# nickirk/pymes

Hardware: AMD Instinct MI355X
Metric: ccsd_iteration_time (lower is better)
Workload: dtype f64

## Files before the change

### include/pymes_amd.h

```cpp
#ifndef PYMES_AMD_H
#define PYMES_AMD_H

#include <stdint.h>

#ifdef __cplusplus
extern "C" {
#endif

typedef struct pymes_ctx pymes_ctx;

#define PYMES_NOCC_MAX_FUSED 90
#define PYMES_NOCC_MAX_LAMBDA 88
#define PYMES_NOCC_MAX_BRA_DRESS 80

const char* pymes_last_error(void);
const char* pymes_backend(void);
int pymes_ctx_create(pymes_ctx** out, int device, int no, int nv, uint64_t workspace_bytes );
int pymes_ctx_destroy(pymes_ctx* ctx);
int pymes_ctx_set_stream(pymes_ctx* ctx, void* hip_stream);
int pymes_ctx_sync(pymes_ctx* ctx);
int pymes_ctx_workspace(pymes_ctx* ctx, uint64_t* capacity_bytes, uint64_t* high_water_bytes);

int pymes_malloc(pymes_ctx* ctx, uint64_t bytes, void** dev_ptr);
int pymes_free(pymes_ctx* ctx, void* dev_ptr);
// ... 7 lines not shown

int pymes_graph_begin(pymes_ctx* ctx);
int pymes_graph_end(pymes_ctx* ctx, void** graph);
int pymes_graph_abort(pymes_ctx* ctx);
int pymes_graph_launch(pymes_ctx* ctx, void* graph);
int pymes_graph_destroy(pymes_ctx* ctx, void* graph);
int pymes_upload(pymes_ctx* ctx, void* dst_dev, const void* src_host, uint64_t bytes);
int pymes_download(pymes_ctx* ctx, void* dst_host, const void* src_dev, uint64_t bytes);
int pymes_copy(pymes_ctx* ctx, void* dst_dev, const void* src_dev, uint64_t bytes);
int pymes_memset_zero(pymes_ctx* ctx, void* dst_dev, uint64_t bytes);

int pymes_contract(pymes_ctx* ctx, double alpha,
                   const double* A_dev, const char* la, const int64_t* dimA, const int64_t* strideA,
                   const double* B_dev, const char* lb, const int64_t* dimB, const int64_t* strideB,
                   double beta, double* C_dev, const char* lc, const int64_t* dimC, const int64_t* strideC,
                   const char* batch);
int pymes_permute(pymes_ctx* ctx, double alpha, const double* in_dev, const char* li, const int64_t* dim_in,
                  const int64_t* stride_in, double beta, double* out_dev, const char* lo,
                  const int64_t* stride_out);
int pymes_dgemm(pymes_ctx* ctx, int64_t M, int64_t N, int64_t K, double alpha, const double* A_dev, int64_t a_sm,
                int64_t a_sk, const double* B_dev, int64_t b_sk, int64_t b_sn, double beta, double* C_dev,
                int64_t ldc);

int pymes_set_V_pqrs(pymes_ctx* ctx, const double* V, int on_device, const int64_t* strides);
int pymes_set_V_block(pymes_ctx* ctx, const char* name, const double* data, int64_t n_elements, int on_device,
                      const int64_t* strides);
int pymes_V_exchange_asymmetry(pymes_ctx* ctx, double* out_host);
int pymes_exchange_asymmetry(pymes_ctx* ctx, const double* A_dev, const double* B_dev, const int64_t* dims,
                             double* out_host);
int pymes_set_V_from_factors(pymes_ctx* ctx, const double* B_host, int naux);
int pymes_set_integral_shard(pymes_ctx* ctx, int rank, int world);
int pymes_integral_bytes(pymes_ctx* ctx, int64_t* bytes);
int pymes_shard_rows_ptr(pymes_ctx* ctx, const double** vp, const double** vm, int64_t* row0, int64_t* row1, int64_t* ldp,
                         int64_t* ldm);
int pymes_V_block_ptr(pymes_ctx* ctx, const char* name, int dressed, double** dev_ptr, int64_t* n_elements);
int pymes_set_orbital_energies(pymes_ctx* ctx, const double* eps_o_host, const double* eps_v_host);

int pymes_ccsd_t_triples(pymes_ctx* ctx, int64_t* n_triples);
int pymes_ccsd_t(pymes_ctx* ctx, const double* eps_host, const double* t1_dev, const double* t2_dev, int64_t t_begin,
                 int64_t t_end, double* per_triple_dev, double* e_out_host);

int pymes_ccsd_t_lambda(pymes_ctx* ctx, const double* eps_host, const double* t2_dev, const double* lam1_dev,
                        const double* lam2_dev, int64_t t_begin, int64_t t_end, double* per_triple_dev, double* e_out_host);

int pymes_fno_density(pymes_ctx* ctx, const double* v_ijab_dev, int n_frozen, double* D_host, double* e_mp2_host);
int pymes_derive_context(pymes_ctx* src, pymes_ctx* dst, int n_frozen, const double* C_host, int nv_dst);

int pymes_mp2(pymes_ctx* ctx, double level_shift, double* t2_dev, double* e_out_host);
int pymes_ccsd_dress_fock(pymes_ctx* ctx, const double* f_dev, const double* t1_dev, double* fd_dev);
#define PYMES_DRESS_ABIJ_REDUCED (1u << 16)
int pymes_ccsd_dress_V(pymes_ctx* ctx, const double* t1_dev, uint32_t block_mask);
int pymes_ccsd_dress_V_slab(pymes_ctx* ctx, const double* t1_dev, uint32_t block_mask, int p_begin, int p_end,
                            int q_begin, int q_end);
int pymes_ccsd_singles_residual(pymes_ctx* ctx, const double* fd_dev, const double* t1_dev, const double* t2_dev,
                                double* r1_dev);
int pymes_ccsd_singles_residual_partial(pymes_ctx* ctx, const double* fd_dev, const double* t1_dev, const double* t2_dev,
                                        double* r1_dev, int rank, int world, uint32_t flags );
#define PYMES_DCD 1u
#define PYMES_USE_DRESSED 2u
#define PYMES_SKIP_LADDER 4u
#define PYMES_SYM_LADDER 8u
#define PYMES_SLAB_RINGS_ONLY 64u
#define PYMES_SLAB_LADDERS_ONLY 128u
#define PYMES_REUSE_LAYOUTS 32u
#define PYMES_T1_ZERO (1u << 20)
#define PYMES_SYM_RINGS 16u
int pymes_doubles_residual(pymes_ctx* ctx, const double* f_dev, const double* t2_dev, double* r2_dev,
                           uint32_t flags);
int pymes_ladder(pymes_ctx* ctx, const double* t2_dev, double* r2_dev, int a_begin, int a_end, int dressed,
                 double beta);
int pymes_ladder_sym(pymes_ctx* ctx, const double* t2_dev, double* L_dev, int64_t row_begin, int64_t row_end,
                     int dressed, int hole_ladder);
int pymes_ladder_sym_unpack(pymes_ctx* ctx, const double* L_dev, double* r2_dev, double beta);
int pymes_ladder_sym_multi(pymes_ctx* ctx, const double* const* x_dev, int k, double* L_all_dev, int dressed);
int pymes_ladder_dress(pymes_ctx* ctx, const double* V_dev, const double* Pk_dev, const double* t1_dev, double* W_dev,
                       int64_t ld, int64_t r0, int64_t r1, int minus_half);
int pymes_pair_layouts(pymes_ctx* ctx, const double* x_dev, double* Xd_dev, double* Xx_dev, double* Xt_dev);
int pymes_symmetrised_assemble(pymes_ctx* ctx, const double* V_dev, const double* L_dev, const double* N_dev,
                               const double* D_dev, const double* X_dev, double* R_dev);
int pymes_hole_ladder_packed(pymes_ctx* ctx, const double* x_dev, const double* I_dev, double* L_dev, int64_t row_begin,
                             int64_t row_end, const double* y_dev);
int pymes_hole_ladder_packed_multi(pymes_ctx* ctx, const double* const* x_dev, const double* const* I_dev,
                                   const double* const* y_dev, int k, double* L_all_dev);
int pymes_ccsd_residuals(pymes_ctx* ctx, const double* f_dev, const double* t1_dev, const double* t2_dev, uint32_t flags,
                         double* r1_dev, double* r2_dev);
int pymes_ccsd_iterate(pymes_ctx* ctx, const double* f_dev, double* t1_dev, double* t2_dev, uint32_t flags, double level_shift,
                       double delta, double* dt1_dev, double* dt2_dev, double* out6_host);
int pymes_ccsd_release(pymes_ctx* ctx);

int pymes_residual_slab(pymes_ctx* ctx, const double* f_dev, const double* t2_dev, double* ETd_dev, double* ETx_dev,
                        double* L_dev, int rank, int world, uint32_t flags, const double* t1_dev, double* QK_dev,
                        const double* P_dev);
int pymes_slab_prepare_ws(pymes_ctx* ctx, int64_t* n_doubles);
int pymes_slab_prepare(pymes_ctx* ctx, const double* t2_dev, double* P_dev, int rank, int world, uint32_t flags);
int pymes_residual_finish(pymes_ctx* ctx, const double* f_dev, const double* t2_dev, const double* ETd_dev,
                          const double* ETx_dev, const double* L_dev, double* r2_dev, uint32_t flags,
                          const double* t1_dev, const double* QK_dev);
int pymes_ccsd_dress_abcd_rows(pymes_ctx* ctx, const double* t1_dev, int a_begin, int a_end, int lower_only);
int pymes_residual_finish_pairs(pymes_ctx* ctx, const double* f_dev, const double* t2_dev, const double* ETd_dev,
                                const double* ETx_dev, const double* L_dev, double* Rc_dev, uint32_t flags,
                                const double* t1_dev, const double* QK_dev, int rank, int world, const double* Xvv_dev);
int pymes_xvv_partial(pymes_ctx* ctx, const double* f_dev, const double* t2_dev, double* Xvv_dev, int rank, int world,
                      uint32_t flags);
int pymes_ccsd_dress_fock_ws(pymes_ctx* ctx, int64_t* n_doubles);
int pymes_ccsd_dress_fock_partial(pymes_ctx* ctx, const double* t1_dev, double* W_dev, int rank, int world);
int pymes_ccsd_dress_fock_finish(pymes_ctx* ctx, const double* f_dev, const double* t1_dev, const double* W_dev,
// ... 30 lines not shown
    double *ETd, *ETx, *L, *QK, *Tall, *W, *Xvv, *P, *R1, *S;
} pymes_shard_buffers;
int pymes_shard_buffer_sizes(pymes_ctx* ctx, int world, int64_t* sizes_out);
int pymes_ccsd_sharded_residuals(pymes_ctx* ctx, const double* f_dev, double* fd_dev, const double* t1_dev, double* t2_dev,
                                 const pymes_shard_buffers* buffers, uint32_t flags, double* rc_dev);
int pymes_ccsd_sharded_finish(pymes_ctx* ctx, const double* f_dev, const double* t1_dev, const double* tc_dev,
                              const double* dtc_dev, const pymes_shard_buffers* buffers, int* slot);
int pymes_ccsd_sharded_energy(pymes_ctx* ctx, int slot, double* out_host );
int pymes_ccsd_sharded_await(pymes_ctx* ctx, double* t2_dev, const pymes_shard_buffers* buffers);
int pymes_ccd_sharded_residuals(pymes_ctx* ctx, const double* f_dev, double* t2_dev, const pymes_shard_buffers* buffers,
                                uint32_t flags, double* rc_dev);
#define PYMES_OWNER_TILES (1u << 21)
typedef int (*pymes_alltoallv_fn)(void* user, const double* send_dev, const int64_t* send_counts, double* recv_dev,
                                  const int64_t* recv_counts, void* stream, int64_t* ticket);
int pymes_set_alltoallv(pymes_ctx* ctx, pymes_alltoallv_fn fn );
int pymes_owner_tile_sizes(pymes_ctx* ctx, int rank, int world, int64_t* send_doubles, int64_t* recv_doubles);
int pymes_set_owner_tile_buffers(pymes_ctx* ctx, double* send_dev, double* recv_dev);
int pymes_ccsd_energy(pymes_ctx* ctx, const double* f_dev, const double* t1_dev, const double* t2_dev,
                      double* e_out_host);
int pymes_ccd_energy(pymes_ctx* ctx, const double* t2_dev, double* e_out_host);

int pymes_ueg_eval_2b(pymes_ctx* ctx, int n_p, int n_ele, int imax, int mode, double L, double k_cutoff, double gamma,
                      int lattice_cutoff, const int32_t* k_int_host, const int32_t* index_map_host, double* V_dev);

int pymes_ueg_eval_2b_corr(pymes_ctx* ctx, int n_p, int n_ele, int imax, int mode, double L, int lattice_cutoff,
                           int correlator, const double* params_host, const int32_t* k_int_host,
                           const int32_t* index_map_host, double* V_dev);
int pymes_ueg_eval_2b_tab(pymes_ctx* ctx, int n_p, int n_ele, int imax, int mode, double L, int lattice_cutoff,
                          const int32_t* k_int_host, const int32_t* index_map_host, const double* tab_scalar_host,
                          const double* tab_array_host, int64_t tab_len, double* V_dev);

int pymes_dots(pymes_ctx* ctx, int npairs, const double* const* x_dev, const double* const* y_dev, int64_t n,
               double* out_host);
int pymes_dots_var(pymes_ctx* ctx, int npairs, const double* const* x_dev, const double* const* y_dev,
                   const int64_t* n, double* out_host);
int pymes_lincomb(pymes_ctx* ctx, double* out_dev, int nx, const double* const* x_dev, const double* c_host,
                  int64_t n);
int pymes_gemm_group_begin(pymes_ctx* ctx);
int pymes_gemm_group_end(pymes_ctx* ctx, int64_t* launches, int64_t* products);
int pymes_gram(pymes_ctx* ctx, int m, int n, const double* const* x_dev, const double* const* y_dev, int64_t len,
               double* out_host);
int pymes_lincomb_multi(pymes_ctx* ctx, int m, int n, const double* const* x_dev, const double* c_host,
                        const double* beta_host, double* const* y_dev, int64_t len);
int pymes_diis_mix(pymes_ctx* ctx, double* state_host, int ntypes, int m, int was_full, const double* const* err_hist_dev,
                   const double* const* err_new_dev, const int64_t* sizes, const double* const* amp_hist_dev,
                   double* const* out_dev);
int pymes_diis_step(pymes_ctx* ctx, double* state_dev, int npairs, const double* const* x_dev, const double* const* y_dev,
                    const int64_t* n, int ntypes, int m, int was_full);
int pymes_diis_solve(double* state_host, const double* overlaps_host, int ntypes, int m, int was_full);
int pymes_lincomb_dev(pymes_ctx* ctx, double* out_dev, int nx, const double* const* x_dev, const double* coeff_dev,
                      int64_t n);
#define PYMES_SYM_TAIL (1u << 22)
int pymes_sym_tail(pymes_ctx* ctx, int* yes);
int pymes_cc_update_to_sym(pymes_ctx* ctx, double* t_out_dev, double* dt_dev, const double* t_in_dev, const double* r_dev,
                           double level_shift, double delta);
int pymes_dots_sym(pymes_ctx* ctx, int npairs, const double* const* x_dev, const double* const* y_dev, const int64_t* n,
                   const int* sym, double* out_host);
int pymes_lincomb_sym(pymes_ctx* ctx, double* out_dev, int nx, const double* const* x_dev, const double* c_host, int64_t n);
int pymes_diis_mix_sym(pymes_ctx* ctx, double* state_host, int ntypes, int m, int was_full, const double* const* err_hist_dev,
                       const double* const* err_new_dev, const int64_t* sizes, const double* const* amp_hist_dev,
                       double* const* out_dev, const int* sym_types);
int pymes_energy_norms_start_sym(pymes_ctx* ctx, const double* f_dev, const double* t1_dev, const double* t2_dev,
                                 const double* dt2_dev, int* slot);
int pymes_pair_layouts_sym(pymes_ctx* ctx, const double* x_dev, double* Xd_dev, double* Xx_dev, double* Xt_dev);
int pymes_cmul(pymes_ctx* ctx, const double* mr_dev, const double* mi_dev, const double* xr_dev, const double* xi_dev,
               double* yr_dev, double* yi_dev, int64_t n);

int pymes_hf_fock_matrix(pymes_ctx* ctx, const double* h_host, double* f_host);

int pymes_fcidump_header(const char* path, int* n_elec, int* n_orb);
int pymes_fcidump_read_host(const char* path, int is_tc, double* e_core, double* eps_host, double* h_host,
                            double* V_host);
int pymes_fcidump_load(pymes_ctx* ctx, const char* path, int is_tc, double* e_core, double* eps_host, double* h_host,
                       int64_t* n_two_electron_lines);

int pymes_packed_header(const char* path, int* kind, int* n_elec, int* n_orb, int* naux);
int pymes_packed_load(pymes_ctx* ctx, const char* path, double* e_core, double* eps_host, double* h_host);
int pymes_packed_write(pymes_ctx* ctx, const char* path, int n_elec, double e_core, const double* eps_host,
                       const double* h_host);
int pymes_packed_write_factors(const char* path, int n_elec, int n_orb, int naux, double e_core, const double* eps_host,
                               const double* h_host, const double* B_host);

typedef struct pymes_eom pymes_eom;
int pymes_eom_sigma_prepare(pymes_ctx* ctx, const double* f_host, const double* t2_dev, int dressed, pymes_eom** out);
int pymes_eom_sigma_flags(pymes_eom* h, int* flags);
int pymes_eom_sigma_apply(pymes_eom* h, int k, const double* const* u1_dev, const double* const* u2_dev, const int* sym,
                          double* const* s1_dev, double* const* s2_dev);
int pymes_eom_diagonals(pymes_ctx* ctx, const double* f_host, const double* t2_dev, int dressed, double* d1_dev, double* d2_dev);
int pymes_scratch_trim(pymes_ctx* ctx);
int pymes_eom_sigma_destroy(pymes_eom* h);

#define PYMES_IPEA_IP 0
#define PYMES_IPEA_EA 1
typedef struct pymes_ipea pymes_ipea;
int pymes_ipea_sigma_prepare(pymes_ctx* ctx, const double* f_host, const double* t2_dev, int dressed, int kind, pymes_ipea** out);
int pymes_ipea_sigma_flags(pymes_ipea* h, int* flags);
int pymes_ipea_sigma_apply(pymes_ipea* h, int k, const double* const* r1_dev, const double* const* r2_dev, double* const* s1_dev,
                           double* const* s2_dev);
int pymes_ipea_sigma_diagonals(pymes_ipea* h, double* d1_dev, double* d2_dev);
int pymes_ipea_sigma_correction(pymes_ipea* h, int n, const double* const* s_dev, const double* const* r_dev, const double* w_host,
                                const double* d_dev, double shift, double* const* q_dev, int64_t off2, int64_t len,
                                double* norms_host);
int pymes_ipea_sigma_destroy(pymes_ipea* h);
int pymes_ipea_sigma_apply_left(pymes_ipea* h, int k, const double* const* l1_dev, const double* const* l2_dev,
                                double* const* o1_dev, double* const* o2_dev);
int pymes_ipea_dyson(pymes_ipea* h, const double* t1_dev, const double* lam1_dev, const double* lam2_dev, int k,
// ... 35 lines not shown
```

### pymes_amd/_lib.py

```python
import ctypes as C
import os

import numpy as np

_HERE = os.path.dirname(os.path.abspath(__file__))
DEFAULT_PATH = os.environ.get("PYMES_AMD_LIBRARY") or os.path.join(_HERE, "lib", "libpymes_amd.so")

c_double_p = C.POINTER(C.c_double)
c_i64_p = C.POINTER(C.c_int64)


class ShardBuffers(C.Structure):
    _fields_ = [(k, C.c_void_p) for k in ("ETd", "ETx", "L", "QK", "Tall", "W", "Xvv", "P", "R1", "S")]

c_pp = C.POINTER(C.c_void_p)

SIGNATURES = {
    "pymes_last_error": (C.c_char_p, []),
    "pymes_backend": (C.c_char_p, []),
    "pymes_ctx_create": (C.c_int, [c_pp, C.c_int, C.c_int, C.c_int, C.c_uint64]),
    "pymes_ctx_destroy": (C.c_int, [C.c_void_p]),
    "pymes_ctx_set_stream": (C.c_int, [C.c_void_p, C.c_void_p]),
    "pymes_ctx_sync": (C.c_int, [C.c_void_p]),
    "pymes_ctx_workspace": (C.c_int, [C.c_void_p, C.POINTER(C.c_uint64), C.POINTER(C.c_uint64)]),
# ... 108 lines not shown
    "pymes_scatter": (C.c_int, [C.c_void_p, C.c_void_p, C.c_uint64, c_i64_p, c_double_p, C.c_int64]),
    "pymes_tc_single_contraction": (C.c_int, [C.c_void_p, C.c_void_p, C.c_int, C.c_int, C.c_void_p]),
    "pymes_tc_double_contraction": (C.c_int, [C.c_void_p, C.c_void_p, C.c_int, C.c_int, C.c_void_p]),
    "pymes_tc_triple_contraction": (C.c_int, [C.c_void_p, C.c_void_p, C.c_int, C.c_int, c_double_p]),
    "pymes_dots": (C.c_int, [C.c_void_p, C.c_int, c_pp, c_pp, C.c_int64, c_double_p]),
    "pymes_dots_var": (C.c_int, [C.c_void_p, C.c_int, c_pp, c_pp, c_i64_p, c_double_p]),
    "pymes_lincomb": (C.c_int, [C.c_void_p, C.c_void_p, C.c_int, c_pp, c_double_p, C.c_int64]),
    "pymes_cmul": (C.c_int, [C.c_void_p] * 7 + [C.c_int64]),
    "pymes_ccsd_residuals": (C.c_int, [C.c_void_p, C.c_void_p, C.c_void_p, C.c_void_p, C.c_uint32, C.c_void_p, C.c_void_p]),
    "pymes_ccsd_iterate": (C.c_int, [C.c_void_p, C.c_void_p, C.c_void_p, C.c_void_p, C.c_uint32, C.c_double, C.c_double,
                                     C.c_void_p, C.c_void_p, C.c_void_p]),
    "pymes_ccsd_release": (C.c_int, [C.c_void_p]),
    "pymes_set_collectives": (C.c_int, [C.c_void_p, C.c_void_p]),
    "pymes_shard_buffer_sizes": (C.c_int, [C.c_void_p, C.c_int, c_i64_p]),
    "pymes_ccsd_sharded_residuals": (C.c_int, [C.c_void_p] * 6 + [C.c_uint32, C.c_void_p]),
    "pymes_ccd_sharded_residuals": (C.c_int, [C.c_void_p] * 4 + [C.c_uint32, C.c_void_p]),
    "pymes_set_alltoallv": (C.c_int, [C.c_void_p, C.c_void_p]),
    "pymes_owner_tile_sizes": (C.c_int, [C.c_void_p, C.c_int, C.c_int, c_i64_p, c_i64_p]),
    "pymes_set_owner_tile_buffers": (C.c_int, [C.c_void_p, C.c_void_p, C.c_void_p]),
    "pymes_ccsd_sharded_finish": (C.c_int, [C.c_void_p] * 6 + [C.POINTER(C.c_int)]),
    "pymes_ccsd_sharded_energy": (C.c_int, [C.c_void_p, C.c_int, C.c_void_p]),
    "pymes_ccsd_sharded_await": (C.c_int, [C.c_void_p, C.c_void_p, C.c_void_p]),
    "pymes_cshift_inv": (C.c_int, [C.c_void_p, C.c_void_p] + [C.c_double] * 5 + [C.c_void_p, C.c_void_p, C.c_int64]),
    "pymes_eom_sigma_prepare": (C.c_int, [C.c_void_p, C.c_void_p, C.c_void_p, C.c_int, C.c_void_p]),
    "pymes_eom_sigma_flags": (C.c_int, [C.c_void_p, C.c_void_p]),
    "pymes_eom_sigma_apply": (C.c_int, [C.c_void_p, C.c_int] + [C.c_void_p] * 5),
    "pymes_eom_diagonals": (C.c_int, [C.c_void_p, C.c_void_p, C.c_void_p, C.c_int, C.c_void_p, C.c_void_p]),
    "pymes_scratch_trim": (C.c_int, [C.c_void_p]),
    "pymes_eom_sigma_destroy": (C.c_int, [C.c_void_p]),
    "pymes_eom_sigma_apply_left": (C.c_int, [C.c_void_p, C.c_int] + [C.c_void_p] * 5),
    "pymes_lambda_step": (C.c_int, [C.c_void_p] * 5 + [C.c_double, C.c_double, C.c_int, C.c_int] + [C.c_void_p] * 5),
    "pymes_rdm1": (C.c_int, [C.c_void_p] * 5 + [C.c_double, C.c_void_p]),
    "pymes_ipea_sigma_prepare": (C.c_int, [C.c_void_p, C.c_void_p, C.c_void_p, C.c_int, C.c_int, C.c_void_p]),
    "pymes_ipea_sigma_flags": (C.c_int, [C.c_void_p, C.c_void_p]),
    "pymes_ipea_sigma_apply": (C.c_int, [C.c_void_p, C.c_int] + [C.c_void_p] * 4),
    "pymes_ipea_sigma_apply_left": (C.c_int, [C.c_void_p, C.c_int] + [C.c_void_p] * 4),
    "pymes_ipea_dyson": (C.c_int, [C.c_void_p] * 4 + [C.c_int] + [C.c_void_p] * 6),
    "pymes_ipea_sigma_diagonals": (C.c_int, [C.c_void_p, C.c_void_p, C.c_void_p]),
    "pymes_ipea_sigma_correction": (C.c_int, [C.c_void_p, C.c_int, C.c_void_p, C.c_void_p, C.c_void_p, C.c_void_p, C.c_double,
                                              C.c_void_p, C.c_int64, C.c_int64, C.c_void_p]),
    "pymes_ipea_sigma_destroy": (C.c_int, [C.c_void_p]),
    "pymes_tdm1": (C.c_int, [C.c_void_p] * 5 + [C.c_int] + [C.c_void_p] * 7),
    "pymes_eom_correction": (C.c_int, [C.c_void_p, C.c_int, C.c_void_p, C.c_void_p, C.c_void_p, C.c_void_p, C.c_double,
                                       C.c_void_p, C.c_int64, C.c_int64, C.c_void_p]),
    "pymes_diis_mix": (C.c_int, [C.c_void_p, C.c_void_p, C.c_int, C.c_int, C.c_int, c_pp, c_pp, c_i64_p, c_pp, c_pp]),
    "pymes_diis_solve": (C.c_int, [C.c_void_p, C.c_void_p, C.c_int, C.c_int, C.c_int]),
    "pymes_diis_step": (C.c_int, [C.c_void_p, C.c_void_p, C.c_int, c_pp, c_pp, c_i64_p, C.c_int, C.c_int, C.c_int]),
    "pymes_gemm_group_begin": (C.c_int, [C.c_void_p]),
    "pymes_gemm_group_end": (C.c_int, [C.c_void_p, c_i64_p, c_i64_p]),
    "pymes_gram": (C.c_int, [C.c_void_p, C.c_int, C.c_int, c_pp, c_pp, C.c_int64, c_double_p]),
    "pymes_lincomb_multi": (C.c_int, [C.c_void_p, C.c_int, C.c_int, c_pp, C.c_void_p, C.c_void_p, c_pp, C.c_int64]),
    "pymes_lincomb_dev": (C.c_int, [C.c_void_p, C.c_void_p, C.c_int, c_pp, C.c_void_p, C.c_int64]),
    "pymes_sym_tail": (C.c_int, [C.c_void_p, C.POINTER(C.c_int)]),
    "pymes_cc_update_to_sym": (C.c_int, [C.c_void_p, C.c_void_p, C.c_void_p, C.c_void_p, C.c_void_p, C.c_double, C.c_double]),
    "pymes_dots_sym": (C.c_int, [C.c_void_p, C.c_int, c_pp, c_pp, c_i64_p, C.POINTER(C.c_int), c_double_p]),
    "pymes_lincomb_sym": (C.c_int, [C.c_void_p, C.c_void_p, C.c_int, c_pp, c_double_p, C.c_int64]),
    "pymes_diis_mix_sym": (C.c_int, [C.c_void_p, C.c_void_p, C.c_int, C.c_int, C.c_int, c_pp, c_pp, c_i64_p, c_pp, c_pp,
                                     C.POINTER(C.c_int)]),
    "pymes_energy_norms_start_sym": (C.c_int, [C.c_void_p, C.c_void_p, C.c_void_p, C.c_void_p, C.c_void_p,
                                               C.POINTER(C.c_int)]),
    "pymes_pair_layouts_sym": (C.c_int, [C.c_void_p, C.c_void_p, C.c_void_p, C.c_void_p, C.c_void_p]),
    "pymes_stats": (C.c_int, [C.c_void_p, C.c_int, c_i64_p, c_double_p, c_i64_p, c_double_p]),
    "pymes_prof_enable": (C.c_int, [C.c_void_p, C.c_int]),
    "pymes_prof_reset": (C.c_int, [C.c_void_p]),
    "pymes_prof_query": (C.c_int, [C.c_void_p, C.c_int, c_i64_p, c_i64_p, c_double_p, c_double_p]),
}

PYMES_DCD, PYMES_USE_DRESSED, PYMES_SKIP_LADDER, PYMES_SYM_LADDER, PYMES_SYM_RINGS = 1, 2, 4, 8, 16
PYMES_OWNER_TILES = 1 << 21
PYMES_REUSE_LAYOUTS = 32
PYMES_T1_ZERO = 1 << 20
PYMES_SYM_TAIL = 1 << 22
PYMES_SLAB_RINGS_ONLY, PYMES_SLAB_LADDERS_ONLY = 64, 128
PYMES_DRESS_ABIJ_REDUCED = 1 << 16


class PymesError(RuntimeError):
    pass


class Library:

    BACKEND = "hip-gfx950"

    def __init__(self, path=None):
        path = path or DEFAULT_PATH
        if not os.path.exists(path):
            raise PymesError(
                f"{path} not found: build the HIP extension first (python -c 'import __graft_entry__ as g; "
                "g.build()' or make -C pymes_amd/csrc).  pymes_amd has no CPU fallback.")
        self.path = path
        self.dll = C.CDLL(path)
        for name, (res, args) in SIGNATURES.items():
            fn = getattr(self.dll, name)
            fn.restype, fn.argtypes = res, args
        self.backend = self.dll.pymes_backend().decode()
        if self.backend != self.BACKEND:
            raise PymesError(f"{path} reports backend '{self.backend}', expected '{self.BACKEND}'")

    def call(self, name, *args):
        rc = getattr(self.dll, name)(*args)
        if rc != 0:
            raise PymesError(f"{name}: {self.dll.pymes_last_error().decode()}")


_default = None
# ... 21 lines not shown
```

### pymes_amd/csrc/capi.cpp

```cpp
#include <chrono>
#include <cstdio>
#include <cstring>
#include <exception>
#include <algorithm>
#include <mutex>
#include <set>
#include <string>
#include <vector>

#include "../../include/pymes_amd.h"
#include "diis_small.h"
#include "engine.h"
#include "eom.h"
#include "fcidump.h"
#include "packed.h"

using pymes::Engine;
using pymes::TView;

struct pymes_ctx {
    Engine* e;
};
struct pymes_eom {
    pymes::EomSigma* s;
// ... 368 lines not shown
        need(eo, "eps_o");
        need(ev, "eps_v");
        E(ctx).set_orbital_energies(eo, ev);
    });
}

int pymes_mp2(pymes_ctx* ctx, double shift, double* t2, double* e_out) {
    return guarded([&] {
        need(t2, "t2");
        need(e_out, "e_out");
        E(ctx).mp2(shift, t2, e_out);
    });
}
int pymes_ccsd_dress_fock(pymes_ctx* ctx, const double* f, const double* t1, double* fd) {
    return guarded([&] {
        need(f, "f"); need(t1, "t1"); need(fd, "fd");
        E(ctx).dress_fock(f, t1, fd);
    });
}
int pymes_ccsd_residuals(pymes_ctx* ctx, const double* f, const double* t1, const double* t2, uint32_t flags, double* r1,
                         double* r2) {
    return guarded([&] {
        need(f, "f"); need(t1, "t1"); need(t2, "t2"); need(r1, "r1"); need(r2, "r2");
        if (flags & ~(PYMES_DCD | PYMES_T1_ZERO | PYMES_SYM_TAIL))
            throw pymes::Error("ccsd_residuals: flags are PYMES_DCD | PYMES_T1_ZERO | PYMES_SYM_TAIL");
        E(ctx).ccsd_residuals(f, t1, t2, (flags & PYMES_DCD) | ((flags & PYMES_T1_ZERO) ? Engine::kT1Zero : 0u) |
                                             ((flags & PYMES_SYM_TAIL) ? Engine::kSymTail : 0u), r1, r2);
    });
}
int pymes_ccsd_iterate(pymes_ctx* ctx, const double* f, double* t1, double* t2, uint32_t flags, double level_shift, double delta,
                       double* dt1, double* dt2, double* out6) {
    return guarded([&] {
        need(f, "f"); need(t1, "t1"); need(t2, "t2"); need(dt1, "dt1"); need(dt2, "dt2"); need(out6, "out");
        if (flags & ~(PYMES_DCD | PYMES_T1_ZERO)) throw pymes::Error("ccsd_iterate: flags are PYMES_DCD | PYMES_T1_ZERO");
        Engine& e = E(ctx);
        if (e.capturing()) throw pymes::Error("ccsd_iterate reads the energy back: not inside a launch graph");
        e.ccsd_iterate(f, t1, t2, (flags & PYMES_DCD) | ((flags & PYMES_T1_ZERO) ? Engine::kT1Zero : 0u), level_shift, delta, dt1,
                       dt2, out6);
    });
}
int pymes_ccsd_release(pymes_ctx* ctx) {
    return guarded([&] {
        Engine& e = E(ctx);
        if (e.capturing()) throw pymes::Error("ccsd_release while a launch graph is being recorded");
        e.release_residual_buffers();
    });
}
int pymes_ccsd_dress_V(pymes_ctx* ctx, const double* t1, uint32_t mask) {
    return guarded([&] {
        need(t1, "t1");
        E(ctx).dress_V(t1, mask);
    });
}
int pymes_ccsd_dress_V_slab(pymes_ctx* ctx, const double* t1, uint32_t mask, int p_begin, int p_end, int q_begin,
                            int q_end) {
    return guarded([&] {
        need(t1, "t1");
        const int64_t cut[4] = {p_begin, p_end, q_begin, q_end};
        E(ctx).dress_V(t1, mask, cut);
    });
}
int pymes_ccsd_singles_residual(pymes_ctx* ctx, const double* fd, const double* t1, const double* t2, double* r1) {
    return guarded([&] {
        need(fd, "fd"); need(t1, "t1"); need(t2, "t2"); need(r1, "r1");
        E(ctx).singles_residual(fd, t1, t2, r1);
    });
}
int pymes_ccsd_singles_residual_partial(pymes_ctx* ctx, const double* fd, const double* t1, const double* t2, double* r1,
                                        int rank, int world, uint32_t flags) {
    return guarded([&] {
        need(fd, "fd"); need(t1, "t1"); need(t2, "t2"); need(r1, "r1");
        E(ctx).singles_residual_partial(fd, t1, t2, r1, rank, world, (flags & PYMES_REUSE_LAYOUTS) != 0);
    });
}
int pymes_doubles_residual(pymes_ctx* ctx, const double* f, const double* t2, double* r2, uint32_t flags) {
    return guarded([&] {
        need(f, "f"); need(t2, "t2"); need(r2, "r2");
        E(ctx).doubles_residual(f, t2, r2, flags);
    });
}
int pymes_ladder(pymes_ctx* ctx, const double* t2, double* r2, int a0, int a1, int dressed, double beta) {
    return guarded([&] {
        need(t2, "t2"); need(r2, "r2");
        E(ctx).ladder(t2, r2, a0, a1, dressed != 0, beta);
    });
}
int pymes_ladder_sym(pymes_ctx* ctx, const double* t2, double* L, int64_t r0, int64_t r1, int dressed, int hole) {
    return guarded([&] {
        need(t2, "t2"); need(L, "L");
        E(ctx).ladder_sym(t2, L, r0, r1, dressed != 0, hole);
    });
}
int pymes_symmetrised_assemble(pymes_ctx* ctx, const double* V, const double* L, const double* N, const double* D,
                               const double* X, double* R) {
    return guarded([&] {
        need(N, "N"); need(D, "D"); need(X, "X"); need(R, "R");
        pymes::Engine& e = E(ctx);
        if (!dev::fused_pair_kernels_ok(e.no)) throw pymes::Error("symmetrised_assemble: nocc too large for the LDS tile");
        dev::residual_assemble(V, L, N, D, X, R, e.no, e.nv, e.stream);
    });
}
int pymes_hole_ladder_packed(pymes_ctx* ctx, const double* x, const double* I, double* L, int64_t r0, int64_t r1,
                             const double* y) {
    return guarded([&] {
        need(x, "x"); need(I, "I"); need(L, "L");
        E(ctx).hole_ladder_packed(x, I, L, r0, r1, y);
// ... 127 lines not shown
            dev::pairs_unpack(xc_all + static_cast<int64_t>(r) * (c1 - c0) * 2 * o2, full, e.no, e.nv, r0, r1, e.stream);
        }
    });
}
int pymes_cc_update_pairs(pymes_ctx* ctx, double* tc, double* dtc, const double* rc, double shift, double delta, int rank,
                          int world) {
    return guarded([&] {
        need(tc, "tc"); need(dtc, "dtc"); need(rc, "rc");
        pymes::Engine& e = E(ctx);
        int64_t r0, r1;
        e.need_eps("cc_update_pairs");
        e.pair_chunk(rank, world, r0, r1);
        dev::cc_update_pairs(tc, dtc, rc, e.eps_o, e.eps_v, shift, delta, e.no, e.nv, r0, r1, e.stream);
    });
}
int pymes_ccsd_dress_abcd_rows(pymes_ctx* ctx, const double* t1, int a0, int a1, int lower_only) {
    return guarded([&] {
        need(t1, "t1");
        E(ctx).dress_abcd_rows(t1, a0, a1, lower_only != 0);
    });
}
int pymes_cc_update(pymes_ctx* ctx, double* t, double* dt, const double* r, double shift, double delta, int rank) {
    return guarded([&] {
        need(t, "t"); need(dt, "dt"); need(r, "r");
        E(ctx).cc_update(t, dt, r, shift, delta, rank);
    });
}
int pymes_cc_update_to(pymes_ctx* ctx, double* t_out, double* dt, const double* t_in, const double* r, double shift,
                       double delta, int rank) {
    return guarded([&] {
        need(t_out, "t_out"); need(dt, "dt"); need(t_in, "t_in"); need(r, "r");
        E(ctx).cc_update_to(t_out, dt, t_in, r, shift, delta, rank);
    });
}
int pymes_energy_norms(pymes_ctx* ctx, const double* f, const double* t1, const double* t2, const double* dt2,
                       double* out) {
    return guarded([&] {
        need(t2, "t2"); need(out, "out");
        if ((f == nullptr) != (t1 == nullptr)) throw pymes::Error("f and t1 must be given together");
        E(ctx).energy_norms(f, t1, t2, dt2, out);
    });
}
int pymes_energy_norms_start(pymes_ctx* ctx, const double* f, const double* t1, const double* t2, const double* dt2, int* slot) {
    return guarded([&] {
        need(t2, "t2"); need(slot, "slot");
        if ((f == nullptr) != (t1 == nullptr)) throw pymes::Error("f and t1 must be given together");
        *slot = E(ctx).energy_norms_start(f, t1, t2, dt2);
    });
}
int pymes_sym_tail(pymes_ctx* ctx, int* yes) {
    return guarded([&] {
        need(yes, "yes");
        *yes = Eq(ctx).sym_tail() ? 1 : 0;
    });
}
int pymes_cc_update_to_sym(pymes_ctx* ctx, double* t_out, double* dt, const double* t_in, const double* r, double shift,
                           double delta) {
    return guarded([&] {
        need(t_out, "t_out"); need(dt, "dt"); need(t_in, "t_in"); need(r, "r");
        E(ctx).cc_update_to(t_out, dt, t_in, r, shift, delta, 4, true);
    });
}
int pymes_energy_norms_start_sym(pymes_ctx* ctx, const double* f, const double* t1, const double* t2, const double* dt2,
                                 int* slot) {
    return guarded([&] {
        need(t2, "t2"); need(slot, "slot");
        if ((f == nullptr) != (t1 == nullptr)) throw pymes::Error("f and t1 must be given together");
        *slot = E(ctx).energy_norms_start(f, t1, t2, dt2, true);
    });
}
int pymes_pair_layouts_sym(pymes_ctx* ctx, const double* x, double* Xd, double* Xx, double* Xt) {
    return guarded([&] {
        need(x, "x"); need(Xx, "Xx"); need(Xt, "Xt");
        Engine& e = E(ctx);
        if (!dev::fused_pair_kernels_ok(e.no)) throw pymes::Error("pair_layouts: nocc too large for the LDS tile");
        if (e.sym_tail()) dev::t2_layouts_sym(x, Xd, Xx, Xt, e.no, e.nv, e.stream);
        else dev::t2_layouts(x, Xd, Xx, Xt, e.no, e.nv, e.stream);
    });
}
int pymes_energy_norms_wait(pymes_ctx* ctx, int slot, double* out) {
    return guarded([&] {
        need(out, "out");
        Eq(ctx).energy_norms_wait(slot, out);
    });
}
int pymes_readback_start(pymes_ctx* ctx, const double* dev_ptr, int n, int* slot) {
    return guarded([&] {
        need(dev_ptr, "dev_ptr"); need(slot, "slot");
        *slot = dev::readback_start(dev_ptr, n, E(ctx).stream);
    });
}
int pymes_readback_wait(pymes_ctx* ctx, int slot, double* out, int n) {
    return guarded([&] {
        need(out, "out");
        Eq(ctx);
        dev::readback_wait(slot, out, n);
    });
}
int pymes_energy_norms_pairs(pymes_ctx* ctx, const double* f, const double* t1, const double* tc, const double* dtc,
                             int rank, int world, double* out) {
    return guarded([&] {
        need(tc, "tc"); need(out, "out");
        if ((f == nullptr) != (t1 == nullptr)) throw pymes::Error("f and t1 must be given together");
        E(ctx).energy_norms_pairs(f, t1, tc, dtc, rank, world, out);
    });
}
// ... 696 lines not shown
```

### pymes_amd/csrc/cc.cpp

```cpp
#include <algorithm>
#include <cstdio>
#include <cstring>
#include <cstdlib>
#include <optional>
#include <vector>

#include "../../include/pymes_amd.h"
#include "engine.h"

#include <cmath>

namespace pymes {
static_assert(Engine::kT1Zero == PYMES_T1_ZERO && Engine::kOwnerTiles == PYMES_OWNER_TILES,
              "the engine's flag bits are the public ones");

namespace {
inline int64_t lpitch(int64_t n) { return PairDims::lpitch(n); }
inline TView packed_rows(double* p, int64_t rows, int64_t cols) { return slice(make_view(p, {rows, lpitch(cols)}), 1, 0, cols); }
inline TView pitched(double* p, int64_t r, int64_t c, int64_t ld) { return slice(make_view(p, {r, ld}), 1, 0, c); }
constexpr int P_klij = 0, P_ijka = 1, P_ijak = 2, P_ijab = 3, P_iajk = 4, P_iajb = 5, P_iabj = 6, P_iabc = 7,
              P_aibc = 11, P_abij = 12, P_abic = 13, P_abci = 14, P_abcd = 15;
}

double* Engine::get_static(const std::string& key) {
// ... 142 lines not shown
        contract(1.0, X1, "ajcl", Tx, "clbi", 0.0, Rx, "ajbi");
    }

    permute(1.0, Rd, "aibj", 1.0, R, "abij");
    if (quad) permute(1.0, Rx, "ajbi", 1.0, R, "abij");
    permute(1.0, Exd, "aibj", 1.0, R, "abij");
    permute(1.0, Exd, "bjai", 1.0, R, "abij");
    permute(1.0, Exx, "ajbi", 1.0, R, "abij");
    permute(1.0, Exx, "biaj", 1.0, R, "abij");
    permute(1.0, Exn, "abij", 1.0, R, "abij");
    permute(1.0, Exn, "baji", 1.0, R, "abij");
}

void Engine::ensure_xs() {
    if (!xs_oo_) xs_oo_ = static_cast<double*>(dev::dmalloc(sizeof(double) * no * no));
    if (!xs_vv_) xs_vv_ = static_cast<double*>(dev::dmalloc(sizeof(double) * nv * nv));
}

bool Engine::ring_fold_enabled() {
    if (const char* e = getenv("PYMES_RING_FOLD")) return atoi(e) != 0;
    return true;
}

bool Engine::sym_tail() const {
    if (const char* e = getenv("PYMES_SYM_TAIL"))
        if (atoi(e) == 0) return false;
    return dev::sym_tail_ok() && dev::fused_pair_kernels_ok(no);
}

void Engine::pair_layouts_of(const double* t2, bool want_td, bool sym) {
    const int64_t o = no, v = nv, ov = o * v;
    for (int i = want_td ? 0 : 1; i < 3; ++i)
        if (!lay_[i]) {
            if (capturing_) throw Error("pair_layouts_of: the pair layouts must exist before a launch graph is recorded (run one eager pass first)");
            lay_[i] = static_cast<double*>(dev::dmalloc(sizeof(double) * ov * ov));
        }
    lay_t2_ = nullptr;
    if (dev::fused_pair_kernels_ok(no)) {
        if (sym && sym_tail()) dev::t2_layouts_sym(t2, want_td ? lay_[0] : nullptr, lay_[1], lay_[2], no, nv, stream);
        else dev::t2_layouts(t2, want_td ? lay_[0] : nullptr, lay_[1], lay_[2], no, nv, stream);
        stats.permute_calls++;
        stats.permute_bytes += 8.0 * (want_td ? 5.0 : 4.0) * double(ov * ov);
    } else {
        TView T = make_view(const_cast<double*>(t2), {v, v, o, o});
        TView t4 = make_view(lay_[0], {v, o, v, o});
        if (want_td) permute(1.0, T, "abij", 0.0, t4, "aibj");
        t4.p = lay_[1];
        permute(1.0, T, "abij", 0.0, t4, "ajbi");
        t4.p = lay_[2];
        permute(2.0, T, "abij", 0.0, t4, "aibj");
        permute(-1.0, T, "baij", 1.0, t4, "aibj");
    }
    lay_t2_ = t2;
}

void Engine::slab_ladders(const double* t2, double* L, int rank, int world, unsigned flags, const double* t1, double* QK,
                          const double* P) {
    const bool dcd = flags & PYMES_DCD, dressed = flags & PYMES_USE_DRESSED;
    const int64_t o = no, v = nv;
    int64_t r0, r1;
    chunk(pair_dims().npp, rank, world, r0, r1);
    if (t1) {
        if (!QK) throw Error("residual_slab: QK buffer missing");
        int64_t q0, q1;
        chunk(o * v, rank, world, q0, q1);
        ladder_t1(t1, t2, L, r0, r1, QK, q0, q1, dcd, P ? P + o * o : nullptr);
    } else {
        ladder_sym(t2, L, r0, r1, dressed, dcd ? 2 : 1);
    }
}

void Engine::slab_rings_rows(const RingSlab& s) {
    const int64_t ov = static_cast<int64_t>(no) * nv, c0 = s.c0, c1 = s.c1, nc = c1 - c0;
    const bool quad = s.quad;
    const TView &Tx = s.Tx, &Ttd = s.Ttd, &ETd = s.ETd, &ETx = s.ETx;
    auto pairm = [&](double* p) { return make_view(p, {ov, ov}); };
    auto slabT = [&]() { return make_view(arena.alloc(nc * ov), {nc, ov}); };
    TView MT = slabT(), N1T = slabT();
    s.load_rows(2.0, s.Viabj, "kbcj", MT);
    s.load_rows(-1.0, s.Viajb, "kbjc", N1T);
    axpby(1.0, N1T, 1.0, MT);
    ring_xd_ = 0.0;
    auto rowsOf = [&](const TView& m) { return slice(m, 0, c0, c1); };
    if (quad) {
        contract(0.5, rowsOf(Ttd), "ny", pairm(get_static("Ld")), "yx", 1.0, MT, "nx");
        contract(0.5, rowsOf(Tx), "ny", pairm(get_static("Vx")), "yx", 1.0, N1T, "nx");
    } else {
        contract(1.0, rowsOf(Ttd), "ny", pairm(get_static("Vd")), "yx", 1.0, MT, "nx");
    }
    contract(1.0, N1T, "nk", Tx, "km", 0.0, ETx, "nm");
    contract(0.5, MT, "nk", Ttd, "km", 0.5, ETd, "nm", "", &ETx);
}

void Engine::slab_rings_cols(const RingSlab& s) {
    const int64_t o = no, v = nv, nn = n, ov = o * v, c0 = s.c0, c1 = s.c1, nc = c1 - c0;
    const bool quad = s.quad, traces = s.traces, fold = s.fold;
    const double w = quad ? 1.0 : 0.5;
    const double* t2 = s.t2;
    const TView &F = s.F, &Viajb = s.Viajb, &Viabj = s.Viabj, &Tx = s.Tx, &Ttd = s.Ttd, &ETd = s.ETd, &ETx = s.ETx;
    auto pairm = [&](double* p) { return make_view(p, {ov, ov}); };
    auto slab = [&]() { return make_view(arena.alloc(ov * nc), {ov, nc}); };
    auto cols = [&](const TView& m) { return slice(m, 1, c0, c1); };
    TView M = slab(), N1 = slab();
    const int64_t ring_tiles = ((ov + 127) / 128) * ((ov + 127) / 128);
    const bool paired = ring_tiles < 512;
    ring_xd_ = paired ? 0.5 : 0.0;
// ... 35 lines not shown
        ensure_xs();
        xs_oo_tag_.clear();
        xs_vv_tag_.clear();
        dev::pair_traces(M.p, nc, -cz, 0.0, xs_vv_, xs_oo_, no, nv, stream, quad ? N1.p : nullptr, -cu);
    }
    if (quad && paired) {
        pair_gemm(0.5, get_static("Ldh"), get_static("Vx"), Ttd.p, Tx.p, 1.0, M.p, N1.p);
    } else if (quad) {
        contract(0.5, pairm(get_static("Ld")), "xy", cols(Ttd), "yn", 1.0, M, "xn");
        contract(0.5, pairm(get_static("Vx")), "xy", cols(Tx), "yn", 1.0, N1, "xn");
    } else {
        contract(paired ? 0.5 : 1.0, pairm(get_static("Vd")), "xy", cols(Ttd), "yn", 1.0, M, "xn");
    }
    if (traces) {
        dev::pair_traces(M.p, nc, cz, 1.0, xs_vv_, xs_oo_, no, nv, stream, quad ? N1.p : nullptr, cu);
        xs_oo_tag_.set(t2, 0, 1);
        xs_vv_tag_.set(t2, 0, 1);
    }
    if (fold) {
        TView Xoo = make_view(arena.alloc(o * o), {o, o}), Xvv = make_view(arena.alloc(v * v), {v, v});
        copy(slice(slice(F, 0, 0, o), 1, 0, o), Xoo);
        axpby(w, make_view(xs_oo_, {o, o}), 1.0, Xoo);
        copy(slice(slice(F, 0, o, nn), 1, o, nn), Xvv);
        axpby(-w, make_view(xs_vv_, {v, v}), 1.0, Xvv);
        auto add_Dx = [&](const TView& m, double wgt) {
            const int64_t ld = m.st[0];
            const int64_t dv[3] = {v, v, o}, sv_in[3] = {1, v, 0}, sv_out[3] = {o * ld, o, ld + 1};
            axpby(wgt, make_view(Xvv.p, 3, dv, sv_in), 1.0, make_view(m.p, 3, dv, sv_out));
            const int64_t dn[3] = {v, o, o}, so_in[3] = {0, o, 1}, so_out[3] = {o * ld + o, ld, 1};
            axpby(-wgt, make_view(Xoo.p, 3, dn, so_in), 1.0, make_view(m.p, 3, dn, so_out));
        };
        add_Dx(M, paired ? 0.25 : 0.5);
        add_Dx(N1, 0.5);
        ring_fold_.set(t2, s.ETd_p);
    }
    if (paired) {
        pair_gemm(1.0, Tx.p, Ttd.p, N1.p, M.p, 0.0, ETx.p, ETd.p);
    } else {
        contract(1.0, Tx, "mk", N1, "kn", 0.0, ETx, "mn");
        contract(0.5, Ttd, "mk", M, "kn", 0.5, ETd, "mn", "", &ETx);
    }
}

void Engine::residual_slab(const double* f, const double* t2, double* ETd_p, double* ETx_p, double* L, int rank,
                           int world, unsigned flags, const double* t1, double* QK, const double* P) {
    const bool dcd = flags & PYMES_DCD, dressed = flags & PYMES_USE_DRESSED,
               skip_ladder = flags & (PYMES_SKIP_LADDER | PYMES_SLAB_RINGS_ONLY), skip_rings = flags & PYMES_SLAB_LADDERS_ONLY;
    const bool quad = !dcd;
    const int64_t o = no, v = nv, nn = n, ov = o * v;
    if (world < 1 || rank < 0 || rank >= world) throw Error("residual_slab: bad rank/world");
    if (L && !skip_ladder) check_shard_rank("residual_slab", rank, world);
    const double w = quad ? 1.0 : 0.5;
    TView F = make_view(const_cast<double*>(f), {nn, nn});
    if (L && !skip_ladder) slab_ladders(t2, L, rank, world, flags, t1, QK, P);
    if (skip_rings) return;
    ring_fold_.clear();
    int64_t c0, c1;
    chunk(ov, rank, world, c0, c1);
    const int64_t nc = c1 - c0;
    if (nc <= 0) return;
    TView Viajb = block(P_iajb, dressed), Viabj = block(P_iabj, dressed);

    ArenaScope scope(arena);
    auto pairm = [&](double* p) { return make_view(p, {ov, ov}); };
    const bool traces = !P && nc == ov;
    const bool fold = traces && ring_fold_enabled();
    pair_layouts_of(t2, !fold, flags & kSymTail);
    TView Td = pairm(lay_[0]), Tx = pairm(lay_[1]), Ttd = pairm(lay_[2]);
    TView ETd = slice(pairm(ETd_p), 0, c0, c1), ETx = slice(pairm(ETx_p), 0, c0, c1);
    const int64_t b0 = c0 / o, b1 = (c1 + o - 1) / o;
    auto load_cols = [&](double alpha, const TView& blk, const char* spec, const TView& dst) {
        TView src = slice(blk, 1, b0, b1);
        if (b0 * o == c0 && b1 * o == c1) {
            permute(alpha, src, spec, 0.0, make_view(dst.p, {v, o, b1 - b0, o}), "ckbj");
        } else {
            ArenaScope s2(arena);
            TView tmp = make_view(arena.alloc(ov * (b1 - b0) * o), {ov, (b1 - b0) * o});
            permute(alpha, src, spec, 0.0, make_view(tmp.p, {v, o, b1 - b0, o}), "ckbj");
            copy(slice(tmp, 1, c0 - b0 * o, c1 - b0 * o), dst);
        }
    };
    auto load_rows = [&](double alpha, const TView& blk, const char* spec, const TView& dst) {
        TView src = slice(blk, 1, b0, b1);
        if (b0 * o == c0 && b1 * o == c1) {
            permute(alpha, src, spec, 0.0, make_view(dst.p, {b1 - b0, o, v, o}), "bjck");
        } else {
            ArenaScope s2(arena);
            TView tmp = make_view(arena.alloc((b1 - b0) * o * ov), {(b1 - b0) * o, ov});
            permute(alpha, src, spec, 0.0, make_view(tmp.p, {b1 - b0, o, v, o}), "bjck");
            copy(slice(tmp, 0, c0 - b0 * o, c1 - b0 * o), dst);
        }
    };
    const RingSlab rs{t2, ETd_p, quad, traces, fold, c0, c1, F, Viajb, Viabj, Tx, Ttd, ETd, ETx, load_cols, load_rows};
    if (nc != ov) slab_rings_rows(rs);
    else slab_rings_cols(rs);
    if (!fold) {
        ArenaScope s2(arena);
        TView Foo = slice(slice(F, 0, 0, o), 1, 0, o);
        TView Xoo = make_view(arena.alloc(o * o), {o, o});
        copy(Foo, Xoo);
        if (P) {
            axpby(1.0, make_view(const_cast<double*>(P), {o, o}), 1.0, Xoo);
        } else if (traces) {
            axpby(w, make_view(xs_oo_, {o, o}), 1.0, Xoo);
        } else {
            TView Tp = make_view(arena.alloc(o * o * v * v), {v, v, o, o});
            permute(1.0, make_view(Ttd.p, {v, o, v, o}), "cidl", 0.0, Tp, "cdli");
            contract(w, make_view(get_static("Vk3"), {v, v, o, o}), "cdlk", Tp, "cdli", 1.0, Xoo, "ki");
        }
        TView Trows = make_view(Td.p + c0 * ov, {nc, v, o});
        TView Erows = make_view(ETd.p, {nc, v, o});
        contract(-1.0, Trows, "nak", Xoo, "ki", 1.0, Erows, "nai");
    }
}

int64_t Engine::slab_prepare_ws_doubles() const {
    const PairDims d = pair_dims();
    return static_cast<int64_t>(no) * no + d.opp * d.ldp + d.opp * d.ldm;
}

// ... 537 lines not shown
    const double t_q = 2.0 * double(o * v) * (double(npp) * double(opp) + double(npm) * double(opm)) / 70e12;
    return t_dress < 0.8 * t_q;
}

void Engine::ladder_t1(const double* t1, const double* t2, double* L, int64_t row0, int64_t row1, double* QK,
                       int64_t q0, int64_t q1, bool dcd, const double* J) {
    const PairDims d = pair_dims();
    const int64_t o = no, v = nv, ov = o * v, npp = d.npp, npm = d.npm, opp = d.opp, opm = d.opm, ldp = d.ldp, ldm = d.ldm;
    if (row0 < 0 || row1 > npp || row0 > row1) throw Error("ladder_t1: bad pair-row range");
    if (q0 < 0 || q1 > ov || q0 > q1) throw Error("ladder_t1: bad (k,b) row range");
    const int64_t rows = row1 - row0, qrows = q1 - q0;
    const PackedV V = rows > 0 ? ladder_rows("ladder_t1", row0, row1, false) : PackedV{nullptr, nullptr, false};
    bool dress = bra_dress_pays();
    const std::string kkey = ":" + std::to_string(q0) + ":" + std::to_string(q1);
    const std::string rkey = ":" + std::to_string(row0) + ":" + std::to_string(row1);
    if (dress && rows > 0 && (!static_.count("VpKx") || !static_.count("VpDress" + rkey))) {
        const int64_t lp = d.vlp, lm = d.vlm;
        const bool need_p = !static_.count("VpKx");
        double *tp = nullptr, *tm = nullptr, *px = nullptr, *mx = nullptr, *wp = nullptr, *wm = nullptr;
        bool ok = true;
        auto grab = [&](double*& p, int64_t n) { if (ok) { p = static_cast<double*>(dev::try_dmalloc(sizeof(double) * n)); ok = p != nullptr; } };
        if (!static_.count("VpDress" + rkey)) { grab(wp, rows * lp); grab(wm, rows * lm); }
        if (need_p) { grab(px, ov * lp); grab(mx, ov * lm); grab(tp, ov * lp); grab(tm, ov * lm); }
        if (!ok) {
            for (double* p : {tp, tm, px, mx, wp, wm}) dev::dfree(p);
            if (!(rows == npp && qrows == ov))
                throw Error("ladder_t1: out of device memory for the dressed copy of the packed V_abcd (PYMES_LADDER_DRESS=0 on every rank selects the Q_kb form)");
            dress_off_ = true;
            dress = false;
        } else {
            if (wp) {
                static_["VpDress" + rkey] = wp; static_["VmDress" + rkey] = wm;
                static_doubles_["VpDress" + rkey] = rows * lp; static_doubles_["VmDress" + rkey] = rows * lm;
            }
            if (need_p) {
                static_["VpKx"] = px;
                static_["VmKx"] = mx;
                static_doubles_["VpKx"] = ov * lp; static_doubles_["VmKx"] = ov * lm;
                dev::ladder_pack_V(block(P_iabc).p, tp, tm, 0, nv, 0, ov, stream, lp, lm);
                permute(1.0, make_view(tp, {o, v, lp}), "kxc", 0.0, make_view(px, {v, o, lp}), "xkc");
                permute(1.0, make_view(tm, {o, v, lm}), "kxc", 0.0, make_view(mx, {v, o, lm}), "xkc");
                dev::stream_sync(stream);
                dev::dfree(tp);
                dev::dfree(tm);
            }
        }
    }
    if (!dress && qrows > 0 && !static_.count("VpK" + kkey)) {
        double* vp = new_static("VpK" + kkey, qrows * d.vlp);
        double* vm = new_static("VmK" + kkey, qrows * d.vlm);
        dev::ladder_pack_V(block(P_iabc).p, vp, vm, 0, nv, q0, q1, stream, d.vlp, d.vlm);
    }
    ijab_pack();
    ArenaScope scope(arena);
    TView Lrows = make_view(L + row0 * o * o, {rows, o * o});
    TView LS = slice(Lrows, 1, 0, opp), LA = slice(Lrows, 1, opp, o * o);
    {
        ArenaScope s2(arena);
        double* Sp = arena.alloc(npp * ldp);
        double* Am = arena.alloc(std::max<int64_t>(npm * ldm, 1));
        dev::ladder_pack_T(t2, t1, Sp, Am, no, nv, dev::PACK_ROW_HALF, ldp, ldm, stream);
        stats.permute_calls++;
        stats.permute_bytes += 8.0 * 2.0 * double(v * v * o * o);
        TView SpT = pitched(Sp, npp, opp, ldp), AmT = pitched(Am, npm, opm, ldm);
        const double* Ap = V.Vp;
        const double* Am_ = V.Vm;
        if (dress && rows > 0) {
            ArenaScope s3(arena);
            double* ws = arena.alloc(dev::ladder_dress_ws_doubles(no, nv));
            dev::ladder_dress(Ap, static_["VpKx"], t1, static_["VpDress" + rkey], no, nv, d.vlp, row0, row1, -1.0, ws, stream);
            if (npm > 0)
                dev::ladder_dress(Am_, static_["VmKx"], t1, static_["VmDress" + rkey], no, nv, d.vlm, row0, row1, 1.0, ws, stream);
            Ap = static_["VpDress" + rkey];
            Am_ = static_["VmDress" + rkey];
        }
        TView Qp, QS, QA;
        if (qrows > 0 && !dress) {
            Qp = make_view(arena.alloc(qrows * o * o), {qrows, o * o});
            QS = slice(Qp, 1, 0, opp);
            QA = slice(Qp, 1, opp, o * o);
        }
        {
            GemmGroupScope grp(stream);
            if (rows > 0) {
                contract(1.0, packed_rows(const_cast<double*>(Ap), rows, npp), "rk", SpT, "kn", 0.0, LS, "rn");
                if (opm > 0 && npm > 0) contract(1.0, packed_rows(const_cast<double*>(Am_), rows, npm), "rk", AmT, "kn", 0.0, LA, "rn");
            }
            if (qrows > 0 && !dress) {
                contract(1.0, packed_rows(static_["VpK" + kkey], qrows, npp), "rk", SpT, "kn", 0.0, QS, "rn");
                if (opm > 0 && npm > 0) contract(1.0, packed_rows(static_["VmK" + kkey], qrows, npm), "rk", AmT, "kn", 0.0, QA, "rn");
            }
            grp.close();
        }
        if (rows > 0 && opm > 0 && npm <= 0) zero(LA);
        if (qrows > 0 && dress) {
            TView t = make_view(const_cast<double*>(t1), {v, o});
            TView Qr = make_view(QK + q0 * o * o, {qrows, o, o});
            axpby(1.0, make_view(block(P_iajk).p + q0 * o * o, {qrows, o, o}), 0.0, Qr);
            contract(1.0, make_view(block(P_iabj).p + q0 * v * o, {qrows, v, o}), "qcj", t, "ci", 1.0, Qr, "qij", "q");
            contract(1.0, make_view(block(P_iajb).p + q0 * o * v, {qrows, o, v}), "qid", t, "dj", 1.0, Qr, "qij");
        } else if (qrows > 0) {
            if (opm > 0 && npm <= 0) zero(QA);
            dev::rows_unpack(Qp.p, QK + q0 * o * o, qrows, no, stream);
            TView t = make_view(const_cast<double*>(t1), {v, o});
            TView Qr = make_view(QK + q0 * o * o, {qrows, o, o});
            axpby(1.0, make_view(block(P_iajk).p + q0 * o * o, {qrows, o, o}), 1.0, Qr);
            contract(1.0, make_view(block(P_iabj).p + q0 * v * o, {qrows, v, o}), "qcj", t, "ci", 1.0, Qr, "qij", "q");
            contract(1.0, make_view(block(P_iajb).p + q0 * o * v, {qrows, o, v}), "qid", t, "dj", 1.0, Qr, "qij");
        }
    }
    if (rows == 0) return;
    const HoleOperand h = hole_operand(block(P_klij, true).p);
    TView Ipv = pitched(h.Ip, opp, opp, ldp), Imv = pitched(h.Im, opp, opm, ldm);
    TView IpK = pitched(h.Ip, ldp, opp, ldp), ImK = pitched(h.Im, ldp, opm, ldm);
    double* SpR = arena.alloc(npp * ldp);
    double* AmR = arena.alloc(npp * ldp);
    const int rflags = dev::PACK_COL_HALF | dev::PACK_AM_PROWS | dev::PACK_AM_PCOLS;
    auto rowsS = [&]() { return slice(make_view(SpR, {npp, ldp}), 0, row0, row1); };
    auto rowsA = [&]() { return slice(make_view(AmR, {npp, ldp}), 0, row0, row1); };
    if (dcd) {
        hole_operand_add(h, nullptr, nullptr, 2.0);
        dev::ladder_pack_T(t2, nullptr, SpR, AmR, no, nv, rflags, ldp, ldp, stream, row0, row1);
        contract(1.0, rowsS(), "rk", IpK, "kn", 1.0, LS, "rn");
        if (opm > 0) contract(1.0, rowsA(), "rk", ImK, "kn", 1.0, LA, "rn");
    }
    const double bI = dcd ? 1.0 : 2.0;
    if (J) {
        double* j = const_cast<double*>(J);
        axpby(1.0, pitched(j, opp, opp, ldp), bI, Ipv);
        if (opm > 0) axpby(1.0, pitched(j + opp * ldp, opp, opm, ldm), bI, Imv);
    } else {
        ArenaScope s2(arena);
        double* Sp = arena.alloc(npp * ldp);
        double* Am = arena.alloc(std::max<int64_t>(npm * ldm, 1));
        dev::ladder_pack_T(t2, nullptr, Sp, Am, no, nv, dev::PACK_ROW_HALF, ldp, ldm, stream);
        hole_operand_add(h, Sp, Am, bI, true);
    }
    dev::ladder_pack_T(dcd ? nullptr : t2, t1, SpR, AmR, no, nv, rflags, ldp, ldp, stream, row0, row1);
    stats.permute_calls += 3;
    stats.permute_bytes += 8.0 * 4.0 * double(v * v * o * o);
    GemmGroupScope grp(stream);
    contract(1.0, rowsS(), "rk", IpK, "kn", 1.0, LS, "rn");
    if (opm > 0) contract(1.0, rowsA(), "rk", ImK, "kn", 1.0, LA, "rn");
    grp.close();
}

void Engine::ladder_sym_unpack(const double* L, double* r2, double beta) {
    dev::ladder_unpack(L, r2, beta, no, nv, stream);
    stats.permute_calls++;
    stats.permute_bytes += 8.0 * 2.5 * double(nv) * nv * no * no;
}

int64_t Engine::dress_fock_ws_doubles() const {
    const int64_t o = no, v = nv;
    return 2 * v * v + 4 * o * v + 2 * o * o;
}

void Engine::dress_fock_partial(const double* t1, double* W, int rank, int world) {
    const int64_t o = no, v = nv;
    if (world < 1 || rank < 0 || rank >= world) throw Error("dress_fock_partial: bad rank/world");
    int64_t j0, j1;
    chunk(o, rank, world, j0, j1);
    TView G1 = make_view(W, {v, v}), G2 = make_view(G1.p + v * v, {v, v}), J1 = make_view(G2.p + v * v, {o, v}),
          J2 = make_view(J1.p + o * v, {o, v}), L1 = make_view(J2.p + o * v, {o, o}), L2 = make_view(L1.p + o * o, {o, o}),
          K1 = make_view(L2.p + o * o, {o, v}), K2 = make_view(K1.p + o * v, {v, o});
    if (j1 <= j0) {
        dev::memset_zero(W, sizeof(double) * dress_fock_ws_doubles(), stream);
        return;
    }
    TView t = slice(make_view(const_cast<double*>(t1), {v, o}), 1, j0, j1);
    const bool all = (j0 == 0 && j1 == o);
    auto js = [&](int pat) { return all ? block(pat) : slice(block(pat), 0, j0, j1); };
    const bool fused_g12 = dev::fock_g12_ok(nv);
    if (fused_g12) {
        ArenaScope s2(arena);
        const int ja = static_cast<int>(j0), jb = static_cast<int>(j1);
        double* ws = arena.alloc(dev::fock_g12_ws_doubles(nv, nv, jb - ja));
        dev::fock_g12(block(P_iabc).p, t1, G1.p, G2.p, no, nv, nv, ja, jb, ws, stream);
        double* ws2 = arena.alloc(dev::fock_g12_ws_doubles(nv, no, jb - ja));
        dev::fock_g12(block(P_ijab).p, t1, J1.p, J2.p, no, nv, no, ja, jb, ws2, stream);
    }
    struct Batch {
        Batch() { dev::gemv_batch_begin(); }
        ~Batch() { try { dev::gemv_batch_end(); } catch (...) {} }
    };
    {
        Batch batch;
        if (!fused_g12) {
            contract(1.0, t, "bj", js(P_iabc), "jabc", 0.0, G1, "ac");
            contract(1.0, t, "bj", js(P_iabc), "jacb", 0.0, G2, "ac");
        }
        if (!fused_g12) {
            contract(1.0, t, "bj", js(P_ijab), "jkbc", 0.0, J1, "kc");
            contract(1.0, t, "bj", js(P_ijab), "jkcb", 0.0, J2, "kc");
        }
        contract(1.0, t, "bj", js(P_ijak), "jkbi", 0.0, L1, "ki");
        contract(1.0, t, "bj", js(P_ijka), "jkib", 0.0, L2, "ki");
        contract(1.0, t, "bj", js(P_iabj), "jabi", 0.0, K1, "ia");
        contract(1.0, t, "bj", js(P_iajb), "jaib", 0.0, K2, "ai");
        dev::gemv_batch_end();
    }
}

void Engine::dress_fock_finish(const double* f, const double* t1, const double* W, double* fd) {
    ArenaScope scope(arena);
    dev::fock_finish(f, t1, W, fd, arena.alloc(static_cast<int64_t>(no) * no), no, nv, stream);
}

void Engine::dress_fock(const double* f, const double* t1, double* fd) {
    ArenaScope scope(arena);
    double* W = arena.alloc(dress_fock_ws_doubles());
    dress_fock_partial(t1, W, 0, 1);
    dress_fock_finish(f, t1, W, fd);
}

void Engine::xvv_partial(const double* f, const double* t2, double* Xvv_p, int rank, int world, unsigned flags) {
    const bool dcd = flags & PYMES_DCD;
    const int64_t o = no, v = nv, nn = n;
    if (world < 1 || rank < 0 || rank >= world) throw Error("xvv_partial: bad rank/world");
    int64_t k0, k1;
    chunk(o, rank, world, k0, k1);
    TView Xvv = make_view(Xvv_p, {v, v});
    TView F = make_view(const_cast<double*>(f), {nn, nn});
    if (rank == 0) copy(slice(slice(F, 0, o, nn), 1, o, nn), Xvv);
    else zero(Xvv);
    ensure_xs();
    xs_vv_tag_.clear();
    TView S = make_view(xs_vv_, {v, v});
    if (k1 <= k0) {
        zero(S);
    } else {
        ArenaScope scope(arena);
        TView T = make_view(const_cast<double*>(t2), {v, v, o, o});
        TView Tk = slice(T, 2, k0, k1);
        TView Ttd = make_view(arena.alloc(v * (k1 - k0) * v * o), {v, k1 - k0, v, o});
        permute(2.0, Tk, "adkl", 0.0, Ttd, "akdl");
        permute(-1.0, Tk, "dakl", 1.0, Ttd, "akdl");
        TView Vk = slice(make_view(get_static("Vk"), {o, v, o, v}), 0, k0, k1);
        contract(1.0, Ttd, "akdl", Vk, "kdlc", 0.0, S, "ac");
        axpby(dcd ? -0.5 : -1.0, S, 1.0, Xvv);
    }
    xs_vv_tag_.set(t2, rank, world);
}

void Engine::dressed_into(int pattern, const std::vector<int>& pos, int k, const TView& t1v, const TView& dst,
                          bool reduced, const int64_t* cut) {
    auto has = [&](int axis) { return cut && cut[2 * axis + 1] > cut[2 * axis]; };
    auto cutq = [&](TView v, int pat) {
        for (int axis = 0; axis < 2; ++axis)
            if (has(axis) && (pat >> (3 - axis) & 1)) v = slice(v, axis, cut[2 * axis], cut[2 * axis + 1]);
        return v;
    };
    if (k == 0) {
        copy(cutq(block(pattern), pattern), dst);
        return;
    }
    const bool fuse_copy = (k - 1 == 0);
    if (!fuse_copy) dressed_into(pattern, pos, k - 1, t1v, dst, reduced, cut);
    const TView raw = fuse_copy ? cutq(block(pattern), pattern) : TView();
    const TView* cin = fuse_copy ? &raw : nullptr;
    if (cin) {
        bool same = true;
        for (int i = 0; i < 4; ++i) same = same && (raw.dim[i] == 1 || raw.st[i] == dst.st[i]);
        if (!same) {
            copy(raw, dst);
            cin = nullptr;
        }
    }
    const int x = pos[k - 1];
    const int other = pattern ^ (1 << (3 - x));
    int depth = k - 1;
    if (reduced && k == 4) depth = 2;
    if (reduced && k == 2) depth = 0;
    ArenaScope scope(arena);
    TView oth;
    long memo_key = ((long)other << 8) | (long)depth;
    for (int i = 0; i < depth; ++i) memo_key = (memo_key << 3) | (long)(pos[i] + 1);
    if (depth == 0) {
        oth = cutq(block(other), other);
    } else if (!reduced && dress_memo_.count(memo_key)) {
        oth = dress_memo_[memo_key];
    } else {
        int64_t d[4];
        for (int i = 0; i < 4; ++i) d[i] = (other >> (3 - i) & 1) ? nv : no;
        for (int axis = 0; axis < 2; ++axis)
            if (has(axis) && (other >> (3 - axis) & 1)) d[axis] = cut[2 * axis + 1] - cut[2 * axis];
        oth = make_view(arena.alloc(d[0] * d[1] * d[2] * d[3]), 4, d, nullptr);
        dressed_into(other, pos, depth, t1v, oth, reduced, cut);
    }
    const TView tcut = (x < 2 && has(x)) ? slice(t1v, 0, cut[2 * x], cut[2 * x + 1]) : t1v;
    switch (x) {
        case 3: contract(1.0, oth, "pqrx", t1v, "xs", 1.0, dst, "pqrs", "", cin); break;
        case 2: contract(1.0, oth, "pqxs", t1v, "xr", 1.0, dst, "pqrs", "pq", cin); break;
        case 1: contract(-1.0, tcut, "qx", oth, "pxrs", 1.0, dst, "pqrs", "p", cin); break;
        case 0: contract(-1.0, tcut, "px", oth, "xqrs", 1.0, dst, "pqrs", "", cin); break;
        default: throw Error("bad index position");
    }
}

void Engine::dress_V(const double* t1, uint32_t mask, const int64_t* cut) {
    ++dress_generation_;
    TView t = make_view(const_cast<double*>(t1), {(int64_t)nv, (int64_t)no});
    for (int axis = 0; axis < 2 && cut; ++axis)
        if (cut[2 * axis] < 0 || cut[2 * axis + 1] > nv || cut[2 * axis] > cut[2 * axis + 1]) throw Error("dress_V: bad index range");
    ArenaScope memo_scope(arena);
    struct MemoGuard {
        std::map<long, TView>& m;
        ~MemoGuard() { m.clear(); }
    } memo_guard{dress_memo_};
    dress_memo_.clear();
    if ((mask >> P_klij & 1u) && (mask >> P_iabj & 1u)) {
        const int pat = P_klij | 2;
        const std::vector<int> pos = {3};
        int64_t d[4] = {no, no, nv, no};
        TView oth = make_view(arena.alloc(d[0] * d[1] * d[2] * d[3]), 4, d, nullptr);
        dressed_into(pat, pos, 1, t, oth, false, cut);
        dress_memo_[(((long)pat << 8 | 1L) << 3) | 4L] = oth;
    }
    for (int pat = 0; pat < 16; ++pat) {
        if (!(mask >> pat & 1u)) continue;
        TView dst = block_view(ensure_dressed(pat), pat);
        for (int axis = 0; axis < 2 && cut; ++axis) {
            if (cut[2 * axis + 1] <= cut[2 * axis]) continue;
            if (!(pat >> (3 - axis) & 1)) continue;
            dst = slice(dst, axis, cut[2 * axis], cut[2 * axis + 1]);
        }
        std::vector<int> pos;
        if (!(pat >> 0 & 1)) pos.push_back(3);
        if (!(pat >> 1 & 1)) pos.push_back(2);
        if (pat >> 2 & 1) pos.push_back(1);
        if (pat >> 3 & 1) pos.push_back(0);
        dressed_into(pat, pos, static_cast<int>(pos.size()), t, dst, pat == P_abij && (mask >> 16 & 1u), cut);
        if (pat == P_abcd && lpack_.dressed) lpack_.valid = false;
    }
}

void Engine::singles_residual(const double* fd, const double* t1, const double* t2, double* r1) {
    const int64_t o = no, v = nv, nn = n;
    TView D = make_view(const_cast<double*>(fd), {nn, nn});
    TView Dov = slice(slice(D, 0, 0, o), 1, o, nn), Dvo = slice(slice(D, 0, o, nn), 1, 0, o);
    TView t = make_view(const_cast<double*>(t1), {v, o});
    TView T = make_view(const_cast<double*>(t2), {v, v, o, o});
    TView R = make_view(r1, {v, o});
    ArenaScope scope(arena);
    TView Tq = make_view(arena.alloc(o * o * v * v), {v, o, v, o});
    TView P1 = make_view(arena.alloc(o * o * v * v), {o, v, v, o});
    permute(2.0, T, "abij", 0.0, Tq, "aibj");
    permute(-1.0, T, "abji", 1.0, Tq, "aibj");
    permute(2.0, T, "bcij", 0.0, P1, "jbci");
    permute(-1.0, T, "bcji", 1.0, P1, "jbci");
    copy(Dvo, R);
    contract(1.0, Tq, "aibj", Dov, "jb", 1.0, R, "ai");
    contract(1.0, block(P_aibc), "ajbc", P1, "jbci", 1.0, R, "ai");
    TView S2 = make_view(arena.alloc(o * o), {o, o});
    contract(1.0, make_view(get_static("Vjbck"), {o, v, v, o}), "jbck", P1, "jbci", 0.0, S2, "ki");
    contract(-1.0, t, "ak", S2, "ki", 1.0, R, "ai");
    contract(-1.0, Tq, "ajbk", block(P_ijka), "jkib", 1.0, R, "ai");
    TView S4 = make_view(arena.alloc(v * v), {v, v});
    contract(1.0, Tq, "ajbk", block(P_ijab), "jkcb", 0.0, S4, "ac");
    contract(-1.0, S4, "ac", t, "ci", 1.0, R, "ai");
}

void Engine::singles_residual_partial(const double* fd, const double* t1, const double* t2, double* r1, int rank, int world,
                                      bool reuse_layouts) {
    const int64_t o = no, v = nv, nn = n;
    if (world < 1 || rank < 0 || rank >= world) throw Error("singles_residual_partial: bad rank/world");
    int64_t j0, j1;
    chunk(o, rank, world, j0, j1);
    const int64_t nj = j1 - j0;
    TView D = make_view(const_cast<double*>(fd), {nn, nn});
// ... 18 lines not shown
    } else {
        Tq = make_view(arena.alloc(v * nj * v * o), {v, nj, v, o});
        P1 = make_view(arena.alloc(nj * v * v * o), {nj, v, v, o});
        permute(2.0, slice(T, 2, j0, j1), "abjk", 0.0, Tq, "ajbk");
        permute(-1.0, slice(T, 3, j0, j1), "abkj", 1.0, Tq, "ajbk");
        permute(2.0, slice(T, 3, j0, j1), "bcij", 0.0, P1, "jbci");
        permute(-1.0, slice(T, 2, j0, j1), "bcji", 1.0, P1, "jbci");
    }
    contract(1.0, Tq, "bjai", slice(Dov, 0, j0, j1), "jb", 1.0, R, "ai");
    contract(1.0, slice(block(P_aibc), 1, j0, j1), "ajbc", P1, lp1, 1.0, R, "ai");
    if (!have_oo) {
        TView S2 = make_view(arena.alloc(o * o), {o, o});
        contract(1.0, slice(make_view(get_static("Vjbck"), {o, v, v, o}), 0, j0, j1), "jbck", P1, lp1, 0.0, S2, "ki");
        contract(-1.0, t, "ak", S2, "ki", 1.0, R, "ai");
    }
    contract(-1.0, Tq, "ajbk", slice(block(P_ijka), 0, j0, j1), "jkib", 1.0, R, "ai");
    if (!have_vv) {
        TView S4 = make_view(arena.alloc(v * v), {v, v});
        contract(1.0, Tq, "ajbk", slice(block(P_ijab), 0, j0, j1), "jkcb", 0.0, S4, "ac");
        contract(-1.0, S4, "ac", t, "ci", 1.0, R, "ai");
    }
}

void Engine::cc_update(double* t, double* dt, const double* r, double shift, double delta, int rank) {
    if (rank != 2 && rank != 4) throw Error("cc_update: rank must be 2 (T1) or 4 (T2)");
    need_eps("cc_update");
    dev::cc_update(t, dt, r, eps_o, eps_v, shift, delta, no, nv, rank, stream);
}

void Engine::ccsd_residuals(const double* f, const double* t1, const double* t2, unsigned flags, double* r1, double* r2) {
    refuse_if_sharded("ccsd_residuals (single rank)");
    const int64_t o = no, v = nv, ov = o * v, npp = v * (v + 1) / 2;
    if (!res_ETd_) {
        if (capturing_) throw Error("ccsd_residuals: the staging buffers must exist before a launch graph is recorded (run one eager pass first)");
        double* got[5] = {nullptr, nullptr, nullptr, nullptr, nullptr};
        const int64_t want[5] = {(o + v) * (o + v), ov * ov, ov * ov, npp * o * o, ov * o * o};
        try {
            for (int i = 0; i < 5; ++i) got[i] = scratch_get(want[i]);
        } catch (...) {
            for (double* p : got)
                if (p) scratch_put(p);
            throw;
        }
        res_fd_ = got[0]; res_ETd_ = got[1]; res_ETx_ = got[2]; res_L_ = got[3]; res_QK_ = got[4];
    }
    const unsigned dcd = flags & PYMES_DCD;
    const unsigned sym = PYMES_SYM_LADDER | PYMES_SYM_RINGS, tail = flags & kSymTail;
    if (flags & PYMES_T1_ZERO) {
        residual_slab(f, t2, res_ETd_, res_ETx_, res_L_, 0, 1, dcd | sym | tail);
        singles_residual_partial(f, t1, t2, r1, 0, 1, true);
        residual_finish(f, t2, res_ETd_, res_ETx_, res_L_, r2, dcd | sym | PYMES_REUSE_LAYOUTS);
        return;
    }
    dress_fock(f, t1, res_fd_);
    dress_V(t1, (1u << pattern_of_name("klij")) | (1u << pattern_of_name("iajb")) | (1u << pattern_of_name("iabj")));
    residual_slab(res_fd_, t2, res_ETd_, res_ETx_, res_L_, 0, 1, dcd | sym | tail | PYMES_USE_DRESSED, t1, res_QK_);
    singles_residual_partial(res_fd_, t1, t2, r1, 0, 1, true);
    residual_finish(res_fd_, t2, res_ETd_, res_ETx_, res_L_, r2, dcd | sym | PYMES_USE_DRESSED | PYMES_REUSE_LAYOUTS, t1, res_QK_);
}

void Engine::ccsd_iterate(const double* f, double* t1, double* t2, unsigned flags, double shift, double delta, double* dt1,
                          double* dt2, double out[6]) {
    refuse_if_sharded("ccsd_iterate (single rank)");
    const int64_t o = no, v = nv;
    if (!res_r1_) {
        if (capturing_) throw Error("ccsd_iterate: the staging buffers must exist before a launch graph is recorded");
        double* r1 = scratch_get(v * o);
        try {
            res_r2_ = scratch_get(v * v * o * o);
        } catch (...) {
            scratch_put(r1);
            throw;
        }
        res_r1_ = r1;
    }
    ccsd_residuals(f, t1, t2, flags | kSymTail, res_r1_, res_r2_);
    cc_update_to(t1, dt1, t1, res_r1_, shift, delta, 2);
    cc_update_to(t2, dt2, t2, res_r2_, shift, delta, 4, true);
    energy_norms(f, t1, t2, dt2, out, true);
}

void Engine::set_collectives(const Collectives* c) {
    if (t2_in_flight_) {
        t2_in_flight_ = false;
        dev::phase_sync();
        if (coll_.wait(coll_.user, t2_ticket_, stream) != 0) throw Error("collective hook: wait failed");
    }
    if (!c) {
        coll_ = Collectives();
        coll_set_ = false;
        return;
    }
    if (!c->allreduce_start || !c->allgather_start || !c->wait) throw Error("set_collectives: allreduce_start, allgather_start and wait are required");
    if (c->world < 1 || c->rank < 0 || c->rank >= c->world) throw Error("set_collectives: need 0 <= rank < world");
    coll_ = *c;
    coll_set_ = true;
}

namespace {
struct Hooks {
    const Engine::Collectives& c;
    void* stream;
    int64_t allreduce(double* buf, int64_t n) const {
        dev::gemm_group_sync();
        dev::phase_sync();
        int64_t t = 0;
        if (c.allreduce_start(c.user, buf, n, stream, &t) != 0) throw Error("collective hook: allreduce_start failed");
        return t;
// ... 834 lines not shown
```

### pymes_amd/csrc/device_api.h

```cpp
#pragma once
#include <cstddef>
#include <cstdint>

namespace dev {

typedef void* stream_t;

const char* backend_name();
void  set_device(int ordinal);
void* dmalloc(size_t bytes);
void* try_dmalloc(size_t bytes);
void  dfree(void* p);
void  memcpy_h2d(void* d, const void* h, size_t bytes, stream_t s);
void  memcpy_d2h(void* h, const void* d, size_t bytes, stream_t s);
void  memcpy_d2d(void* d, const void* s_, size_t bytes, stream_t s);
void  memset_zero(void* d, size_t bytes, stream_t s);
void  stream_sync(stream_t s);
size_t mem_free_bytes();
size_t mem_total_bytes();
stream_t stream_create();
void  stream_destroy(stream_t s);
int64_t live_allocations();
typedef void* event_t;
event_t event_create();
// ... 29 lines not shown
bool fock_g12_ok(int nv);
int64_t fock_g12_ws_doubles(int nv, int na, int nj);
void fock_g12(const double* V, const double* t1, double* G1, double* G2, int no, int nv, int na, int j0, int j1, double* ws,
              stream_t s);
void fock_finish(const double* f, const double* t1, const double* W, double* fd, double* ft, int no, int nv, stream_t s);
void gemv_batch_begin();
void gemv_batch_end();

void gemm_group_begin(stream_t s);
void gemm_group_end();
void gemm_group_sync();
void gemm_group_stats(long* launches, long* products);

void phase_sync();
bool phase_pending();
long phase_generation();
void phase_enable(int mode);
void phase_hold(bool on);
void phase_call_end();
void phase_stats(long* tasks, long* launches, long* levels, long* flushes);

struct Permute {
    int rank;
    int64_t dim[6];
    int64_t s_in[6], s_out[6];
    double alpha, beta;
    const double* in; double* out;
};
void permute(const Permute& p, stream_t s);

void mp2_amplitudes(double* t, const double* w, const double* eo, const double* ev, double shift,
                    int no, int nv, stream_t s);
void cc_update(double* t, double* dt, const double* r, const double* eo, const double* ev, double shift,
               double delta, int no, int nv, int rank, stream_t s);
void dots(int npairs, const double* const* x, const double* const* y, const int64_t* n, double* out_host,
          stream_t s);
void energy_norms(const double* f, const double* t1, const double* t2, const double* Edir, const double* Eex,
                  const double* dt2, int no, int nv, double out_host[6], stream_t s);
int energy_norms_start(const double* f, const double* t1, const double* t2, const double* Edir, const double* Eex,
                       const double* dt2, int no, int nv, stream_t s);
int readback_start(const double* dev_ptr, int n, stream_t s);
void readback_wait(int slot, double* out_host, int n);
void energy_norms_pairs(const double* f, const double* t1, const double* tc, const double* Edir, const double* Eex,
                        const double* dtc, int no, int nv, int64_t r0, int64_t r1, bool with_t1, double out_host[6],
                        stream_t s);
void energy_norms_pairs_dev(const double* f, const double* t1, const double* tc, const double* Edir, const double* Eex,
                            const double* dtc, int no, int nv, int64_t r0, int64_t r1, bool with_t1, double* out_dev,
                            stream_t s);
void exchange_asymmetry(const double* A, const double* B, const int64_t d[4], double out_host[2], stream_t s);
void cc_update_to(double* t_out, double* dt, const double* t_in, const double* r, const double* eo, const double* ev,
                  double shift, double delta, int no, int nv, int rank, stream_t s);
void lincomb(double* out, int nx, const double* const* x, const double* c, int64_t n, stream_t s);
bool sym_tail_ok();
void cc_update_to_sym(double* t_out, double* dt, const double* t_in, const double* r, const double* eo, const double* ev,
                      double shift, double delta, int no, int nv, stream_t s);
void lincomb_sym(double* out, int nx, const double* const* x, const double* c, int no, int nv, stream_t s);
void dots_sym(int npairs, const double* const* x, const double* const* y, const int64_t* n, const int* sym, int no, int nv,
              double* out_host, stream_t s);
int energy_norms_start_sym(const double* f, const double* t1, const double* t2, const double* Edir, const double* Eex,
                           const double* dt2, int no, int nv, stream_t s);
void t2_layouts_sym(const double* T, double* Td, double* Tx, double* Ttd, int no, int nv, stream_t s);
void gram(int m, int n, const double* const* x, const double* const* y, int64_t len, double* out_host, stream_t s);
void lincomb_multi(int m, int n, const double* const* x, const double* c, const double* beta, double* const* y, int64_t len,
                   stream_t s);
void diis_step(double* state, int npairs, const double* const* x, const double* const* y, const int64_t* n, int ntypes, int m,
               int was_full, stream_t s);
void lincomb_dev(double* out, int nx, const double* const* x, const double* coeff_dev, int64_t n, stream_t s);
void cmul(const double* mr, const double* mi, const double* xr, const double* xi, double* yr, double* yi, int64_t n, stream_t s);
void exchange_split(const double* u, double* us, double* w, double* dg, int no, int nv, stream_t s);
void sgn_ij_add(double* D, const double* R, int no, int nv, stream_t s);
void cshift_inv(const double* d, double zr, double zi, double hr, double hi, double shift, double* mr, double* mi, int64_t n,
                stream_t s);
int64_t eom_diag_ws_doubles(int no, int nv);
void eom_diagonals(const double* V, const double* T, const double* dai, const double* iaai, const double* iaia, const double* ijij,
                   const double* abab, double* d1, double* d2, int no, int nv, double* ws, stream_t s);
void tau_build(double* tau, const double* t2, const double* t1, int no, int nv, stream_t s);

void ladder_pack_V(const double* V, double* Vp, double* Vm, int nr, int nc, int64_t rp0, int64_t rp1, stream_t s,
                   int64_t ldvp = 0, int64_t ldvm = 0);
void ladder_pack_V_factors(const double* B, double* Vp, double* Vm, int naux, int n, int no, int64_t rp0, int64_t rp1,
                           stream_t s, int64_t ldvp, int64_t ldvm);
int64_t triples_partial_doubles(int nv, int64_t nt);
void triples_energy(const double* W, int64_t nt, int64_t t0, const double* Vijab, const double* t1, const double* eps,
                    double* partial, double* out, int no, int nv, stream_t s);
void lambda_triples_energy(const double* WR, const double* WL, int64_t nt, int64_t t0, const double* Vijab, const double* l1,
                           const double* eps, double* partial, double* out, int no, int nv, stream_t s);
int64_t fno_density_partial_doubles(int noa, int nv);
void fno_density(const double* Vijab, const double* eps_o, const double* eps_v, int no, int nf, int nv, double* partial,
                 double* D, double* e, stream_t s);
bool ladder_dress_ok(int no, int nv);
int64_t ladder_dress_ws_doubles(int no, int nv);
void ladder_dress(const double* V, const double* Pk, const double* t1, double* W, int no, int nv, int64_t ld, int64_t row0,
                  int64_t row1, double sgn, double* ws, stream_t s);
enum { PACK_ROW_HALF = 1, PACK_AM_PROWS = 2, PACK_COL_HALF = 4, PACK_AM_PCOLS = 8 };
void ladder_pack_T(const double* X, const double* t1, double* Sp, double* Am, int nc, int nr, int flags, int64_t ldp,
                   int64_t ldm, stream_t s, int64_t rp0 = 0, int64_t rp1 = -1);
void ladder_unpack(const double* L, double* R, double beta, int no, int nv, stream_t s);
bool fused_pair_kernels_ok(int no);
void t2_layouts(const double* T, double* Td, double* Tx, double* Ttd, int no, int nv, stream_t s, double ca = 2.0,
                double cb = -1.0);
void residual_assemble(const double* V, const double* L, const double* N, const double* D, const double* X, double* R,
                       int no, int nv, stream_t s, double xd = 0.0);
void pairs_pack(const double* full, double* Xc, int no, int nv, int64_t r0, int64_t r1, stream_t s);
void pairs_unpack(const double* Xc, double* full, int no, int nv, int64_t r0, int64_t r1, stream_t s);
void cc_update_pairs(double* tc, double* dtc, const double* rc, const double* eo, const double* ev, double shift,
                     double delta, int no, int nv, int64_t r0, int64_t r1, stream_t s);
void residual_assemble_pairs(const double* V, const double* L, const double* Np, const double* D, const double* X,
                             double* Rc, int no, int nv, int64_t r0, int64_t r1, int a0, int nbp, stream_t s, double xd = 0.0);
void rows_unpack(const double* Q, double* out, int64_t rows, int no, stream_t s);
void ring_operands(const double* Viabj, const double* Viajb, double* M, double* N1, double a1, double a2, int no, int nv,
                   stream_t s);
void pair_traces(const double* M, int64_t ld, double alpha, double beta, double* out_vv, double* out_oo, int no, int nv,
                 stream_t s, const double* M2 = nullptr, double alpha2 = 0.0);

void ipea_pack(int k, const double* const* r1, const double* const* r2, int P, int S, int n1, double* U1, double* R, double* Rx,
               double* Rt, double* Rn, stream_t s);
void ipea_assemble(int k, const double* D, const double* E, const double* L, const double* S1, int P, int S, int n1,
                   double* const* s1, double* const* s2, stream_t s);
void ipea_unpack(int k, const double* dU1, const double* dR, const double* dRx, const double* dRt, const double* dRn, int P, int S,
                 int n1, double* const* o1, double* const* o2, stream_t s);
struct DysonParts {
    const double* t1 = nullptr; const double* lam1 = nullptr; const double* Yoo = nullptr; const double* Yvv = nullptr;
    const double* L1 = nullptr; const double* R1 = nullptr; const double* A = nullptr; const double* B = nullptr;
    const double* C = nullptr;
    double* psiL = nullptr; double* psiR = nullptr;
};
void ipea_dyson_assemble(const DysonParts& q, int k, int kind, int no, int nv, stream_t s);
void ipea_diagonals(const double* Loo, const double* Lvv, int kind, int no, int nv, double* d1, double* d2, stream_t s);
int64_t ipea_correction_ws_doubles(int n, int64_t len);
void ipea_correction(int n, const double* const* sv, const double* const* rv, const double* w_host, const double* d, double shift,
                     double* const* q, int64_t n1, int64_t off2, int64_t len, double* ws, double* out_dev, stream_t s);

struct LambdaParts {
    const double* D = nullptr; const double* Pd = nullptr; const double* Px = nullptr; const double* Lp = nullptr;
    const double* La = nullptr; const double* S1 = nullptr;
    double cd = 1.0, cx = 0.0;
    const double* Vijab = nullptr; const double* eta1 = nullptr; const double* eo = nullptr; const double* ev = nullptr;
    double shift = 0.0, err_scale = 1.0;
    const double* lam1 = nullptr; const double* lam2 = nullptr;
    double* out1 = nullptr; double* out2 = nullptr; double* err1 = nullptr; double* err2 = nullptr;
    double* ws = nullptr; double* norm_dev = nullptr;
    int64_t lp_ld = 0, la_ld = 0;
};
int64_t lambda_assemble_ws_doubles(int nv);
void lambda_assemble(const LambdaParts& q, int no, int nv, stream_t s);
bool lambda_assemble_ok(int no);
void rdm1_assemble(const double* Xvv, const double* Xoo, const double* Xov, const double* l1, const double* t1, int no, int nv,
                   double ref, double* g, stream_t s);
struct Tdm1Parts {
    const double* t1 = nullptr; const double* lam1 = nullptr; const double* L1 = nullptr; const double* R1 = nullptr;
    const double* Xvv = nullptr; const double* Xoo = nullptr; const double* Xov = nullptr;
    const double* Yvv = nullptr; const double* Yoo = nullptr; const double* Yov = nullptr;
    const double* Zvv = nullptr; const double* Zoo = nullptr; const double* Zov = nullptr;
    const double* Le = nullptr; const double* Eov = nullptr;
    double* gl = nullptr; double* gr = nullptr; double* r0 = nullptr;
};
void tdm1_assemble(const Tdm1Parts& q, int k, int no, int nv, stream_t s);

void hf_fock(const double* const dir[4], const double* const exc[4], const double* h_dev, double* f_dev, int no, int nv,
             stream_t s);

int64_t fcidump_fill(double* V, const double* val_host, const int32_t* pqrs_host, int64_t count, int n, bool is_tc,
                     stream_t s);

void scatter(double* dst, const int64_t* idx_host, const double* val_host, int64_t n, stream_t s);
void tc_single_contraction(const double* L, double* D, int nb, int no, stream_t s);
// ... 19 lines not shown
```

### pymes_amd/csrc/engine.cpp

```cpp
#include "engine.h"

#include <algorithm>
#include <cstdio>
#include <cstdlib>
#include <cstring>
#include <tuple>

namespace pymes {

TView make_view(double* p, int rank, const int64_t* dims, const int64_t* strides) {
    if (rank < 0 || rank > 6) throw Error("tensor rank must be 0..6");
    TView t;
    t.p = p;
    t.rank = rank;
    int64_t s = 1;
    for (int i = rank - 1; i >= 0; --i) {
        t.dim[i] = dims[i];
        t.st[i] = strides ? strides[i] : s;
        s *= dims[i];
    }
    return t;
}
TView make_view(double* p, std::initializer_list<int64_t> dims) {
    int64_t d[6];
// ... 52 lines not shown
    if (top_ + bytes > cap_)
        throw Error("workspace exhausted: need " + std::to_string((top_ + bytes) >> 20) + " MiB, have " +
                    std::to_string(cap_ >> 20) + " MiB (pass a larger workspace_bytes to pymes_ctx_create)");
    double* p = reinterpret_cast<double*>(base_ + top_);
    top_ += bytes;
    high_ = std::max(high_, top_);
    return p;
}

int pattern_of_name(const char* name) {
    if (!name || std::strlen(name) != 4) throw Error("block name must have 4 letters");
    int pat = 0;
    for (int i = 0; i < 4; ++i) {
        const char c = name[i];
        if (c >= 'a' && c <= 'd') pat |= 1 << (3 - i);
        else if (!(c >= 'i' && c <= 'l')) throw Error(std::string("bad block name: ") + name);
    }
    return pat;
}
std::string canonical_name(int pattern) {
    static const char* names[16] = {"klij", "ijka", "ijak", "ijab", "iajk", "iajb", "iabj", "iabc",
                                    "aijk", "aijb", "aibj", "aibc", "abij", "abic", "abci", "abcd"};
    return names[pattern & 15];
}

Engine::Engine(int device_, int no_, int nv_, size_t workspace_bytes) : device(device_), no(no_), nv(nv_), n(no_ + nv_) {
    if (no < 1 || nv < 1) throw Error("need at least one occupied and one virtual orbital");
    dev::set_device(device);
    own_stream_ = dev::stream_create();
    stream = own_stream_;
    if (workspace_bytes == 0) {
        const double o = no, v = nv;
        double bytes = 8.0 * (24.0 * o * o * v * v + 2.0 * o * v * v * v + 4.0 * (o + v) * (o + v) * o * o) +
                       (64 << 20);
        workspace_bytes = static_cast<size_t>(bytes);
    }
    arena.init(workspace_bytes);
    splitk_doubles_ = 32 << 20;
    splitk_ws_ = static_cast<double*>(dev::dmalloc(sizeof(double) * splitk_doubles_));
    eps_o = static_cast<double*>(dev::dmalloc(sizeof(double) * no));
    eps_v = static_cast<double*>(dev::dmalloc(sizeof(double) * nv));
}

Engine::~Engine() {
    try {
        dev::set_device(device);
        if (capturing_) dev::graph_abort(stream);
        dev::stream_sync(stream);
        for (auto g : graphs_) dev::graph_destroy(g);
        for (void* p : user_allocs_) dev::dfree(p);
        for (auto& kv : scratch_free_) dev::dfree(kv.second);
        for (auto& kv : scratch_live_) dev::dfree(kv.first);
        for (auto& p : lay_) dev::dfree(p);
        dev::dfree(xs_oo_);
        dev::dfree(xs_vv_);
        for (auto& p : V_) dev::dfree(p);
        for (auto& p : Vd_) dev::dfree(p);
        for (auto& kv : static_) dev::dfree(kv.second);
        dev::dfree(splitk_ws_);
        dev::dfree(lpack_.Vp);
        dev::dfree(lpack_.Vm);
        dev::dfree(srows_.Vp);
        dev::dfree(srows_.Vm);
        dev::dfree(eps_o);
        dev::dfree(eps_v);
        arena.release();
        dev::stream_destroy(own_stream_);
    } catch (...) {
    }
}


double* Engine::scratch_get(int64_t doubles) {
    doubles = std::max<int64_t>(doubles, 1);
    auto it = scratch_free_.find(doubles);
    double* p;
    if (it != scratch_free_.end()) {
        p = it->second;
        scratch_free_.erase(it);
    } else {
        p = static_cast<double*>(dev::try_dmalloc(sizeof(double) * static_cast<size_t>(doubles)));
        if (!p) {
            scratch_trim();
            try {
                p = static_cast<double*>(dev::dmalloc(sizeof(double) * static_cast<size_t>(doubles)));
            } catch (const std::exception&) {
                throw Error("out of device memory (" + std::to_string((doubles * 8) >> 20) + " MiB of scratch)");
            }
        }
    }
    scratch_live_[p] = doubles;
    return p;
}
void Engine::scratch_put(double* p) {
    auto it = scratch_live_.find(p);
    if (it == scratch_live_.end()) return;
    scratch_free_.emplace(it->second, p);
    scratch_live_.erase(it);
}
void Engine::scratch_trim() {
    if (scratch_free_.empty()) return;
    dev::stream_sync(stream);
    for (auto& kv : scratch_free_) dev::dfree(kv.second);
    scratch_free_.clear();
}
int64_t Engine::scratch_free_bytes() const {
// ... 577 lines not shown
                                     double*, double*, stream_t) {
    throw std::runtime_error("ipea_pack: not available in this backend");
}
__attribute__((weak)) void ipea_assemble(int, const double*, const double*, const double*, const double*, int, int, int,
                                         double* const*, double* const*, stream_t) {
    throw std::runtime_error("ipea_assemble: not available in this backend");
}
__attribute__((weak)) void ipea_unpack(int, const double*, const double*, const double*, const double*, const double*, int, int, int,
                                       double* const*, double* const*, stream_t) {
    throw std::runtime_error("ipea_unpack: not available in this backend");
}
__attribute__((weak)) void ipea_dyson_assemble(const DysonParts&, int, int, int, int, stream_t) {
    throw std::runtime_error("ipea_dyson_assemble: not available in this backend");
}
__attribute__((weak)) void ipea_diagonals(const double*, const double*, int, int, int, double*, double*, stream_t) {
    throw std::runtime_error("ipea_diagonals: not available in this backend");
}
__attribute__((weak)) int64_t ipea_correction_ws_doubles(int, int64_t) { return 1; }
__attribute__((weak)) void ipea_correction(int, const double* const*, const double* const*, const double*, const double*, double,
                                           double* const*, int64_t, int64_t, int64_t, double*, double*, stream_t) {
    throw std::runtime_error("ipea_correction: not available in this backend");
}
__attribute__((weak)) int64_t lambda_assemble_ws_doubles(int) { return 1; }
__attribute__((weak)) bool lambda_assemble_ok(int) { return true; }
__attribute__((weak)) void lambda_assemble(const LambdaParts&, int, int, stream_t) {
    throw std::runtime_error("lambda_assemble: not available in this backend");
}
__attribute__((weak)) void rdm1_assemble(const double*, const double*, const double*, const double*, const double*, int, int,
                                         double, double*, stream_t) {
    throw std::runtime_error("rdm1_assemble: not available in this backend");
}
__attribute__((weak)) void tdm1_assemble(const Tdm1Parts&, int, int, int, stream_t) {
    throw std::runtime_error("tdm1_assemble: not available in this backend");
}
__attribute__((weak)) bool sym_tail_ok() { return false; }
__attribute__((weak)) void cc_update_to_sym(double*, double*, const double*, const double*, const double*, const double*, double,
                                            double, int, int, stream_t) {
    throw std::runtime_error("cc_update_to_sym: not available in this backend");
}
__attribute__((weak)) void lincomb_sym(double*, int, const double* const*, const double*, int, int, stream_t) {
    throw std::runtime_error("lincomb_sym: not available in this backend");
}
__attribute__((weak)) void dots_sym(int, const double* const*, const double* const*, const int64_t*, const int*, int, int, double*,
                                    stream_t) {
    throw std::runtime_error("dots_sym: not available in this backend");
}
__attribute__((weak)) int energy_norms_start_sym(const double*, const double*, const double*, const double*, const double*,
                                                 const double*, int, int, stream_t) {
    throw std::runtime_error("energy_norms_start_sym: not available in this backend");
}
__attribute__((weak)) void t2_layouts_sym(const double*, double*, double*, double*, int, int, stream_t) {
    throw std::runtime_error("t2_layouts_sym: not available in this backend");
}
}
```

### pymes_amd/csrc/engine.h

```cpp
#pragma once
#include <algorithm>
#include <cstdint>
#include <functional>
#include <map>
#include <set>
#include <stdexcept>
#include <string>
#include <vector>

#include "device_api.h"

namespace pymes {

struct TView {
    double* p = nullptr;
    int rank = 0;
    int64_t dim[6] = {1, 1, 1, 1, 1, 1};
    int64_t st[6] = {0, 0, 0, 0, 0, 0};
    int64_t size() const {
        int64_t n = 1;
        for (int i = 0; i < rank; ++i) n *= dim[i];
        return n;
    }
};
// ... 71 lines not shown
std::string canonical_name(int pattern);

class Engine {
  public:
    Engine(int device, int no, int nv, size_t workspace_bytes);
    ~Engine();

    int device;
    int no, nv, n;
    dev::stream_t stream = nullptr;
    Arena arena;
    ContractStats stats;

    void set_stream(dev::stream_t s) { stream = s; }
    void* user_malloc(size_t bytes);
    void user_free(void* p);
    double* scratch_get(int64_t doubles);
    void scratch_put(double* p);
    void scratch_trim();
    int64_t scratch_free_bytes() const;
    void graph_begin();
    dev::graph_t graph_end();
    void graph_abort();
    void graph_launch(dev::graph_t g);
    void graph_destroy(dev::graph_t g);
    bool capturing() const { return capturing_; }
    uint64_t dress_generation() const { return dress_generation_; }
    void exchange_asymmetry_V(double out[2]);

    void contract(double alpha, const TView& A, const char* sa, const TView& B, const char* sb, double beta,
                  const TView& C, const char* sc, const char* batch = "", const TView* Cin = nullptr);
    void permute(double alpha, const TView& in, const char* si, double beta, const TView& out, const char* so);
    void axpby(double alpha, const TView& in, double beta, const TView& out);
    void copy(const TView& in, const TView& out) { axpby(1.0, in, 0.0, out); }
    void zero(const TView& t);

    void set_V_full(const double* V, bool on_device, const int64_t strides[4]);
    void set_V_block(const char* name, const double* data, bool on_device, const int64_t strides[4]);
    void set_V_from_factors(const double* B_host, int naux);
    void set_integral_shard(int rank, int world);
    bool integral_shard() const { return shard_on_; }
    void refuse_if_sharded(const char* who) const;
    void shard_rows(const double** vp, const double** vm, int64_t* row0, int64_t* row1, int64_t* ldp, int64_t* ldm) const;
    int64_t integral_bytes() const;
    TView block(int pattern, bool dressed = false);
    double* ensure_block(int pattern);
    bool has_block(int pattern, bool dressed = false) const;
    void set_orbital_energies(const double* eo_host, const double* ev_host);

    void mp2(double shift, double* t2, double e_out[2]);
    void hf_fock_matrix(const double* h_host, double* f_host);
    void dress_fock(const double* f, const double* t1, double* fd);
    int64_t dress_fock_ws_doubles() const;
    void dress_fock_partial(const double* t1, double* W, int rank, int world);
    void dress_fock_finish(const double* f, const double* t1, const double* W, double* fd);
    void xvv_partial(const double* f, const double* t2, double* Xvv, int rank, int world, unsigned flags);
    void dress_V(const double* t1, uint32_t mask, const int64_t* cut = nullptr);
    void singles_residual(const double* fd, const double* t1, const double* t2, double* r1);
    void singles_residual_partial(const double* fd, const double* t1, const double* t2, double* r1, int rank, int world,
                                  bool reuse_layouts = false);
    void doubles_residual(const double* f, const double* t2, double* r2, unsigned flags);
    void ladder(const double* t2, double* r2, int a0, int a1, bool dressed, double beta);
    void ladder_sym(const double* t2, double* L, int64_t row0, int64_t row1, bool dressed, int hole = 0);
    void ladder_sym_multi(const double* const* xs, int k, double* L_all, bool dressed);
    void ladder_sym_adjoint(const double* x, double* LS, double* LA, bool dressed);
    void ladder_sym_adjoint_multi(const double* const* xs, int k, double* LS, double* LA, bool dressed);
    PairDims pair_dims() const { return PairDims(no, nv); }
    int64_t ladder_adjoint_pitch(bool symmetric_half) const { return pair_dims().adjoint_pitch(symmetric_half); }
    void hole_ladder_packed_multi(const double* const* xs, const double* const* Is, const double* const* ys, int k, double* L_all);
    void hole_ladder_packed(const double* x, const double* I, double* L, int64_t row0, int64_t row1,
                            const double* y = nullptr);
    void ladder_sym_unpack(const double* L, double* r2, double beta);
    void residual_slab(const double* f, const double* t2, double* ETd, double* ETx, double* L, int rank, int world,
                       unsigned flags, const double* t1 = nullptr, double* QK = nullptr, const double* P = nullptr);
    int64_t slab_prepare_ws_doubles() const;
    void slab_prepare(const double* t2, double* P, int rank, int world, unsigned flags);
    void residual_finish(const double* f, const double* t2, const double* ETd, const double* ETx, const double* L,
                         double* r2, unsigned flags, const double* t1 = nullptr, const double* QK = nullptr);
    void residual_finish_pairs(const double* f, const double* t2, const double* ETd, const double* ETx, const double* L,
                               double* Rc, unsigned flags, const double* t1, const double* QK, int rank, int world,
                               const double* Xvv_in = nullptr);
    void pair_chunk(int rank, int world, int64_t& r0, int64_t& r1) const;
    void amplitude_side_abij(const double* t1, const double* QK, const TView& N, int64_t a0, int64_t a1, int64_t b1,
                             bool with_partner, double beta = 1.0);
    void ladder_t1(const double* t1, const double* t2, double* L, int64_t row0, int64_t row1, double* QK, int64_t q0,
                   int64_t q1, bool dcd, const double* J = nullptr);
    void dress_abcd_rows(const double* t1, int a0, int a1, bool lower_only);
    static constexpr unsigned kT1Zero = 1u << 20;
    static constexpr unsigned kSymTail = 1u << 22;
    bool sym_tail() const;
    void ccsd_residuals(const double* f, const double* t1, const double* t2, unsigned flags, double* r1, double* r2);
    void ccsd_iterate(const double* f, double* t1, double* t2, unsigned flags, double shift, double delta, double* dt1,
                      double* dt2, double out[6]);
    void release_residual_buffers();
    void cc_update(double* t, double* dt, const double* r, double shift, double delta, int rank);
    void cc_update_to(double* t_out, double* dt, const double* t_in, const double* r, double shift, double delta, int rank,
                      bool sym = false);
    void dots(int npairs, const double* const* x, const double* const* y, const int64_t* n, const int* sym, double* out);
    void lincomb(double* out, int nx, const double* const* x, const double* c, int64_t n, bool sym);
    void ccsd_energy(const double* f, const double* t1, const double* t2, double out[3]);
    void ccd_energy(const double* t2, double out[2]);
    void energy_norms(const double* f, const double* t1, const double* t2, const double* dt2, double out[6], bool sym = false);
    int energy_norms_start(const double* f, const double* t1, const double* t2, const double* dt2, bool sym = false);
    void energy_norms_wait(int slot, double out[6]);
    void energy_norms_pairs(const double* f, const double* t1, const double* tc, const double* dtc, int rank, int world,
                            double out[6]);
    struct Collectives {
        void* user = nullptr;
        int rank = 0, world = 1;
        int (*allreduce_start)(void* user, double* buf, int64_t n, void* stream, int64_t* ticket) = nullptr;
        int (*allgather_start)(void* user, double* buf, int64_t chunk, void* stream, int64_t* ticket) = nullptr;
        int (*wait)(void* user, int64_t ticket, void* stream) = nullptr;
        void (*mark)(void* user, const char* phase) = nullptr;
    };
    struct ShardBuffers {
        double *ETd, *ETx, *L, *QK, *Tall, *W, *Xvv, *P, *R1, *S;
    };
    void set_collectives(const Collectives* c);
    bool has_collectives() const { return coll_set_; }
    typedef int (*alltoallv_fn)(void* user, const double* send, const int64_t* send_counts, double* recv,
                                const int64_t* recv_counts, void* stream, int64_t* ticket);
    void set_alltoallv(alltoallv_fn fn) { alltoallv_ = fn; }
    void set_owner_tile_buffers(double* send, double* recv) { xs_ = send; xr_ = recv; }
    void owner_tile_sizes(int rank, int world, int64_t* send_doubles, int64_t* recv_doubles) const;
    static constexpr unsigned kOwnerTiles = 1u << 21;
    void ccsd_sharded_residuals(const double* f, double* fd, const double* t1, double* t2, const ShardBuffers& b,
                                unsigned flags, double* rc);
    void ccd_sharded_residuals(const double* f, double* t2, const ShardBuffers& b, unsigned flags, double* rc);
    int ccsd_sharded_finish(const double* f, const double* t1, const double* tc, const double* dtc, const ShardBuffers& b);
    void ccsd_sharded_energy(int slot, double out[6]);
    void ccsd_sharded_await(double* t2, const ShardBuffers& b);
    static int64_t triples_count(int no);
    double ccsd_t(const double* eps_host, const double* t1, const double* t2, int64_t t_begin, int64_t t_end, double* per_triple);
    double ccsd_t_lambda(const double* eps_host, const double* t2, const double* lam1, const double* lam2, int64_t t_begin,
                         int64_t t_end, double* per_triple);
    void check_hermitian(const char* who, const char* why);
    double fno_density(const double* Vijab, int n_frozen, double* D_host);
    void derive_from(Engine& src, int n_frozen, const double* C_host, int nv_dst);
    void invalidate_static();

    double* eps_o = nullptr;
    double* eps_v = nullptr;
    bool eps_set = false;
    void need_eps(const char* who) const;
    double* splitk_ws() const { return splitk_ws_; }
    int64_t splitk_ws_doubles() const { return splitk_doubles_; }

  private:
    double* lay_[3] = {nullptr, nullptr, nullptr};
    const double* lay_t2_ = nullptr;
    void pair_layouts_of(const double* t2, bool want_td, bool sym = false);
    struct FoldTag {
        const double* t2 = nullptr;
        const double* etd = nullptr;
        bool is(const double* t, const double* e) const { return t2 && t2 == t && etd == e; }
        void set(const double* t, const double* e) { t2 = t; etd = e; }
        void clear() { t2 = etd = nullptr; }
    } ring_fold_;
    static bool ring_fold_enabled();
    struct SumTag {
        const double* t2 = nullptr;
        int rank = 0, world = 0;
        bool is(const double* p, int r, int w) const { return t2 && t2 == p && rank == r && world == w; }
        void set(const double* p, int r, int w) { t2 = p; rank = r; world = w; }
        void clear() { t2 = nullptr; }
    };
    double ring_xd_ = 0.0;
    double* xs_oo_ = nullptr;
    double* xs_vv_ = nullptr;
    SumTag xs_oo_tag_, xs_vv_tag_;
    void ensure_xs();
    dev::stream_t own_stream_ = nullptr;
    std::set<void*> user_allocs_;
    Collectives coll_;
    alltoallv_fn alltoallv_ = nullptr;
    double *xs_ = nullptr, *xr_ = nullptr;
    struct Rect { int64_t r0, r1, c0, c1; };
    std::vector<Rect> owner_tile_rects(int from, int to, int world) const;
    int64_t owner_tiles_start(const ShardBuffers& b);
    void owner_tiles_finish(const ShardBuffers& b);
    bool coll_set_ = false, t2_in_flight_ = false;
    int64_t t2_ticket_ = 0;
    double *res_fd_ = nullptr, *res_ETd_ = nullptr, *res_ETx_ = nullptr, *res_L_ = nullptr, *res_QK_ = nullptr, *res_r1_ = nullptr,
           *res_r2_ = nullptr;
    std::multimap<int64_t, double*> scratch_free_;
    std::map<double*, int64_t> scratch_live_;
    std::set<dev::graph_t> graphs_;
    std::set<dev::graph_t> graphs_dressing_;
    bool release_wanted_ = false;
    bool capturing_ = false;
    uint64_t dress_generation_ = 0, capture_generation_ = 0;
    double* V_[16] = {nullptr};
    double* Vd_[16] = {nullptr};
    std::map<std::string, double*> static_;
    std::map<std::string, int64_t> static_doubles_;
    double* new_static(const std::string& key, int64_t doubles);
    bool shard_on_ = false;
    int shard_rank_ = 0, shard_world_ = 1;
    struct ShardRows {
        double* Vp = nullptr;
        double* Vm = nullptr;
        int64_t row0 = 0, row1 = 0;
        bool set = false;
    } srows_;
    void shard_rows_alloc();
    void set_V_full_sharded(const double* V, bool on_device, const int64_t strides[4]);
    void shard_rows_from(const double* V0, const int64_t st[4], bool on_device);
    void shard_rows_from_factors(const double* Bd, int naux);
    void check_shard_rows(const char* who, int64_t row0, int64_t row1, bool dressed) const;
    void check_shard_rank(const char* who, int rank, int world) const;
    struct LadderPack {
        double* Vp = nullptr;
        double* Vm = nullptr;
        int64_t row0 = 0, row1 = 0;
        bool dressed = false, valid = false;
    } lpack_;
    bool ensure_ladder_pack(int64_t row0, int64_t row1, bool dressed);
    struct PackedV {
        double* Vp;
        double* Vm;
        bool packed;
    };
    PackedV ladder_rows(const char* who, int64_t row0, int64_t row1, bool dressed);
    PackedV ijab_pack();
    struct HoleOperand {
        double* Ip;
        double* Im;
    };
    void hole_operand_pack(const double* I, const HoleOperand& h);
    HoleOperand hole_operand(const double* I);
    void hole_operand_add(const HoleOperand& h, const double* Sp, const double* Am, double beta, bool grouped = false);
    void hole_ladder_rows(const double* x, const double* I, double* L, int64_t row0, int64_t row1, const double* y,
                          const double* ySp = nullptr, const double* yAm = nullptr);
    struct RingSlab {
        const double* t2;
        const double* ETd_p;
        bool quad, traces, fold;
        int64_t c0, c1;
        TView F, Viajb, Viabj, Tx, Ttd, ETd, ETx;
        std::function<void(double, const TView&, const char*, const TView&)> load_cols, load_rows;
    };
    void slab_ladders(const double* t2, double* L, int rank, int world, unsigned flags, const double* t1, double* QK,
                      const double* P);
    void slab_rings_rows(const RingSlab& s);
    void slab_rings_cols(const RingSlab& s);
    bool bra_dress_pays() const;
    bool dress_off_ = false;
    double* splitk_ws_ = nullptr;
    int64_t splitk_doubles_ = 0;
    double* get_static(const std::string& key);
    std::map<long, TView> dress_memo_;
    void dressed_into(int pattern, const std::vector<int>& pos, int k, const TView& t1v, const TView& dst,
                      bool reduced = false, const int64_t* cut = nullptr);
    int64_t block_size(int pattern) const;
    TView block_view(double* p, int pattern) const;
    double* ensure_dressed(int pattern);
};

}
```

### pymes_amd/csrc/kernels.hip

```cpp
#include <hip/hip_runtime.h>
#include <type_traits>

#include <algorithm>
#include <atomic>
#include <chrono>
#include <cmath>
#include <cstdio>
#include <cstdlib>
#include <cstring>
#include <mutex>
#include <stdexcept>
#include <string>
#include <vector>

#include "../../include/pymes_amd.h"
#include "device_api.h"
#include "diis_small.h"
#include "device_util.h"
#include "launch.h"

namespace {

constexpr int kThreads = 256;
constexpr int BK = 16;
// ... 2156 lines not shown
    double* out;
    LinPtrs p;
    int nx, no, nv;
};
__global__ void __launch_bounds__(256) lincomb_sym_kernel(const LinSymK k) {
    double* out = k.out;
    const int nx = k.nx, no = k.no, nv = k.nv;
    extern __shared__ double tile[];
    int a, b;
    unrank_pair(blockIdx.x, a, b);
    const int p = no + 1, o2 = no * no;
    const long ab = ((long)a * nv + b) * o2, ba = ((long)b * nv + a) * o2;
    for (int e = threadIdx.x; e < o2; e += blockDim.x) {
        const int i = e / no, j = e - i * no;
        double s = 0.0;
        for (int q = 0; q < nx; ++q) s += k.p.x[q][ab + e] * k.p.c[q];
        out[ab + e] = s;
        tile[i * p + j] = s;
    }
    if (a == b) return;
    __syncthreads();
    for (int e = threadIdx.x; e < o2; e += blockDim.x) {
        const int j = e / no, i = e - j * no;
        out[ba + e] = tile[i * p + j];
    }
}

__global__ void __launch_bounds__(256) t2_layouts_sym_kernel(const LayoutsK k) {
    const double* __restrict__ T = k.T;
    double* __restrict__ Td = k.Td;
    double* __restrict__ Tx = k.Tx;
    double* __restrict__ Ttd = k.Ttd;
    const int no = k.no, nv = k.nv;
    extern __shared__ double tile[];
    const int a = blockIdx.x / nv, b = blockIdx.x - a * nv;
    const int p = no + 1, o2 = no * no;
    const long ov = (long)no * nv;
    const double* __restrict__ Tab = T + ((long)a * nv + b) * o2;
    const long base = (long)a * no * ov + (long)b * no;
    for (int e = threadIdx.x; e < o2; e += blockDim.x) {
        const int i = e / no, j = e - i * no;
        const double x = Tab[e];
        tile[i * p + j] = x;
        if (Td) Td[base + (long)i * ov + j] = x;
    }
    __syncthreads();
    for (int e = threadIdx.x; e < o2; e += blockDim.x) {
        const int i = e / no, j = e - i * no;
        Ttd[base + (long)i * ov + j] = 2.0 * tile[i * p + j] - tile[j * p + i];
    }
    for (int e = threadIdx.x; e < o2; e += blockDim.x) {
        const int j = e / no, i = e - j * no;
        Tx[base + (long)j * ov + i] = tile[i * p + j];
    }
}

struct DotsSymK {
    DotsK d;
    unsigned symmask;
    int o2, nv;
};
template <int VEC, int SVEC>
__global__ void __launch_bounds__(256) dots_stage1_sym_kernel(const DotsSymK k) {
    __shared__ double sh[4];
    const int nb = k.d.nb, npairs = k.d.npairs;
    const int lin = blockIdx.x;
    int pair, b;
    if ((nb & 7) == 0) { const int q = lin >> 3; pair = q % npairs; b = (q / npairs) * 8 + (lin & 7); }
    else { pair = lin / nb; b = lin - pair * nb; }
    if (!((k.symmask >> pair) & 1u)) {
        dots_stage1_body<VEC>(k.d, blockIdx.x, sh);
        return;
    }
    const double* __restrict__ x = k.d.p.x[pair];
    const double* __restrict__ y = k.d.p.y[pair];
    const int o2 = k.o2, nv = k.nv;
    const long npp = (long)nv * (nv + 1) / 2;
    double off = 0.0, dia = 0.0;
    for (long t = b; t < npp; t += nb) {
        int va, vb;
        unrank_pair(t, va, vb);
        const long base = ((long)va * nv + vb) * o2;
        double s = 0.0;
        if (SVEC == 2) {
            const double2* __restrict__ x2 = reinterpret_cast<const double2*>(x + base);
            const double2* __restrict__ y2 = reinterpret_cast<const double2*>(y + base);
            double s1 = 0.0;
#pragma unroll 4
            for (int i = threadIdx.x; i < (o2 >> 1); i += 256) {
                const double2 u = x2[i], w = y2[i];
                s += u.x * w.x;
                s1 += u.y * w.y;
            }
            s += s1;
        } else {
#pragma unroll 4
            for (int i = threadIdx.x; i < o2; i += 256) s += x[base + i] * y[base + i];
        }
        if (va == vb) dia += s;
        else off += s;
    }
    const double r_off = block_sum(off, sh), r_dia = block_sum(dia, sh);
    if (threadIdx.x == 0) k.d.partial[pair * kDotBlocks + b] = 2.0 * r_off + r_dia;
}

template <int VEC>
// ... 427 lines not shown
        double acc[4] = {0.0, 0.0, 0.0, 0.0};
#pragma unroll
        for (int u = 0; u < 4; ++u) {
            const int a = a0 + 4 * u;
            if (a < nv)
                for (int k = lane; k < no; k += 64) {
                    const long e = (long)k * ld + (long)a * no + k;
                    double v = alpha * base[e];
                    if (base2) v += alpha2 * base2[e];
                    acc[u] += v;
                }
        }
#pragma unroll
        for (int u = 0; u < 4; ++u) {
#pragma unroll
            for (int off = 32; off > 0; off >>= 1) acc[u] += __shfl_down(acc[u], off, 64);
            const int a = a0 + 4 * u;
            if (lane == 0 && a < nv) {
                double* o = out_vv + (long)a * nv + c;
                *o = (beta == 0.0 ? 0.0 : beta * *o) + acc[u];
            }
        }
        return;
    }
    double (*part)[64] = reinterpret_cast<double (*)[64]>(smem);
    const int k = vb - nvv;
    for (int i0 = 0; i0 < no; i0 += 64) {
        const int i = i0 + lane;
        double acc = 0.0;
        if (i < no) {
#pragma unroll 4
            for (int c = wave; c < nv; c += 4) {
                const long e = ((long)c * no + k) * ld + (long)c * no + i;
                double v = alpha * M[e];
                if (M2) v += alpha2 * M2[e];
                acc += v;
            }
        }
        part[wave][lane] = acc;
        __syncthreads();
        if (wave == 0 && i < no) {
            const double sum = ((part[0][lane] + part[1][lane]) + part[2][lane]) + part[3][lane];
            double* o = out_oo + (long)k * no + i;
            *o = (beta == 0.0 ? 0.0 : beta * *o) + sum;
        }
        __syncthreads();
    }
}
__global__ void __launch_bounds__(256) pair_traces_kernel(const TracesK q) {
    __shared__ double part[kTracesLdsDoubles];
    pair_traces_body(q, blockIdx.x, part);
}

enum : unsigned short {
    PK_GEMM = 0, PK_SPLITK, PK_PERM_DIRECT, PK_PERM_TILED, PK_GEMV_COLS, PK_GEMV_FINISH, PK_GEMV_ROWS, PK_CC_UPDATE, PK_LINCOMB,
    PK_DOTS1, PK_DOTS2, PK_ENERGY, PK_TAU, PK_PACK_T, PK_LADDER_UNPACK, PK_RING_OPERANDS, PK_T2_LAYOUTS, PK_ASSEMBLE,
    PK_ROWS_UNPACK, PK_FOCK_G12, PK_FOCK_G12_FIN, PK_FOCK_FT, PK_FOCK_FIN, PK_TRACES, PK_DOTS_FINAL, PK_KINDS
};
constexpr const char* kPhaseKindNames[] = {"gemm", "splitk", "perm", "permT", "gemvC", "gemvF", "gemvR", "update", "lincomb", "dots1", "dots2",
                                           "energy", "tau", "packT", "unpackL", "ringops", "layouts", "assemble", "unpackR", "fockG", "fockGf",
                                           "fockFt", "fockFin", "traces", "dotsF"};
static_assert(sizeof(kPhaseKindNames) / sizeof(kPhaseKindNames[0]) == PK_KINDS, "one name per phase kind");
struct SplitkTaskK { GemmK g; int BM, BN; };
struct PermTaskK { PermK p; long total; int tiles_q, tiles_l; };
struct GemvTaskK { GemvItem it; double* ws; const double* yin; double beta; };

constexpr int kPhaseMaxTasks = 24;
constexpr int kPhaseBlobWords = 440;
struct PhaseK {
    int n;
    int blk_end[kPhaseMaxTasks];
    int nblk[kPhaseMaxTasks];
    unsigned short kind[kPhaseMaxTasks], sub[kPhaseMaxTasks], off[kPhaseMaxTasks];
    long blob[kPhaseBlobWords];
};
static_assert(sizeof(PhaseK) <= 4096, "kernel arguments are limited to 4 KB");

template <typename T>
__device__ __forceinline__ const T& phase_args(const long* args) { return *reinterpret_cast<const T*>(args); }
template <int BM, int BN>
__device__ __forceinline__ void phase_gemm_layouts(const GemmK& g, const int lay, const long bid) {
    switch (lay) {
        case 0: dgemm_body<BM, BN, false, false, 1>(g, bid); break;
        case 1: dgemm_body<BM, BN, false, false, 2>(g, bid); break;
        case 2: dgemm_body<BM, BN, false, true, 1>(g, bid); break;
        case 3: dgemm_body<BM, BN, false, true, 2>(g, bid); break;
        case 4: dgemm_body<BM, BN, true, false, 1>(g, bid); break;
        case 5: dgemm_body<BM, BN, true, false, 2>(g, bid); break;
        case 6: dgemm_body<BM, BN, true, true, 1>(g, bid); break;
        default: dgemm_body<BM, BN, true, true, 2>(g, bid); break;
    }
}
template <bool HEAVY>
__device__ __forceinline__ void phase_body(const PhaseK& ph) {
    extern __shared__ __attribute__((aligned(16))) double smem[];
    __shared__ double sh[4];
    const int b = blockIdx.x;
    int it = 0;
    while (it + 1 < ph.n && b >= ph.blk_end[it]) ++it;
    const int start = it ? ph.blk_end[it - 1] : 0;
    const int span = ph.blk_end[it] - start;
    const int nblk = ph.nblk[it];
    const int kind = ph.kind[it], sub = ph.sub[it];
    const long* const args = ph.blob + ph.off[it];
    int vb = b - start;
    if (kind == PK_GEMM) vb = (int)xcd_remap(vb, span);
    if (vb >= nblk) return;
    switch (kind) {
        case PK_GEMM:
            if constexpr (HEAVY) {
                const GemmK& g = phase_args<GemmK>(args);
                const int shape = sub >> 3, lay = sub & 7;
                if (shape == 0) phase_gemm_layouts<64, 64>(g, lay, vb);
                else if (shape == 1) phase_gemm_layouts<64, 32>(g, lay, vb);
// ... 13 lines not shown
            const PermTaskK& k = phase_args<PermTaskK>(args);
            permute_tiled_body(k.p, k.tiles_q, k.tiles_l, vb, smem);
        } break;
        case PK_GEMV_COLS: {
            const GemvTaskK& k = phase_args<GemvTaskK>(args);
            gemv_cols_item(k.it, vb, k.ws);
        } break;
        case PK_GEMV_FINISH: {
            const GemvTaskK& k = phase_args<GemvTaskK>(args);
            gemv_finish_item(k.it, vb, k.ws, k.beta, k.yin);
        } break;
        case PK_GEMV_ROWS:
            if (sub) gemv_rows_body<2>(phase_args<GemvRowsK>(args), vb);
            else gemv_rows_body<1>(phase_args<GemvRowsK>(args), vb);
            break;
        case PK_CC_UPDATE: cc_update_body(phase_args<CcUpdateK>(args), vb, nblk); break;
        case PK_LINCOMB: lincomb_body(phase_args<LinK>(args), vb, nblk); break;
        case PK_DOTS1:
            if (sub) dots_stage1_body<2>(phase_args<DotsK>(args), vb, sh);
            else dots_stage1_body<1>(phase_args<DotsK>(args), vb, sh);
            break;
        case PK_DOTS2: dots_stage2_body(phase_args<Dots2K>(args), vb, sh); break;
        case PK_DOTS_FINAL: dots_final_body(phase_args<DotsFinalK>(args), vb, sh); break;
        case PK_ENERGY:
            if constexpr (HEAVY) {
                if (sub) energy_norms_body<2>(phase_args<EnergyK>(args), vb, nblk, sh);
                else energy_norms_body<1>(phase_args<EnergyK>(args), vb, nblk, sh);
            }
            break;
        case PK_TAU: tau_body(phase_args<TauK>(args), vb, nblk); break;
        case PK_PACK_T: ladder_pack_T_body(phase_args<PackTK>(args), vb); break;
        case PK_LADDER_UNPACK: ladder_unpack_body(phase_args<UnpackK>(args), vb, nblk); break;
        case PK_RING_OPERANDS: ring_operands_body(phase_args<RingOpK>(args), vb); break;
        case PK_T2_LAYOUTS:
            if (sub) t2_layouts_body<true>(phase_args<LayoutsK>(args), vb);
            else t2_layouts_body<false>(phase_args<LayoutsK>(args), vb);
            break;
        case PK_ASSEMBLE: residual_assemble_body(phase_args<AssembleK>(args), vb); break;
        case PK_ROWS_UNPACK: rows_unpack_body(phase_args<RowsUnpackK>(args), vb, nblk); break;
        case PK_FOCK_G12:
            if constexpr (HEAVY) {
                if (sub) fock_g12_body<2>(phase_args<FockG12K>(args), vb);
                else fock_g12_body<1>(phase_args<FockG12K>(args), vb);
            }
            break;
        case PK_FOCK_G12_FIN: fock_g12_finish_body(phase_args<FockG12FinK>(args), vb); break;
        case PK_FOCK_FT:
            if constexpr (HEAVY) fock_ft_body(phase_args<FockFinK>(args), vb);
            break;
        case PK_FOCK_FIN:
            if constexpr (HEAVY) fock_finish_body(phase_args<FockFinK>(args), vb);
            break;
        case PK_TRACES: pair_traces_body(phase_args<TracesK>(args), vb, smem); break;
        default: break;
    }
}
__global__ void __launch_bounds__(kThreads, 2) phase_kernel(const PhaseK ph) { phase_body<true>(ph); }
__global__ void __launch_bounds__(kThreads, 8) phase_light_kernel(const PhaseK ph) { phase_body<false>(ph); }
__host__ __device__ constexpr bool phase_kind_heavy(int kind) {
    return kind == PK_GEMM || kind == PK_ENERGY || kind == PK_FOCK_G12 || kind == PK_FOCK_FT || kind == PK_FOCK_FIN;
}

struct Prof {
    bool on = false;
    std::vector<std::pair<hipEvent_t, hipEvent_t>> ev;
    std::vector<std::pair<hipEvent_t, hipEvent_t>> pool;
    std::vector<std::string> what;
    std::vector<double> fl;
    std::vector<int> klass;
    std::vector<int> nk;
    double flops = 0.0;
};
thread_local Prof g_prof;

double* g_dot_ws[kMaxDevices] = {nullptr};
double* g_dot_host[kMaxDevices] = {nullptr};
constexpr int kGramTiles = 64;
double* g_gram_ws[kMaxDevices] = {nullptr};
double* g_gram_host[kMaxDevices] = {nullptr};
std::atomic<long> g_live_allocs{0};

struct PhaseRange { uintptr_t lo, hi; uintptr_t pitch = 0, width = 0; };
inline PhaseRange prange(const void* p, long doubles) {
    const uintptr_t lo = reinterpret_cast<uintptr_t>(p);
    return PhaseRange{lo, p && doubles > 0 ? lo + 8 * (uintptr_t)doubles : lo};
}
inline PhaseRange pbox(const void* base, std::initializer_list<std::pair<long, long>> dims, long slack = 0) {
    long lo = 0, hi = 0;
    for (const auto& d : dims) {
        if (d.first <= 0) return PhaseRange{0, 0};
        const long span = (d.first - 1) * d.second;
        if (span < 0) lo += span; else hi += span;
    }
    const uintptr_t b = reinterpret_cast<uintptr_t>(base);
    PhaseRange r{b + 8 * lo, b + 8 * (hi + 1 + slack)};
    long w = 0, pch = 0;
    int nd = 0;
    for (const auto& d : dims)
        if (d.first > 1) {
            ++nd;
            if (d.second == 1) w = d.first;
            else pch = d.second;
        }
    if (nd == 2 && w > 0 && pch > w + slack) { r.pitch = 8 * (uintptr_t)pch; r.width = 8 * (uintptr_t)(w + slack); }
    return r;
}
// ... 1755 lines not shown

constexpr size_t kPairTileBudget = 64 * 1024;
constexpr size_t pair_tile_bytes(size_t no) { return no * (no + 1) * sizeof(double); }
static_assert(pair_tile_bytes(PYMES_NOCC_MAX_FUSED) <= kPairTileBudget && pair_tile_bytes(PYMES_NOCC_MAX_FUSED + 1) > kPairTileBudget,
              "PYMES_NOCC_MAX_FUSED is the largest nocc whose tile fits the budget");
bool fused_pair_kernels_ok(int no) { return no <= PYMES_NOCC_MAX_FUSED; }

void ring_operands(const double* Viabj, const double* Viajb, double* M, double* N1, double a1, double a2, int no, int nv,
                   stream_t s) {
    if (no < 1 || nv < 1) return;
    const size_t lds = sizeof(double) * (size_t)no * 33;
    if (lds > 64 * 1024) throw std::runtime_error("ring_operands: nocc too large for the LDS tile");
    const RingOpK k{Viabj, Viajb, M, N1, a1, a2, no, nv};
    const long ov2 = (long)no * nv * no * nv;
    const double cost = 32.0 * (double)ov2 / 4.0e6;
    if (phase_open((hipStream_t)s) && phase_small(cost)) {
        PhaseRec& t = phase_push(PK_RING_OPERANDS, 0, (long)no * nv, (int)lds, cost, k);
        phase_reads(t, {prange(Viabj, ov2), prange(Viajb, ov2)});
        phase_writes(t, {prange(M, ov2), prange(N1, ov2)});
        return;
    }
    launch_kernel(ring_operands_kernel, dim3((unsigned)((long)no * nv)), dim3(256), lds, (hipStream_t)s, k);
}

void t2_layouts(const double* T, double* Td, double* Tx, double* Ttd, int no, int nv, stream_t s, double ca, double cb) {
    if (!fused_pair_kernels_ok(no)) throw std::runtime_error("t2_layouts: nocc too large for the LDS tile");
    const size_t lds = sizeof(double) * no * (no + 1);
    const LayoutsK k{T, Td, Tx, Ttd, ca, cb, no, nv};
    const bool res = ca == 2.0 && cb == -1.0;
    const long n4 = (long)nv * nv * no * no;
    const double cost = 40.0 * (double)n4 / 4.0e6;
    if (phase_open((hipStream_t)s) && phase_small(cost)) {
        PhaseRec& t = phase_push(PK_T2_LAYOUTS, res ? 1 : 0, (long)nv * nv, (int)lds, cost, k);
        phase_reads(t, {prange(T, n4)});
        phase_writes(t, {prange(Td, Td ? n4 : 0), prange(Tx, n4), prange(Ttd, n4)});
        return;
    }
    if (res) launch_kernel(t2_layouts_kernel<true>, dim3((unsigned)(nv * nv)), dim3(256), lds, (hipStream_t)s, k);
    else launch_kernel(t2_layouts_kernel<false>, dim3((unsigned)(nv * nv)), dim3(256), lds, (hipStream_t)s, k);
}
void t2_layouts_sym(const double* T, double* Td, double* Tx, double* Ttd, int no, int nv, stream_t s) {
    if (!fused_pair_kernels_ok(no)) throw std::runtime_error("t2_layouts: nocc too large for the LDS tile");
    const long n4 = (long)nv * nv * no * no;
    phase_open((hipStream_t)s);
    if (phase_small(40.0 * (double)n4 / 4.0e6)) {
        t2_layouts(T, Td, Tx, Ttd, no, nv, s);
        return;
    }
    if (!n4) return;
    const LayoutsK k{T, Td, Tx, Ttd, 2.0, -1.0, no, nv};
    launch_kernel(t2_layouts_sym_kernel, dim3((unsigned)(nv * nv)), dim3(256), sizeof(double) * no * (no + 1), (hipStream_t)s, k);
}

void residual_assemble(const double* V, const double* L, const double* N, const double* D, const double* X, double* R,
                       int no, int nv, stream_t s, double xd) {
    if (!fused_pair_kernels_ok(no)) throw std::runtime_error("residual_assemble: nocc too large for the LDS tile");
    const size_t lds = sizeof(double) * no * (no + 1);
    const AssembleK k{V, L, N, D, X, R, xd, no, nv};
    const long n4 = (long)nv * nv * no * no;
    const double cost = 48.0 * (double)n4 / 4.0e6;
    if (phase_open((hipStream_t)s) && phase_small(cost)) {
        PhaseRec& t = phase_push(PK_ASSEMBLE, 0, (long)nv * (nv + 1) / 2, (int)lds, cost, k);
        phase_reads(t, {prange(V, V ? n4 : 0), prange(L, L ? (long)nv * (nv + 1) / 2 * no * no : 0), prange(N, n4), prange(D, n4), prange(X, n4)});
        phase_writes(t, {prange(R, n4)});
        return;
    }
    launch_kernel(residual_assemble_kernel, dim3((unsigned)((long)nv * (nv + 1) / 2)), dim3(256), lds, (hipStream_t)s, k);
}

void pairs_pack(const double* full, double* Xc, int no, int nv, int64_t r0, int64_t r1, stream_t s) {
    if (r1 <= r0) return;
    launch_kernel(pairs_pack_kernel, dim3((unsigned)(r1 - r0)), dim3(256), 0, (hipStream_t)s, full, Xc, no, nv, (long)r0);
}
void energy_norms_pairs(const double* f, const double* t1, const double* tc, const double* Edir, const double* Eex,
                        const double* dtc, int no, int nv, int64_t r0, int64_t r1, bool with_t1, double out_host[6],
                        stream_t s) {
    hipStream_t st = (hipStream_t)s;
    const int dv = current_device();
    ensure_dot_ws(dv);
    const long npairs = std::max<long>(0, (long)(r1 - r0));
    const int nb = (int)std::max<long>(1, std::min<long>(kDotBlocks, 2 * npairs));
    launch_kernel(energy_norms_pairs_kernel, dim3(nb), dim3(256), 0, st, f, t1, tc, Edir, Eex, dtc, no, nv, (long)r0,
                       npairs, with_t1 ? 1 : 0, g_dot_ws[dv]);
    double* out_dev = g_dot_ws[dv] + 16 * kDotBlocks;
    launch_kernel(dots_stage2_kernel, dim3(6), dim3(256), 0, st, g_dot_ws[dv], nb, out_dev);
    HIP_CHECK(copy_async(g_dot_host[dv], out_dev, sizeof(double) * 6, hipMemcpyDeviceToHost, st));
    wait_idle(st);
    for (int i = 0; i < 6; ++i) out_host[i] = g_dot_host[dv][i];
}
void energy_norms_pairs_dev(const double* f, const double* t1, const double* tc, const double* Edir, const double* Eex,
                            const double* dtc, int no, int nv, int64_t r0, int64_t r1, bool with_t1, double* out_dev,
                            stream_t s) {
    hipStream_t st = (hipStream_t)s;
    const int dv = current_device();
    ensure_dot_ws(dv);
    const long npairs = std::max<long>(0, (long)(r1 - r0));
    const int nb = (int)std::max<long>(1, std::min<long>(kDotBlocks, 2 * npairs));
    launch_kernel(energy_norms_pairs_kernel, dim3(nb), dim3(256), 0, st, f, t1, tc, Edir, Eex, dtc, no, nv, (long)r0,
                       npairs, with_t1 ? 1 : 0, g_dot_ws[dv]);
    launch_kernel(dots_stage2_kernel, dim3(6), dim3(256), 0, st, g_dot_ws[dv], nb, out_dev);
}
void pairs_unpack(const double* Xc, double* full, int no, int nv, int64_t r0, int64_t r1, stream_t s) {
    if (r1 <= r0) return;
    launch_kernel(pairs_unpack_kernel, dim3((unsigned)(r1 - r0)), dim3(256), 0, (hipStream_t)s, Xc, full, no, nv, (long)r0);
}
void cc_update_pairs(double* tc, double* dtc, const double* rc, const double* eo, const double* ev, double shift,
// ... 44 lines not shown
    const size_t lds = sizeof(double) * 6 * (size_t)nv;
    const dim3 grid((unsigned)(na * used)), block(256);
    const bool vec2 = !(nv & 1) && !(reinterpret_cast<uintptr_t>(V) & 15);
    if (!vec2 && nv > 512) throw std::runtime_error("fock_g12: unaligned block with nvirt above 512");
    const long av = (long)na * nv;
    const FockG12K k{V, t1, ws, no, nv, na, j0, j1, jper};
    const FockG12FinK kf{ws, G1, G2, av, used};
    const double cost = 8.0 * (double)nj * (double)av * (double)nv / 4.0e6;
    if (phase_open(st) && phase_small(cost)) {
        PhaseRec& t = phase_push(PK_FOCK_G12, vec2 ? 1 : 0, (long)na * used, (int)lds, cost, k);
        phase_reads(t, {prange(V + (long)j0 * av * nv, (long)nj * av * nv), prange(t1, (long)no * nv)});
        phase_writes(t, {prange(ws, (long)used * 2 * av)});
        PhaseRec& u = phase_push(PK_FOCK_G12_FIN, 0, (av + 255) / 256, 0, 1.0, kf);
        phase_reads(u, {prange(ws, (long)used * 2 * av)});
        phase_writes(u, {prange(G1, av), prange(G2, av)});
        return;
    }
    if (vec2) launch_kernel(fock_g12_kernel<2>, grid, block, lds, st, k);
    else launch_kernel(fock_g12_kernel<1>, grid, block, lds, st, k);
    launch_kernel(fock_g12_finish_kernel, dim3((unsigned)((av + 255) / 256)), dim3(256), 0, st, kf);
}

void fock_finish(const double* f, const double* t1, const double* W, double* fd, double* ft, int no, int nv, stream_t s) {
    const long n = no + nv;
    const FockFinK k{f, t1, W, ft, fd, no, nv};
    if (phase_open((hipStream_t)s)) {
        const long wlen = 2L * nv * nv + 4L * no * nv + 2L * no * no;
        PhaseRec& t = phase_push(PK_FOCK_FT, 0, (no * no + 3) / 4, 0, 2.0, k);
        phase_reads(t, {prange(f, n * n), prange(t1, (long)no * nv), prange(W, wlen)});
        phase_writes(t, {prange(ft, (long)no * no)});
        PhaseRec& u = phase_push(PK_FOCK_FIN, 0, (n * n + 3) / 4, 0, 3.0, k);
        phase_reads(u, {prange(f, n * n), prange(t1, (long)no * nv), prange(W, wlen), prange(ft, (long)no * no)});
        phase_writes(u, {prange(fd, n * n)});
        return;
    }
    launch_kernel(fock_ft_kernel, dim3((unsigned)((no * no + 3) / 4)), dim3(256), 0, (hipStream_t)s, k);
    launch_kernel(fock_finish_kernel, dim3((unsigned)((n * n + 3) / 4)), dim3(256), 0, (hipStream_t)s, k);
}

void pair_traces(const double* M, int64_t ld, double alpha, double beta, double* out_vv, double* out_oo, int no, int nv,
                 stream_t s, const double* M2, double alpha2) {
    if (no <= 0 || nv <= 0) return;
    const unsigned blocks = (unsigned)nv * (unsigned)((nv + 15) / 16) + (unsigned)no;
    const TracesK k{M, M2, out_vv, out_oo, (long)ld, alpha, beta, alpha2, no, nv};
    const long ov = (long)no * nv;
    const double cost = 128.0 / 3.0 * (double)ov * (double)ov / 8.0 / 4.0e6 * (M2 ? 2.0 : 1.0) + 3.0;
    if (phase_open((hipStream_t)s) && phase_small(cost)) {
        PhaseRec& t = phase_push(PK_TRACES, 0, blocks, kTracesLdsDoubles * (int)sizeof(double), cost, k);
        phase_reads(t, {pbox(M, {{ov, ld}, {ov, 1}}), M2 ? pbox(M2, {{ov, ld}, {ov, 1}}) : PhaseRange{0, 0}});
        phase_writes(t, {prange(out_vv, (long)nv * nv), prange(out_oo, (long)no * no)});
        return;
    }
    launch_kernel(pair_traces_kernel, dim3(blocks), dim3(256), 0, (hipStream_t)s, k);
}

}

namespace {

bool gemv_dispatch(const GemmProduct& p, hipStream_t st) {
    const dev::Gemm& g = p.g;
    if (g.nb1 != 1 || g.nb2 != 1 || g.K < 256) return false;
    GemvItem it;
    bool cols;
    if (g.M == 1 && g.N >= 64) {
        it.x = g.A; it.xs = p.a_sk; it.W = g.B; it.ys = 1;
        if (p.b_sn == 1) { cols = true; it.R = g.K; it.C = g.N; it.ld = p.b_sk; }
        else { cols = false; it.R = g.N; it.C = g.K; it.ld = p.b_sn; }
    } else if (g.N == 1 && g.M >= 64) {
        it.x = g.B; it.xs = p.b_sk; it.W = g.A; it.ys = g.ldc;
        if (p.a_sk == 1) { cols = false; it.R = g.M; it.C = g.K; it.ld = p.a_sm; }
        else { cols = true; it.R = g.K; it.C = g.M; it.ld = p.a_sk; }
    } else {
        return false;
    }
    const long R = it.R, C = it.C;
    if (!cols && R < 512) return false;
    const double* yin = g.Cin ? g.Cin : g.C;
    const int vec = (even(it.ld) && even(C) && aligned16(it.W)) ? 2 : 1;
    const long cblocks = (C + 256L * vec - 1) / (256L * vec);
    long nchunk = 1;
    it.rchunk = R;
    if (cols) {
        if (!g.splitk_ws || C > g.splitk_ws_doubles) return false;
        nchunk = std::max<long>(1, std::min<long>((2048 + cblocks - 1) / cblocks, R / 32));
        nchunk = std::min<long>(nchunk, g.splitk_ws_doubles / C);
        it.rchunk = (R + nchunk - 1) / nchunk;
        nchunk = (R + it.rchunk - 1) / it.rchunk;
    }
    it.y = g.C; it.ws_off = 0; it.alpha = g.alpha; it.nchunk = (int)nchunk; it.cblocks = (int)cblocks; it.vec = vec;
    it.blk0 = it.out0 = 0;
    const GemvRowsK rk{it.W, it.x, yin, g.C, it.ld, it.xs, R, C, it.ys, g.alpha, g.beta};
    if (phase_open(st)) {
        const double cost = 8.0 * (double)R * (double)C / 4.0e6;
        if (phase_small(cost)) {
            const PhaseRange rW = pbox(it.W, {{R, it.ld}, {C, 1}}, 1);
            if (cols) {
                double* part = phase_ws(g.splitk_ws, g.splitk_ws_doubles, nchunk * C);
                if (part) {
                    const GemvTaskK t{it, part, yin, g.beta};
                    const PhaseRange rP = prange(part, nchunk * C);
                    PhaseRec& a = phase_push(PK_GEMV_COLS, 0, cblocks * nchunk, 0, cost, t);
                    phase_reads(a, {rW, pbox(it.x, {{R, it.xs}})});
                    phase_writes(a, {rP});
                    PhaseRec& f = phase_push(PK_GEMV_FINISH, 0, (C + 255) / 256, 0, 1.0, t);
                    phase_reads(f, {rP, g.beta != 0.0 ? pbox(yin, {{C, it.ys}}) : PhaseRange{0, 0}});
// ... 51 lines not shown
```

### pymes_amd/device.py

```python
import ctypes as C
import weakref

import numpy as np

from . import _lib
from ._lib import PymesError, i64_array, ptr_array

BLOCK_NAMES = ("abci", "iabj", "iajk", "aijk", "klij", "aibj", "ijak", "abic",
               "iajb", "abcd", "iabc", "aijb", "ijka", "aibc", "ijab", "abij")


def pattern_of(name):
    return sum((1 << (3 - p)) for p, ch in enumerate(name) if ch in "abcd")


class DeviceArray:

    def __init__(self, ctx, ptr, shape, owned=True, keepalive=None):
        self.ctx, self.ptr, self.shape = ctx, int(ptr), tuple(int(s) for s in shape)
        self._owned, self._keep = owned, keepalive
        self.size = int(np.prod(self.shape)) if self.shape else 1

    @property
    def nbytes(self):
# ... 285 lines not shown

    def set_orbital_energies(self, eps_o, eps_v):
        eo = np.ascontiguousarray(eps_o, dtype=np.float64)
        ev = np.ascontiguousarray(eps_v, dtype=np.float64)
        assert eo.shape == (self.no,) and ev.shape == (self.nv,)
        self.lib.call("pymes_set_orbital_energies", self.handle, _lib.host_ptr(eo), _lib.host_ptr(ev))

    def phase_enable(self, mode):
        self.lib.call("pymes_phase_enable", int(mode))

    def phase_hold(self):
        import contextlib

        @contextlib.contextmanager
        def hold():
            self.lib.call("pymes_phase_hold", 1)
            try:
                yield
            finally:
                self.lib.call("pymes_phase_hold", 0)
        return hold()

    def phase_stats(self):
        v = [C.c_int64() for _ in range(4)]
        self.lib.call("pymes_phase_stats", *[C.byref(x) for x in v])
        return dict(zip(("tasks", "launches", "levels", "flushes"), (int(x.value) for x in v)))

    @property
    def dress_generation(self):
        n = C.c_uint64()
        self.lib.call("pymes_dress_generation", self.handle, C.byref(n))
        return int(n.value)

    def mp2(self, t2, level_shift=0.0):
        e = (C.c_double * 2)()
        self.lib.call("pymes_mp2", self.handle, float(level_shift), C.c_void_p(t2.ptr), e)
        return e[0], e[1]

    def dress_fock(self, f, t1, out):
        self.lib.call("pymes_ccsd_dress_fock", self.handle, C.c_void_p(f.ptr), C.c_void_p(t1.ptr), C.c_void_p(out.ptr))
        return out

    def dress_V(self, t1, names, reduced_abij=False, q_range=None, p_range=None):
        mask = _lib.PYMES_DRESS_ABIJ_REDUCED if reduced_abij else 0
        for nm in names:
            mask |= 1 << pattern_of(nm)
        if q_range is not None or p_range is not None:
            p0, p1 = p_range if p_range is not None else (0, 0)
            q0, q1 = q_range if q_range is not None else (0, 0)
            self.lib.call("pymes_ccsd_dress_V_slab", self.handle, C.c_void_p(t1.ptr), mask, int(p0), int(p1), int(q0), int(q1))
        else:
            self.lib.call("pymes_ccsd_dress_V", self.handle, C.c_void_p(t1.ptr), mask)

    def ccsd_residuals(self, f, t1, t2, r1, r2, is_dcd=False, t1_zero=False, sym_tail=False):
        self.lib.call("pymes_ccsd_residuals", self.handle, C.c_void_p(f.ptr), C.c_void_p(t1.ptr), C.c_void_p(t2.ptr),
                      (_lib.PYMES_DCD if is_dcd else 0) | (_lib.PYMES_T1_ZERO if t1_zero else 0) |
                      (_lib.PYMES_SYM_TAIL if sym_tail else 0), C.c_void_p(r1.ptr), C.c_void_p(r2.ptr))

    def sym_tail(self):
        yes = C.c_int()
        self.lib.call("pymes_sym_tail", self.handle, C.byref(yes))
        return bool(yes.value)

    def ccsd_iterate(self, f, t1, t2, dt1, dt2, level_shift=0.0, delta=1.0, is_dcd=False, t1_zero=False):
        out = (C.c_double * 6)()
        self.lib.call("pymes_ccsd_iterate", self.handle, C.c_void_p(f.ptr), C.c_void_p(t1.ptr), C.c_void_p(t2.ptr),
                      (_lib.PYMES_DCD if is_dcd else 0) | (_lib.PYMES_T1_ZERO if t1_zero else 0), float(level_shift), float(delta),
                      C.c_void_p(dt1.ptr), C.c_void_p(dt2.ptr), out)
        return tuple(out)

    def ccsd_release(self):
        self.lib.call("pymes_ccsd_release", self.handle)

    def singles_residual(self, fd, t1, t2, out):
        self.lib.call("pymes_ccsd_singles_residual", self.handle, C.c_void_p(fd.ptr), C.c_void_p(t1.ptr),
                      C.c_void_p(t2.ptr), C.c_void_p(out.ptr))
        return out

    def singles_residual_partial(self, fd, t1, t2, out, rank, world, reuse_layouts=False):
        self.lib.call("pymes_ccsd_singles_residual_partial", self.handle, C.c_void_p(fd.ptr), C.c_void_p(t1.ptr),
                      C.c_void_p(t2.ptr), C.c_void_p(out.ptr), int(rank), int(world),
                      _lib.PYMES_REUSE_LAYOUTS if reuse_layouts else 0)
        return out

    def doubles_residual(self, f, t2, out, is_dcd=False, dressed=False, skip_ladder=False, sym_ladder=False,
                         sym_rings=None, sym_tail=False):
        sym_rings = sym_ladder if sym_rings is None else sym_rings
        flags = (_lib.PYMES_DCD if is_dcd else 0) | (_lib.PYMES_USE_DRESSED if dressed else 0) | \
                (_lib.PYMES_SKIP_LADDER if skip_ladder else 0) | (_lib.PYMES_SYM_LADDER if sym_ladder else 0) | \
                (_lib.PYMES_SYM_RINGS if sym_rings else 0) | (_lib.PYMES_SYM_TAIL if sym_tail and sym_rings else 0)
        self.lib.call("pymes_doubles_residual", self.handle, C.c_void_p(f.ptr), C.c_void_p(t2.ptr),
                      C.c_void_p(out.ptr), flags)
        return out

    def ladder(self, t2, out, a_begin, a_end, dressed=False, beta=0.0):
        self.lib.call("pymes_ladder", self.handle, C.c_void_p(t2.ptr), C.c_void_p(out.ptr), int(a_begin), int(a_end),
                      int(dressed), float(beta))
        return out

    @staticmethod
    def _flags(is_dcd, dressed, skip_ladder=False, sym_ladder=False, sym_rings=False):
        return (_lib.PYMES_DCD if is_dcd else 0) | (_lib.PYMES_USE_DRESSED if dressed else 0) | \
               (_lib.PYMES_SKIP_LADDER if skip_ladder else 0) | (_lib.PYMES_SYM_LADDER if sym_ladder else 0) | \
               (_lib.PYMES_SYM_RINGS if sym_rings else 0)

    def residual_slab(self, f, t2, ETd, ETx, L, rank, world, is_dcd=False, dressed=False, t1=None, QK=None, P=None,
# ... 346 lines not shown
```

Baseline: 0.1595.

## Fuse t2 layout and ladder pack fan-out; derive Fock sums from dress_V traces

A single symmetric fan-out kernel now produces the pair layouts (Xx, Xt) and the three ladder packs from t2 in one pass over pair blocks. The ladder and ring code reuse these persistent buffers instead of running separate ladder_pack_T and layout permutes. In addition, dress_V computes partial diagonal traces of the dressed blocks, so the Fock dressing can skip its G1/G2/J contractions. This trades extra persistent device memory and more complex state tracking (fan_t2_/fan_t1_ guards) for fewer full passes over the o^2v^2 amplitudes.

```diff
diff --git a/include/pymes_amd.h b/include/pymes_amd.h
--- a/include/pymes_amd.h
+++ b/include/pymes_amd.h
@@ -83,6 +83,8 @@
 int pymes_ccsd_dress_V(pymes_ctx* ctx, const double* t1_dev, uint32_t block_mask);
 int pymes_ccsd_dress_V_slab(pymes_ctx* ctx, const double* t1_dev, uint32_t block_mask, int p_begin, int p_end,
                             int q_begin, int q_end);
+int pymes_ccsd_dress_V_fock_sums(pymes_ctx* ctx, const double* t1_dev, uint32_t block_mask, double* sums_dev);
+int pymes_fock_traces(pymes_ctx* ctx, int* yes, uint64_t* reads);
 int pymes_ccsd_singles_residual(pymes_ctx* ctx, const double* fd_dev, const double* t1_dev, const double* t2_dev,
                                 double* r1_dev);
 int pymes_ccsd_singles_residual_partial(pymes_ctx* ctx, const double* fd_dev, const double* t1_dev, const double* t2_dev,
@@ -219,6 +221,9 @@
                       int64_t n);
 #define PYMES_SYM_TAIL (1u << 22)
 int pymes_sym_tail(pymes_ctx* ctx, int* yes);
+int pymes_t2_fanout_info(pymes_ctx* ctx, int* yes, uint64_t* fanouts, int64_t* pack_doubles);
+int pymes_t2_fanout(pymes_ctx* ctx, const double* t2_dev, const double* t1_dev, double* Xx_dev, double* Xt_dev,
+                    double* const* packs_dev, int separate);
 int pymes_cc_update_to_sym(pymes_ctx* ctx, double* t_out_dev, double* dt_dev, const double* t_in_dev, const double* r_dev,
                            double level_shift, double delta);
 int pymes_dots_sym(pymes_ctx* ctx, int npairs, const double* const* x_dev, const double* const* y_dev, const int64_t* n,
diff --git a/pymes_amd/_lib.py b/pymes_amd/_lib.py
--- a/pymes_amd/_lib.py
+++ b/pymes_amd/_lib.py
@@ -184,6 +184,10 @@
     "pymes_lincomb_multi": (C.c_int, [C.c_void_p, C.c_int, C.c_int, c_pp, C.c_void_p, C.c_void_p, c_pp, C.c_int64]),
     "pymes_lincomb_dev": (C.c_int, [C.c_void_p, C.c_void_p, C.c_int, c_pp, C.c_void_p, C.c_int64]),
     "pymes_sym_tail": (C.c_int, [C.c_void_p, C.POINTER(C.c_int)]),
+    "pymes_t2_fanout_info": (C.c_int, [C.c_void_p, C.POINTER(C.c_int), C.POINTER(C.c_uint64), c_i64_p]),
+    "pymes_t2_fanout": (C.c_int, [C.c_void_p, C.c_void_p, C.c_void_p, C.c_void_p, C.c_void_p, c_pp, C.c_int]),
+    "pymes_ccsd_dress_V_fock_sums": (C.c_int, [C.c_void_p, C.c_void_p, C.c_uint32, C.c_void_p]),
+    "pymes_fock_traces": (C.c_int, [C.c_void_p, C.POINTER(C.c_int), C.POINTER(C.c_uint64)]),
     "pymes_cc_update_to_sym": (C.c_int, [C.c_void_p, C.c_void_p, C.c_void_p, C.c_void_p, C.c_void_p, C.c_double, C.c_double]),
     "pymes_dots_sym": (C.c_int, [C.c_void_p, C.c_int, c_pp, c_pp, c_i64_p, C.POINTER(C.c_int), c_double_p]),
     "pymes_lincomb_sym": (C.c_int, [C.c_void_p, C.c_void_p, C.c_int, c_pp, c_double_p, C.c_int64]),
diff --git a/pymes_amd/csrc/capi.cpp b/pymes_amd/csrc/capi.cpp
--- a/pymes_amd/csrc/capi.cpp
+++ b/pymes_amd/csrc/capi.cpp
@@ -444,6 +444,19 @@
         E(ctx).dress_V(t1, mask);
     });
 }
+int pymes_ccsd_dress_V_fock_sums(pymes_ctx* ctx, const double* t1, uint32_t mask, double* sums) {
+    return guarded([&] {
+        need(t1, "t1"); need(sums, "sums");
+        E(ctx).dress_V(t1, mask, nullptr, sums);
+    });
+}
+int pymes_fock_traces(pymes_ctx* ctx, int* yes, uint64_t* reads) {
+    return guarded([&] {
+        need(yes, "yes");
+        *yes = Eq(ctx).fock_traces_ok() ? 1 : 0;
+        if (reads) *reads = Eq(ctx).fock_trace_reads();
+    });
+}
 int pymes_ccsd_dress_V_slab(pymes_ctx* ctx, const double* t1, uint32_t mask, int p_begin, int p_end, int q_begin,
                             int q_end) {
     return guarded([&] {
@@ -677,6 +690,25 @@
     return guarded([&] {
         need(yes, "yes");
         *yes = Eq(ctx).sym_tail() ? 1 : 0;
+    });
+}
+int pymes_t2_fanout_info(pymes_ctx* ctx, int* yes, uint64_t* fanouts, int64_t* pack_doubles) {
+    return guarded([&] {
+        need(yes, "yes");
+        Engine& e = Eq(ctx);
+        *yes = e.t2_fanout_ok() ? 1 : 0;
+        if (fanouts) *fanouts = e.fanouts();
+        if (pack_doubles) e.t2_fanout_sizes(pack_doubles);
+    });
+}
+int pymes_t2_fanout(pymes_ctx* ctx, const double* t2, const double* t1, double* Xx, double* Xt, double* const* packs, int separate) {
+    return guarded([&] {
+        need(t2, "t2"); need(t1, "t1"); need(Xx, "Xx"); need(Xt, "Xt"); need(packs, "packs");
+        for (int i = 0; i < 6; ++i) need(packs[i], "packs[i]");
+        Engine& e = E(ctx);
+        if (!dev::fused_pair_kernels_ok(e.no)) throw pymes::Error("t2_fanout: nocc too large for the LDS tile");
+        if (!separate && !dev::sym_tail_ok()) throw pymes::Error("t2_fanout: not available in this backend");
+        e.t2_fanout_to(t2, t1, Xx, Xt, packs, separate != 0);
     });
 }
 int pymes_cc_update_to_sym(pymes_ctx* ctx, double* t_out, double* dt, const double* t_in, const double* r, double shift,
diff --git a/pymes_amd/csrc/cc.cpp b/pymes_amd/csrc/cc.cpp
--- a/pymes_amd/csrc/cc.cpp
+++ b/pymes_amd/csrc/cc.cpp
@@ -218,6 +218,67 @@
         permute(-1.0, T, "baij", 1.0, t4, "aibj");
     }
     lay_t2_ = t2;
+}
+
+bool Engine::t2_fanout_ok() {
+    if (const char* e = getenv("PYMES_T2_FANOUT"))
+        if (atoi(e) == 0) return false;
+    return !fan_off_ && sym_tail() && dev::t2_fanout_sym_ok(no, nv, stream);
+}
+
+void Engine::t2_fanout_sizes(int64_t out[6]) const {
+    const PairDims d = pair_dims();
+    const int64_t sp = d.npp * d.ldp, am = std::max<int64_t>(d.npm * d.ldm, 1);
+    out[0] = sp; out[1] = am; out[2] = sp; out[3] = am; out[4] = sp; out[5] = sp;
+}
+
+void Engine::t2_fanout_to(const double* t2, const double* t1, double* Tx, double* Ttd, double* const packs[6], bool separate) {
+    const PairDims d = pair_dims();
+    if (!separate) {
+        double* const Sp[3] = {packs[0], packs[2], packs[4]};
+        double* const Am[3] = {packs[1], packs[3], packs[5]};
+        dev::t2_fanout_sym(t2, t1, Tx, Ttd, Sp, Am, no, nv, d.ldp, d.ldm, stream);
+        return;
+    }
+    const int rflags = dev::PACK_COL_HALF | dev::PACK_AM_PROWS | dev::PACK_AM_PCOLS;
+    if (sym_tail()) dev::t2_layouts_sym(t2, nullptr, Tx, Ttd, no, nv, stream);
+    else dev::t2_layouts(t2, nullptr, Tx, Ttd, no, nv, stream);
+    dev::ladder_pack_T(t2, t1, packs[0], packs[1], no, nv, dev::PACK_ROW_HALF, d.ldp, d.ldm, stream);
+    dev::ladder_pack_T(t2, nullptr, packs[2], packs[3], no, nv, dev::PACK_ROW_HALF, d.ldp, d.ldm, stream);
+    dev::ladder_pack_T(t2, t1, packs[4], packs[5], no, nv, rflags, d.ldp, d.ldp, stream, 0, d.npp);
+}
+
+bool Engine::t2_fanout(const double* t2, const double* t1) {
+    const PairDims d = pair_dims();
+    const int64_t o = no, v = nv, ov = o * v;
+    int64_t want[6];
+    t2_fanout_sizes(want);
+    bool have = lay_[1] && lay_[2];
+    for (double* p : fan_) have = have && p;
+    if (!have) {
+        if (capturing_) throw Error("t2_fanout: the layouts and packs must exist before a launch graph is recorded (run one eager pass first)");
+        for (int i = 1; i < 3; ++i)
+            if (!lay_[i]) lay_[i] = static_cast<double*>(dev::dmalloc(sizeof(double) * ov * ov));
+        bool ok = true;
+        for (int i = 0; i < 6 && ok; ++i)
+            if (!fan_[i]) ok = (fan_[i] = static_cast<double*>(dev::try_dmalloc(sizeof(double) * want[i]))) != nullptr;
+        if (!ok) {
+            for (double*& p : fan_) { dev::dfree(p); p = nullptr; }
+            fan_off_ = true;
+            return false;
+        }
+    }
+    lay_t2_ = nullptr;
+    fan_t2_ = fan_t1_ = nullptr;
+    t2_fanout_to(t2, t1, lay_[1], lay_[2], fan_, false);
+    ++fanouts_;
+    stats.permute_calls++;
+    stats.permute_bytes += 8.0 * (double(d.npp) * double(o * o) + 2.0 * double(ov) * double(ov) + 4.0 * double(d.npp) * double(d.ldp) +
+                                  2.0 * double(d.npm) * double(d.ldm));
+    lay_t2_ = t2;
+    fan_t2_ = t2;
+    fan_t1_ = t1;
+    return true;
 }
 
 void Engine::slab_ladders(const double* t2, double* L, int rank, int world, unsigned flags, const double* t1, double* QK,
@@ -359,7 +420,16 @@
     if (L && !skip_ladder) check_shard_rank("residual_slab", rank, world);
     const double w = quad ? 1.0 : 0.5;
     TView F = make_view(const_cast<double*>(f), {nn, nn});
+    bool fan = L && !skip_ladder && !skip_rings && t1 && !dcd && !P && world == 1 && (flags & kSymTail) && ring_fold_enabled() &&
+               t2_fanout_ok();
+    struct FanGuard {
+        Engine& e;
+        ~FanGuard() { e.fan_t2_ = e.fan_t1_ = nullptr; }
+    } fan_guard{*this};
+    fan_t2_ = fan_t1_ = nullptr;
+    if (fan) fan = t2_fanout(t2, t1);
     if (L && !skip_ladder) slab_ladders(t2, L, rank, world, flags, t1, QK, P);
+    fan_t2_ = fan_t1_ = nullptr;
     if (skip_rings) return;
     ring_fold_.clear();
     int64_t c0, c1;
@@ -372,7 +442,7 @@
     auto pairm = [&](double* p) { return make_view(p, {ov, ov}); };
     const bool traces = !P && nc == ov;
     const bool fold = traces && ring_fold_enabled();
-    pair_layouts_of(t2, !fold, flags & kSymTail);
+    if (!(fan && fold && lay_t2_ == t2)) pair_layouts_of(t2, !fold, flags & kSymTail);
     TView Td = pairm(lay_[0]), Tx = pairm(lay_[1]), Ttd = pairm(lay_[2]);
     TView ETd = slice(pairm(ETd_p), 0, c0, c1), ETx = slice(pairm(ETx_p), 0, c0, c1);
     const int64_t b0 = c0 / o, b1 = (c1 + o - 1) / o;
@@ -1016,16 +1086,19 @@
         dev::ladder_pack_V(block(P_iabc).p, vp, vm, 0, nv, q0, q1, stream, d.vlp, d.vlm);
     }
     ijab_pack();
+    const bool fan = fan_t2_ == t2 && fan_t1_ == t1 && t2 && t1 && !dcd && !J && row0 == 0 && row1 == npp && fan_[0];
     ArenaScope scope(arena);
     TView Lrows = make_view(L + row0 * o * o, {rows, o * o});
     TView LS = slice(Lrows, 1, 0, opp), LA = slice(Lrows, 1, opp, o * o);
     {
         ArenaScope s2(arena);
-        double* Sp = arena.alloc(npp * ldp);
-        double* Am = arena.alloc(std::max<int64_t>(npm * ldm, 1));
-        dev::ladder_pack_T(t2, t1, Sp, Am, no, nv, dev::PACK_ROW_HALF, ldp, ldm, stream);
-        stats.permute_calls++;
-        stats.permute_bytes += 8.0 * 2.0 * double(v * v * o * o);
+        double* Sp = fan ? fan_[0] : arena.alloc(npp * ldp);
+        double* Am = fan ? fan_[1] : arena.alloc(std::max<int64_t>(npm * ldm, 1));
+        if (!fan) {
+            dev::ladder_pack_T(t2, t1, Sp, Am, no, nv, dev::PACK_ROW_HALF, ldp, ldm, stream);
+            stats.permute_calls++;
+            stats.permute_bytes += 8.0 * 2.0 * double(v * v * o * o);
+        }
         TView SpT = pitched(Sp, npp, opp, ldp), AmT = pitched(Am, npm, opm, ldm);
         const double* Ap = V.Vp;
         const double* Am_ = V.Vm;
@@ -1077,8 +1150,8 @@
     const HoleOperand h = hole_operand(block(P_klij, true).p);
     TView Ipv = pitched(h.Ip, opp, opp, ldp), Imv = pitched(h.Im, opp, opm, ldm);
     TView IpK = pitched(h.Ip, ldp, opp, ldp), ImK = pitched(h.Im, ldp, opm, ldm);
-    double* SpR = arena.alloc(npp * ldp);
-    double* AmR = arena.alloc(npp * ldp);
+    double* SpR = fan ? fan_[4] : arena.alloc(npp * ldp);
+    double* AmR = fan ? fan_[5] : arena.alloc(npp * ldp);
     const int rflags = dev::PACK_COL_HALF | dev::PACK_AM_PROWS | dev::PACK_AM_PCOLS;
     auto rowsS = [&]() { return slice(make_view(SpR, {npp, ldp}), 0, row0, row1); };
     auto rowsA = [&]() { return slice(make_view(AmR, {npp, ldp}), 0, row0, row1); };
@@ -1093,6 +1166,8 @@
         double* j = const_cast<double*>(J);
         axpby(1.0, pitched(j, opp, opp, ldp), bI, Ipv);
         if (opm > 0) axpby(1.0, pitched(j + opp * ldp, opp, opm, ldm), bI, Imv);
+    } else if (fan) {
+        hole_operand_add(h, fan_[2], fan_[3], bI, true);
     } else {
         ArenaScope s2(arena);
         double* Sp = arena.alloc(npp * ldp);
@@ -1100,9 +1175,11 @@
         dev::ladder_pack_T(t2, nullptr, Sp, Am, no, nv, dev::PACK_ROW_HALF, ldp, ldm, stream);
         hole_operand_add(h, Sp, Am, bI, true);
     }
-    dev::ladder_pack_T(dcd ? nullptr : t2, t1, SpR, AmR, no, nv, rflags, ldp, ldp, stream, row0, row1);
-    stats.permute_calls += 3;
-    stats.permute_bytes += 8.0 * 4.0 * double(v * v * o * o);
+    if (!fan) {
+        dev::ladder_pack_T(dcd ? nullptr : t2, t1, SpR, AmR, no, nv, rflags, ldp, ldp, stream, row0, row1);
+        stats.permute_calls += 3;
+        stats.permute_bytes += 8.0 * 4.0 * double(v * v * o * o);
+    }
     GemmGroupScope grp(stream);
     contract(1.0, rowsS(), "rk", IpK, "kn", 1.0, LS, "rn");
     if (opm > 0) contract(1.0, rowsA(), "rk", ImK, "kn", 1.0, LA, "rn");
@@ -1120,9 +1197,10 @@
     return 2 * v * v + 4 * o * v + 2 * o * o;
 }
 
-void Engine::dress_fock_partial(const double* t1, double* W, int rank, int world) {
+void Engine::dress_fock_partial(const double* t1, double* W, int rank, int world, bool have_gj) {
     const int64_t o = no, v = nv;
     if (world < 1 || rank < 0 || rank >= world) throw Error("dress_fock_partial: bad rank/world");
+    if (have_gj && world != 1) throw Error("dress_fock_partial: the sums of dress_V are whole sums (one rank)");
     int64_t j0, j1;
     chunk(o, rank, world, j0, j1);
     TView G1 = make_view(W, {v, v}), G2 = make_view(G1.p + v * v, {v, v}), J1 = make_view(G2.p + v * v, {o, v}),
@@ -1135,7 +1213,7 @@
     TView t = slice(make_view(const_cast<double*>(t1), {v, o}), 1, j0, j1);
     const bool all = (j0 == 0 && j1 == o);
     auto js = [&](int pat) { return all ? block(pat) : slice(block(pat), 0, j0, j1); };
-    const bool fused_g12 = dev::fock_g12_ok(nv);
+    const bool fused_g12 = !have_gj && dev::fock_g12_ok(nv);
     if (fused_g12) {
         ArenaScope s2(arena);
         const int ja = static_cast<int>(j0), jb = static_cast<int>(j1);
@@ -1150,11 +1228,11 @@
     };
     {
         Batch batch;
-        if (!fused_g12) {
+        if (!fused_g12 && !have_gj) {
             contract(1.0, t, "bj", js(P_iabc), "jabc", 0.0, G1, "ac");
             contract(1.0, t, "bj", js(P_iabc), "jacb", 0.0, G2, "ac");
         }
-        if (!fused_g12) {
+        if (!fused_g12 && !have_gj) {
             contract(1.0, t, "bj", js(P_ijab), "jkbc", 0.0, J1, "kc");
             contract(1.0, t, "bj", js(P_ijab), "jkcb", 0.0, J2, "kc");
         }
@@ -1260,9 +1338,38 @@
         case 0: contract(-1.0, tcut, "px", oth, "xqrs", 1.0, dst, "pqrs", "", cin); break;
         default: throw Error("bad index position");
     }
-}
-
-void Engine::dress_V(const double* t1, uint32_t mask, const int64_t* cut) {
+    if (fock_sums_ && fuse_copy && !reduced && !cut) {
+        const int64_t vv = static_cast<int64_t>(nv) * nv;
+        if (pattern == P_iajb && x == 2 && dst.p == Vd_[P_iajb]) fock_trace(dst, raw, 0, 2, 1, 3, fock_sums_);
+        if (pattern == P_iabj && x == 3 && dst.p == Vd_[P_iabj]) fock_trace(dst, raw, 0, 3, 1, 2, fock_sums_ + vv);
+    }
+}
+
+void Engine::fock_trace(const TView& D, const TView& R, int sa, int sb, int ia, int ja, double* out) {
+    if (D.rank != 4 || R.rank != 4 || D.dim[sa] != D.dim[sb]) throw Error("fock_trace: bad views");
+    for (int i = 0; i < 4; ++i)
+        if (D.dim[i] != R.dim[i]) throw Error("fock_trace: the two blocks differ in shape");
+    const int64_t ds[3] = {D.st[sa] + D.st[sb], D.st[ia], D.st[ja]}, rs[3] = {R.st[sa] + R.st[sb], R.st[ia], R.st[ja]};
+    dev::diag_traces(D.p, ds, R.p, rs, out, static_cast<int>(D.dim[ia]), static_cast<int>(D.dim[ja]), static_cast<int>(D.dim[sa]), stream);
+}
+
+bool Engine::fock_traces_ok() const {
+    if (const char* e = getenv("PYMES_FOCK_TRACES"))
+        if (atoi(e) == 0) return false;
+    return dev::diag_traces_ok();
+}
+
+void Engine::dress_V(const double* t1, uint32_t mask, const int64_t* cut, double* fock_sums) {
+    if (fock_sums) {
+        const uint32_t need = (1u << P_klij) | (1u << P_iajb) | (1u << P_iabj);
+        if (cut || (mask & need) != need) throw Error("dress_V: the Fock sums need the whole blocks klij, iajb and iabj");
+        if (!fock_traces_ok()) throw Error("dress_V: the partial traces are not available (PYMES_FOCK_TRACES=0 or this backend)");
+    }
+    struct SumsGuard {
+        double*& p;
+        ~SumsGuard() { p = nullptr; }
+    } sums_guard{fock_sums_};
+    fock_sums_ = fock_sums;
     ++dress_generation_;
     TView t = make_view(const_cast<double*>(t1), {(int64_t)nv, (int64_t)no});
     for (int axis = 0; axis < 2 && cut; ++axis)
@@ -1280,6 +1387,12 @@
         TView oth = make_view(arena.alloc(d[0] * d[1] * d[2] * d[3]), 4, d, nullptr);
         dressed_into(pat, pos, 1, t, oth, false, cut);
         dress_memo_[(((long)pat << 8 | 1L) << 3) | 4L] = oth;
+        if (fock_sums_) {
+            const int64_t vv = static_cast<int64_t>(nv) * nv, ov = static_cast<int64_t>(no) * nv;
+            fock_trace(oth, block(pat), 1, 3, 0, 2, fock_sums_ + 2 * vv);
+            fock_trace(oth, block(pat), 0, 3, 1, 2, fock_sums_ + 2 * vv + ov);
+            ++fock_trace_reads_;
+        }
     }
     for (int pat = 0; pat < 16; ++pat) {
         if (!(mask >> pat & 1u)) continue;
@@ -1404,8 +1517,17 @@
         residual_finish(f, t2, res_ETd_, res_ETx_, res_L_, r2, dcd | sym | PYMES_REUSE_LAYOUTS);
         return;
     }
-    dress_fock(f, t1, res_fd_);
-    dress_V(t1, (1u << pattern_of_name("klij")) | (1u << pattern_of_name("iajb")) | (1u << pattern_of_name("iabj")));
+    const uint32_t dmask = (1u << pattern_of_name("klij")) | (1u << pattern_of_name("iajb")) | (1u << pattern_of_name("iabj"));
+    if (fock_traces_ok()) {
+        ArenaScope scope(arena);
+        double* W = arena.alloc(dress_fock_ws_doubles());
+        dress_V(t1, dmask, nullptr, W);
+        dress_fock_partial(t1, W, 0, 1, true);
+        dress_fock_finish(f, t1, W, res_fd_);
+    } else {
+        dress_fock(f, t1, res_fd_);
+        dress_V(t1, dmask);
+    }
     residual_slab(res_fd_, t2, res_ETd_, res_ETx_, res_L_, 0, 1, dcd | sym | tail | PYMES_USE_DRESSED, t1, res_QK_);
     singles_residual_partial(res_fd_, t1, t2, r1, 0, 1, true);
     residual_finish(res_fd_, t2, res_ETd_, res_ETx_, res_L_, r2, dcd | sym | PYMES_USE_DRESSED | PYMES_REUSE_LAYOUTS, t1, res_QK_);
diff --git a/pymes_amd/csrc/device_api.h b/pymes_amd/csrc/device_api.h
--- a/pymes_amd/csrc/device_api.h
+++ b/pymes_amd/csrc/device_api.h
@@ -105,6 +105,9 @@
                   double shift, double delta, int no, int nv, int rank, stream_t s);
 void lincomb(double* out, int nx, const double* const* x, const double* c, int64_t n, stream_t s);
 bool sym_tail_ok();
+bool t2_fanout_sym_ok(int no, int nv, stream_t s);
+void t2_fanout_sym(const double* T, const double* t1, double* Tx, double* Ttd, double* const Sp[3], double* const Am[3], int no,
+                   int nv, int64_t ldp, int64_t ldm, stream_t s);
 void cc_update_to_sym(double* t_out, double* dt, const double* t_in, const double* r, const double* eo, const double* ev,
                       double shift, double delta, int no, int nv, stream_t s);
 void lincomb_sym(double* out, int nx, const double* const* x, const double* c, int no, int nv, stream_t s);
@@ -165,6 +168,9 @@
                    stream_t s);
 void pair_traces(const double* M, int64_t ld, double alpha, double beta, double* out_vv, double* out_oo, int no, int nv,
                  stream_t s, const double* M2 = nullptr, double alpha2 = 0.0);
+bool diag_traces_ok();
+void diag_traces(const double* D, const int64_t ds[3], const double* R, const int64_t rs[3], double* out, int ni, int nj, int ns,
+                 stream_t s);
 
 void ipea_pack(int k, const double* const* r1, const double* const* r2, int P, int S, int n1, double* U1, double* R, double* Rx,
                double* Rt, double* Rn, stream_t s);
diff --git a/pymes_amd/csrc/engine.cpp b/pymes_amd/csrc/engine.cpp
--- a/pymes_amd/csrc/engine.cpp
+++ b/pymes_amd/csrc/engine.cpp
@@ -128,6 +128,7 @@
         for (auto& kv : scratch_free_) dev::dfree(kv.second);
         for (auto& kv : scratch_live_) dev::dfree(kv.first);
         for (auto& p : lay_) dev::dfree(p);
+        for (auto& p : fan_) dev::dfree(p);
         dev::dfree(xs_oo_);
         dev::dfree(xs_vv_);
         for (auto& p : V_) dev::dfree(p);
@@ -811,4 +812,14 @@
 __attribute__((weak)) void t2_layouts_sym(const double*, double*, double*, double*, int, int, stream_t) {
     throw std::runtime_error("t2_layouts_sym: not available in this backend");
 }
-}
+__attribute__((weak)) bool t2_fanout_sym_ok(int, int, stream_t) { return false; }
+__attribute__((weak)) void t2_fanout_sym(const double*, const double*, double*, double*, double* const*, double* const*, int, int,
+                                         int64_t, int64_t, stream_t) {
+    throw std::runtime_error("t2_fanout_sym: not available in this backend");
+}
+__attribute__((weak)) bool diag_traces_ok() { return false; }
+__attribute__((weak)) void diag_traces(const double*, const int64_t*, const double*, const int64_t*, double*, int, int, int,
+                                       stream_t) {
+    throw std::runtime_error("diag_traces: not available in this backend");
+}
+}
diff --git a/pymes_amd/csrc/engine.h b/pymes_amd/csrc/engine.h
--- a/pymes_amd/csrc/engine.h
+++ b/pymes_amd/csrc/engine.h
@@ -147,10 +147,16 @@
     void hf_fock_matrix(const double* h_host, double* f_host);
     void dress_fock(const double* f, const double* t1, double* fd);
     int64_t dress_fock_ws_doubles() const;
-    void dress_fock_partial(const double* t1, double* W, int rank, int world);
+    void dress_fock_partial(const double* t1, double* W, int rank, int world, bool have_gj = false);
     void dress_fock_finish(const double* f, const double* t1, const double* W, double* fd);
     void xvv_partial(const double* f, const double* t2, double* Xvv, int rank, int world, unsigned flags);
-    void dress_V(const double* t1, uint32_t mask, const int64_t* cut = nullptr);
+    void dress_V(const double* t1, uint32_t mask, const int64_t* cut = nullptr, double* fock_sums = nullptr);
+    bool t2_fanout_ok();
+    void t2_fanout_sizes(int64_t out[6]) const;
+    void t2_fanout_to(const double* t2, const double* t1, double* Tx, double* Ttd, double* const packs[6], bool separate);
+    uint64_t fanouts() const { return fanouts_; }
+    bool fock_traces_ok() const;
+    uint64_t fock_trace_reads() const { return fock_trace_reads_; }
     void singles_residual(const double* fd, const double* t1, const double* t2, double* r1);
     void singles_residual_partial(const double* fd, const double* t1, const double* t2, double* r1, int rank, int world,
                                   bool reuse_layouts = false);
@@ -244,7 +250,13 @@
   private:
     double* lay_[3] = {nullptr, nullptr, nullptr};
     const double* lay_t2_ = nullptr;
+    double* fan_[6] = {nullptr, nullptr, nullptr, nullptr, nullptr, nullptr};
+    const double* fan_t2_ = nullptr;
+    const double* fan_t1_ = nullptr;
+    uint64_t fanouts_ = 0;
     void pair_layouts_of(const double* t2, bool want_td, bool sym = false);
+    bool t2_fanout(const double* t2, const double* t1);
+    bool fan_off_ = false;
     struct FoldTag {
         const double* t2 = nullptr;
         const double* etd = nullptr;
@@ -345,6 +357,9 @@
     int64_t splitk_doubles_ = 0;
     double* get_static(const std::string& key);
     std::map<long, TView> dress_memo_;
+    double* fock_sums_ = nullptr;
+    uint64_t fock_trace_reads_ = 0;
+    void fock_trace(const TView& D, const TView& R, int sa, int sb, int ia, int ja, double* out);
     void dressed_into(int pattern, const std::vector<int>& pos, int k, const TView& t1v, const TView& dst,
                       bool reduced = false, const int64_t* cut = nullptr);
     int64_t block_size(int pattern) const;
diff --git a/pymes_amd/csrc/kernels.hip b/pymes_amd/csrc/kernels.hip
--- a/pymes_amd/csrc/kernels.hip
+++ b/pymes_amd/csrc/kernels.hip
@@ -2232,6 +2232,85 @@
     for (int e = threadIdx.x; e < o2; e += blockDim.x) {
         const int j = e / no, i = e - j * no;
         Tx[base + (long)j * ov + i] = tile[i * p + j];
+    }
+}
+
+struct FanoutK {
+    const double* T; const double* t1; double* Tx; double* Ttd;
+    double* Sp[3]; double* Am[3];
+    long ldp, ldm;
+    int no, nv;
+};
+__global__ void __launch_bounds__(256) t2_fanout_sym_kernel(const FanoutK k) {
+    const double* __restrict__ T = k.T;
+    const double* __restrict__ t1 = k.t1;
+    double* __restrict__ Tx = k.Tx;
+    double* __restrict__ Ttd = k.Ttd;
+    const int no = k.no, nv = k.nv;
+    const long ldp = k.ldp, ldm = k.ldm;
+    extern __shared__ double tile[];
+    int c, d;
+    unrank_pair(blockIdx.x, c, d);
+    const int p = no + 1, o2 = no * no;
+    const long ov = (long)no * nv;
+    const double* __restrict__ Tab = T + ((long)c * nv + d) * o2;
+    for (int e = threadIdx.x; e < o2; e += blockDim.x) {
+        const int i = e / no, j = e - i * no;
+        tile[i * p + j] = Tab[e];
+    }
+    __syncthreads();
+    const long base = (long)c * no * ov + (long)d * no;
+    for (int e = threadIdx.x; e < o2; e += blockDim.x) {
+        const int i = e / no, j = e - i * no;
+        Ttd[base + (long)i * ov + j] = 2.0 * tile[i * p + j] - tile[j * p + i];
+    }
+    for (int e = threadIdx.x; e < o2; e += blockDim.x) {
+        const int j = e / no, i = e - j * no;
+        Tx[base + (long)j * ov + i] = tile[i * p + j];
+    }
+    if (c != d) {
+        const long bt = (long)d * no * ov + (long)c * no;
+        for (int e = threadIdx.x; e < o2; e += blockDim.x) {
+            const int i = e / no, j = e - i * no;
+            Ttd[bt + (long)i * ov + j] = 2.0 * tile[j * p + i] - tile[i * p + j];
+        }
+        for (int e = threadIdx.x; e < o2; e += blockDim.x) {
+            const int j = e / no, i = e - j * no;
+            Tx[bt + (long)j * ov + i] = tile[j * p + i];
+        }
+    }
+    const long row = blockIdx.x, mrow = (long)c * (c - 1) / 2 + d;
+    const long opp = (long)no * (no + 1) / 2, opm = opp - no;
+    const double fr = (c == d) ? 0.25 : 0.5;
+    if (threadIdx.x == 0) {
+        if (ldp > opp) {
+            k.Sp[0][row * ldp + opp] = 0.0;
+            k.Sp[1][row * ldp + opp] = 0.0;
+            k.Sp[2][row * ldp + opp] = 0.0;
+            k.Am[2][row * ldp + opp] = 0.0;
+        }
+        if (c > d && ldm > opm) {
+            k.Am[0][mrow * ldm + opm] = 0.0;
+            k.Am[1][mrow * ldm + opm] = 0.0;
+        }
+    }
+    for (int e = threadIdx.x; e < o2; e += blockDim.x) {
+        const int i = e / no, j = e - i * no;
+        if (i < j) continue;
+        const double x1 = tile[i * p + j], x2 = tile[j * p + i];
+        double y1 = x1, y2 = x2;
+        y1 += t1[(long)c * no + i] * t1[(long)d * no + j];
+        y2 += t1[(long)d * no + i] * t1[(long)c * no + j];
+        const long pc = (long)i * (i + 1) / 2 + j;
+        k.Sp[0][row * ldp + pc] = fr * (y1 + y2);
+        k.Sp[1][row * ldp + pc] = fr * (x1 + x2);
+        k.Sp[2][row * ldp + pc] = ((i == j) ? 0.5 * 0.5 : 0.5) * (y1 + y2);
+        k.Am[2][row * ldp + pc] = (c > d && i > j) ? 0.5 * (y1 - y2) : 0.0;
+        if (c > d && i > j) {
+            const long mc = (long)i * (i - 1) / 2 + j;
+            k.Am[0][mrow * ldm + mc] = 0.5 * (y1 - y2);
+            k.Am[1][mrow * ldm + mc] = 0.5 * (x1 - x2);
+        }
     }
 }
 
@@ -2765,14 +2844,42 @@
     pair_traces_body(q, blockIdx.x, part);
 }
 
+struct DiagTracesK {
+    const double* D; const double* R; double* out;
+    long ds, di, dj, rs, ri, rj;
+    int ni, nj, ns, jtiles;
+};
+__device__ __forceinline__ void diag_traces_body(const DiagTracesK& q, const unsigned vb, double* __restrict__ smem) {
+    const double* __restrict__ D = q.D;
+    const double* __restrict__ R = q.R;
+    const int lane = threadIdx.x & 63, wave = threadIdx.x >> 6;
+    const int i = vb / q.jtiles, j = (vb - i * q.jtiles) * 64 + lane;
+    double (*part)[64] = reinterpret_cast<double (*)[64]>(smem);
+    double acc = 0.0;
+    if (i < q.ni && j < q.nj) {
+        const double* __restrict__ d = D + (long)i * q.di + (long)j * q.dj;
+        const double* __restrict__ r = R + (long)i * q.ri + (long)j * q.rj;
+#pragma unroll 4
+        for (int s = wave; s < q.ns; s += 4) acc += d[(long)s * q.ds] - r[(long)s * q.rs];
+    }
+    part[wave][lane] = acc;
+    __syncthreads();
+    if (wave == 0 && i < q.ni && j < q.nj)
+        q.out[(long)i * q.nj + j] = ((part[0][lane] + part[1][lane]) + part[2][lane]) + part[3][lane];
+}
+__global__ void __launch_bounds__(256) diag_traces_kernel(const DiagTracesK q) {
+    __shared__ double part[kTracesLdsDoubles];
+    diag_traces_body(q, blockIdx.x, part);
+}
+
 enum : unsigned short {
     PK_GEMM = 0, PK_SPLITK, PK_PERM_DIRECT, PK_PERM_TILED, PK_GEMV_COLS, PK_GEMV_FINISH, PK_GEMV_ROWS, PK_CC_UPDATE, PK_LINCOMB,
     PK_DOTS1, PK_DOTS2, PK_ENERGY, PK_TAU, PK_PACK_T, PK_LADDER_UNPACK, PK_RING_OPERANDS, PK_T2_LAYOUTS, PK_ASSEMBLE,
-    PK_ROWS_UNPACK, PK_FOCK_G12, PK_FOCK_G12_FIN, PK_FOCK_FT, PK_FOCK_FIN, PK_TRACES, PK_DOTS_FINAL, PK_KINDS
+    PK_ROWS_UNPACK, PK_FOCK_G12, PK_FOCK_G12_FIN, PK_FOCK_FT, PK_FOCK_FIN, PK_TRACES, PK_DOTS_FINAL, PK_DIAG_TRACES, PK_KINDS
 };
 constexpr const char* kPhaseKindNames[] = {"gemm", "splitk", "perm", "permT", "gemvC", "gemvF", "gemvR", "update", "lincomb", "dots1", "dots2",
                                            "energy", "tau", "packT", "unpackL", "ringops", "layouts", "assemble", "unpackR", "fockG", "fockGf",
-                                           "fockFt", "fockFin", "traces", "dotsF"};
+                                           "fockFt", "fockFin", "traces", "dotsF", "diagTr"};
 static_assert(sizeof(kPhaseKindNames) / sizeof(kPhaseKindNames[0]) == PK_KINDS, "one name per phase kind");
 struct SplitkTaskK { GemmK g; int BM, BN; };
 struct PermTaskK { PermK p; long total; int tiles_q, tiles_l; };
@@ -2892,6 +2999,7 @@
             if constexpr (HEAVY) fock_finish_body(phase_args<FockFinK>(args), vb);
             break;
         case PK_TRACES: pair_traces_body(phase_args<TracesK>(args), vb, smem); break;
+        case PK_DIAG_TRACES: diag_traces_body(phase_args<DiagTracesK>(args), vb, smem); break;
         default: break;
     }
 }
@@ -4753,6 +4861,25 @@
     launch_kernel(t2_layouts_sym_kernel, dim3((unsigned)(nv * nv)), dim3(256), sizeof(double) * no * (no + 1), (hipStream_t)s, k);
 }
 
+bool t2_fanout_sym_ok(int no, int nv, stream_t s) {
+    if (!fused_pair_kernels_ok(no) || no < 1 || nv < 1) return false;
+    phase_open((hipStream_t)s);
+    return !phase_small(40.0 * (double)nv * nv * no * no / 4.0e6);
+}
+void t2_fanout_sym(const double* T, const double* t1, double* Tx, double* Ttd, double* const Sp[3], double* const Am[3], int no,
+                   int nv, int64_t ldp, int64_t ldm, stream_t s) {
+    if (!fused_pair_kernels_ok(no)) throw std::runtime_error("t2_fanout_sym: nocc too large for the LDS tile");
+    if (no < 1 || nv < 1) return;
+    const long opp = (long)no * (no + 1) / 2;
+    if (ldp < opp || ldm < opp - no) throw std::runtime_error("t2_fanout_sym: pitch below the packed row");
+    if (!T || !t1 || !Tx || !Ttd) throw std::runtime_error("t2_fanout_sym: null array");
+    for (int z = 0; z < 3; ++z)
+        if (!Sp[z] || !Am[z]) throw std::runtime_error("t2_fanout_sym: null pack");
+    const FanoutK k{T, t1, Tx, Ttd, {Sp[0], Sp[1], Sp[2]}, {Am[0], Am[1], Am[2]}, (long)ldp, (long)ldm, no, nv};
+    launch_kernel(t2_fanout_sym_kernel, dim3((unsigned)((long)nv * (nv + 1) / 2)), dim3(256), sizeof(double) * no * (no + 1),
+                  (hipStream_t)s, k);
+}
+
 void residual_assemble(const double* V, const double* L, const double* N, const double* D, const double* X, double* R,
                        int no, int nv, stream_t s, double xd) {
     if (!fused_pair_kernels_ok(no)) throw std::runtime_error("residual_assemble: nocc too large for the LDS tile");
@@ -4903,6 +5030,26 @@
         return;
     }
     launch_kernel(pair_traces_kernel, dim3(blocks), dim3(256), 0, (hipStream_t)s, k);
+}
+
+bool diag_traces_ok() { return true; }
+void diag_traces(const double* D, const int64_t ds[3], const double* R, const int64_t rs[3], double* out, int ni, int nj, int ns,
+                 stream_t s) {
+    if (ni <= 0 || nj <= 0 || ns <= 0) throw std::runtime_error("diag_traces: empty extents");
+    for (int x = 0; x < 3; ++x)
+        if (ds[x] <= 0 || rs[x] <= 0) throw std::runtime_error("diag_traces: strides must be positive");
+    const int jtiles = (nj + 63) / 64;
+    const long blocks = (long)ni * jtiles;
+    const DiagTracesK k{D, R, out, (long)ds[0], (long)ds[1], (long)ds[2], (long)rs[0], (long)rs[1], (long)rs[2], ni, nj, ns, jtiles};
+    const double lines = (double)ni * (double)nj * (double)ns;
+    const double cost = ((ds[2] == 1 ? 8.0 : 128.0) + (rs[2] == 1 ? 8.0 : 128.0)) * lines / 4.0e6 + 2.0;
+    if (phase_open((hipStream_t)s) && phase_small(cost)) {
+        PhaseRec& t = phase_push(PK_DIAG_TRACES, 0, blocks, kTracesLdsDoubles * (int)sizeof(double), cost, k);
+        phase_reads(t, {pbox(D, {{ns, ds[0]}, {ni, ds[1]}, {nj, ds[2]}}), pbox(R, {{ns, rs[0]}, {ni, rs[1]}, {nj, rs[2]}})});
+        phase_writes(t, {prange(out, (long)ni * nj)});
+        return;
+    }
+    launch_kernel(diag_traces_kernel, dim3((unsigned)blocks), dim3(256), 0, (hipStream_t)s, k);
 }
 
 }
diff --git a/pymes_amd/device.py b/pymes_amd/device.py
--- a/pymes_amd/device.py
+++ b/pymes_amd/device.py
@@ -361,6 +361,26 @@
         else:
             self.lib.call("pymes_ccsd_dress_V", self.handle, C.c_void_p(t1.ptr), mask)
 
+    def t2_fanout_info(self):
+        yes, n, sizes = C.c_int(), C.c_uint64(), (C.c_int64 * 6)()
+        self.lib.call("pymes_t2_fanout_info", self.handle, C.byref(yes), C.byref(n), sizes)
+        return bool(yes.value), int(n.value), [int(x) for x in sizes]
+
+    def t2_fanout(self, t2, t1, Xx, Xt, packs, separate=False):
+        ptrs = (C.c_void_p * 6)(*[p.ptr for p in packs])
+        self.lib.call("pymes_t2_fanout", self.handle, C.c_void_p(t2.ptr), C.c_void_p(t1.ptr), C.c_void_p(Xx.ptr), C.c_void_p(Xt.ptr),
+                      ptrs, int(separate))
+
+    def dress_V_fock_sums(self, t1, sums):
+        mask = sum(1 << pattern_of(nm) for nm in ("klij", "iajb", "iabj"))
+        self.lib.call("pymes_ccsd_dress_V_fock_sums", self.handle, C.c_void_p(t1.ptr), mask, C.c_void_p(sums.ptr))
+        return sums
+
+    def fock_traces(self):
+        yes, n = C.c_int(), C.c_uint64()
+        self.lib.call("pymes_fock_traces", self.handle, C.byref(yes), C.byref(n))
+        return bool(yes.value), int(n.value)
+
     def ccsd_residuals(self, f, t1, t2, r1, r2, is_dcd=False, t1_zero=False, sym_tail=False):
         self.lib.call("pymes_ccsd_residuals", self.handle, C.c_void_p(f.ptr), C.c_void_p(t1.ptr), C.c_void_p(t2.ptr),
                       (_lib.PYMES_DCD if is_dcd else 0) | (_lib.PYMES_T1_ZERO if t1_zero else 0) |
```

Result: no change. 0.1580 (median of 6 runs) (-0.9%).
